# niels747/2D-Weather-Sandbox

Hardware: AMD Instinct MI355X
Metric: Mcell-steps/s (higher is better)
Workload: dtype f32

## Files before the change

2d-weather-sandbox_amd/csrc/wx_ens_score.h:

```cpp
#pragma once
#include <hip/hip_runtime.h>
#include <stdint.h>
#include <string.h>
#include "../../include/wxsim.h"
#include "wx_diag.h"
#include "wx_ens_quant.h"
#include "wx_ens_score_cell.h"

namespace wxs {

typedef unsigned long long u64;
enum { WG = wxq::WG, WAVES = wxq::WAVES, MAX_WGS = 2048, SHARDS = 8, MAP_ROWS = 4 };
enum { NQ = NT * 4, T_LO = 0, T_HI = NQ * wxd::NB, T_CNT = 2 * NQ * wxd::NB, T_SUMN = T_CNT + 16, T_LOW = T_SUMN + 4, T_HIGH = T_LOW + 4 * BINS, T_WORDS = T_HIGH + 4 * BINS };
enum { L_BINS = 0, L_CNT = 2 * NQ * wxd::NB, L_SUMN = L_CNT + 16, L_LOW = L_SUMN + 4, L_HIGH = L_LOW + 4 * BINS, L_WORDS = L_HIGH + 4 * BINS };
static_assert(MAX_MEMBERS == wxq::STAGED_MEMBERS && L_WORDS * 4 == 4720 && T_WORDS == 1180, "the tables");

struct Args {
  int X;
  int x0, y0, w, h;
  int n_sel;
  const wxe::Member *tab;
  u64 *table;
  float4 *error, *variance, *crps;
};
// ... 106 lines not shown
    for (int c = 0; c < 4; c++) {
      for (int k = 0; k < NT; k++)
        for (int b = 0; b < wxd::NB; b++) {
          a.lo[c][k][b] += tab[T_LO + (k * 4 + c) * wxd::NB + b];
          a.hi[c][k][b] += (int64_t)tab[T_HI + (k * 4 + c) * wxd::NB + b];
        }
      for (int q = 0; q < 4; q++) a.cnt[q][c] += (int64_t)tab[T_CNT + q * 4 + c];
      a.sum_count[c] += (int64_t)tab[T_SUMN + c];
      for (int b = 0; b < BINS; b++) a.low[c][b] += (int64_t)tab[T_LOW + c * BINS + b], a.high[c][b] += (int64_t)tab[T_HIGH + c * BINS + b];
    }
}

template <int P>
static hipError_t launch(const Args &a, unsigned wgs, hipStream_t stream)
{
  hipLaunchKernelGGL(k_ens_score<P>, dim3(wgs), dim3(WG), 0, stream, a);
  return hipGetLastError();
}

}

int wx_ens_score_max_members(void) { return wxs::MAX_MEMBERS; }

int wx_ens_score_cells(int n_members, size_t n_cells, const float *const *field, const int8_t *const *wall, const float *truth_field, const int8_t *truth_wall,
                       const uint8_t *member_mask, wx_ens_score *out)
{
  return wxs::score_cells(n_members, n_cells, field, wall, truth_field, truth_wall, member_mask, out);
}

int wx_ensemble_scores(wx_ensemble *e, wx_sim *truth, int field, int x, int y, int w, int h, const uint8_t *member_mask, wx_ens_score *out)
{
  if (!e || !truth || !out) return WX_E_INVALID;
  if (field != WX_FIELD_BASE_CUR && field != WX_FIELD_WATER_CUR)
    return efail(e, WX_E_INVALID, "wx_ensemble_scores: field %d: WX_FIELD_BASE_CUR or WX_FIELD_WATER_CUR (the fields that are stored whole and interleaved)", field);
  const int B = (int)e->member.size();
  const char *why;
  if (int rc = wxs::check_selection(B, member_mask, &why)) return efail(e, rc, "wx_ensemble_scores: %s", why);
  std::vector<int> sel;
  for (int i = 0; i < B; i++)
    if (!member_mask || member_mask[i]) sel.push_back(i);
  for (int i : sel)
    if (e->member[i] == truth) return efail(e, WX_E_INVALID, "wx_ensemble_scores: truth is member %d, which is selected: the truth does not enter (mask it out)", i);
  if (truth->halo != 0 || truth->X != truth->Xg) return efail(e, WX_E_INVALID, "wx_ensemble_scores: truth is a slab handle (whole-domain handles only)");
  if (truth->X != e->X || truth->Y != e->Y) return efail(e, WX_E_INVALID, "wx_ensemble_scores: truth has %d x %d cells, the members %d x %d", truth->X, truth->Y, e->X, e->Y);
  if (truth->device != e->device) return efail(e, WX_E_INVALID, "wx_ensemble_scores: truth lives on device %d, the ensemble on device %d", truth->device, e->device);
  if (w <= 0 || h <= 0 || x < 0 || y < 0 || (long long)x + w > e->X || (long long)y + h > e->Y)
    return efail(e, WX_E_RANGE, "wx_ensemble_scores: rect (%d,%d %dx%d) outside %dx%d (no wrap)", x, y, w, h, e->X, e->Y);
  for (int i : sel)
    if (!e->member[i]->uploaded) return efail(e, WX_E_STATE, "member %d: wx_ensemble_scores before wx_upload", i);
  if (!truth->uploaded) return efail(e, WX_E_STATE, "truth: wx_ensemble_scores before wx_upload");
  if (e->broken) return WX_E_STATE;
  DeviceScope dev_scope(e->member[0]);

  if (truth->ens != e)
    if (int rc = wx_sync(truth)) return efail(e, rc, "truth: %s", truth->err.c_str());

  const size_t cells = (size_t)w * h, table_bytes = (size_t)wxs::SHARDS * wxs::T_WORDS * sizeof(wxs::u64);
  float *const host_ptr[3] = {out->error, out->variance, out->crps};
  size_t at[3], out_bytes = table_bytes;
  for (int p = 0; p < 3; p++) {
    at[p] = out_bytes;
    if (host_ptr[p]) out_bytes += cells * 16;
  }
  const int n_sel = (int)sel.size();
  if (int rc = ens_stat_reserve(e, n_sel + 1, out_bytes)) return rc;
  EnsStatState *st = e->stat;

  auto entry = [&](const wx_sim *m, int i) { return wxe::Member{field == WX_FIELD_BASE_CUR ? m->base[0] : m->water[1], m->wall[0], i, 0}; };
  for (int k = 0; k < n_sel; k++) st->tab_host[k] = entry(e->member[sel[k]], sel[k]);
  st->tab_host[n_sel] = entry(truth, -1);
  wxs::Args a;
  memset(&a, 0, sizeof(a));
  a.X = e->X, a.x0 = x, a.y0 = y, a.w = w, a.h = h, a.n_sel = n_sel;
  a.tab = st->tab_dev;
  a.table = (wxs::u64 *)st->out_dev;
  auto dev_plane = [&](int p) -> float4 * { return host_ptr[p] ? (float4 *)(st->out_dev + at[p]) : nullptr; };
  a.error = dev_plane(0), a.variance = dev_plane(1), a.crps = dev_plane(2);
  int P = 1;
  while (P < n_sel) P <<= 1;

  hipError_t he = hipMemcpyAsync(st->tab_dev, st->tab_host, (size_t)(n_sel + 1) * sizeof(wxe::Member), hipMemcpyHostToDevice, e->stream);
  if (he == hipSuccess) he = hipMemsetAsync(st->out_dev, 0, table_bytes, e->stream);
  if (he == hipSuccess) {
    const unsigned chunks = (unsigned)((w + 63) / 64) * (unsigned)h;
    const unsigned wgs = std::min<unsigned>(chunks, wxs::MAX_WGS);
    ProfScope ps(e->member[0], K_ENS_SCORE);
    switch (P) {
    case 1: he = wxs::launch<1>(a, wgs, e->stream); break;
    case 2: he = wxs::launch<2>(a, wgs, e->stream); break;
    case 4: he = wxs::launch<4>(a, wgs, e->stream); break;
    case 8: he = wxs::launch<8>(a, wgs, e->stream); break;
    case 16: he = wxs::launch<16>(a, wgs, e->stream); break;
    case 32: he = wxs::launch<32>(a, wgs, e->stream); break;
    default: he = wxs::launch<wxs::MAX_MEMBERS>(a, wgs, e->stream); break;
    }
  }
  if (he == hipSuccess) he = hipMemcpyAsync(st->out_host, st->out_dev, out_bytes, hipMemcpyDeviceToHost, e->stream);
  if (he != hipSuccess) {
    (void)hipStreamSynchronize(e->stream);
    return efail(e, WX_E_DEVICE, "wx_ensemble_scores (%s): %s", kKernelNames[K_ENS_SCORE], hipGetErrorString(he));
  }
  if (int rc = wx_ensemble_sync(e)) return rc;
  wxs::Acc *acc = new wxs::Acc();
  wxs::acc_from_table((const wxs::u64 *)st->out_host, *acc);
  wxs::acc_finish(*acc, out);
  delete acc;
// ... 5 lines not shown
```

2d-weather-sandbox_amd/csrc/wx_state_copy.h:

```cpp
#pragma once

namespace {

struct StateCopyPlan {
  FullCtx fc;
};

int state_copy_check(wx_sim *dst, const wx_sim *src, const char *fn)
{
  if (src->halo != 0 || dst->halo != 0 || src->X != src->Xg || dst->X != dst->Xg) return fail(dst, WX_E_INVALID, "%s: whole-domain handles only (a slab's ghost columns and pool bookkeeping belong to its ring)", fn);
  if (src->X != dst->X || src->Y != dst->Y || src->n_drops != dst->n_drops)
    return fail(dst, WX_E_INVALID, "%s: %d x %d cells with %d droplets into %d x %d cells with %d droplets", fn, src->X, src->Y, src->n_drops, dst->X, dst->Y, dst->n_drops);
  if (src->device != dst->device) return fail(dst, WX_E_INVALID, "%s: the handles live on devices %d and %d", fn, src->device, dst->device);
  if (!src->uploaded) return fail(dst, WX_E_STATE, "%s: src was never uploaded", fn);
  if (!src->have_params) return fail(dst, WX_E_STATE, "%s: src has no parameters (wx_set_params)", fn);
  const Storage &a = src->store, &b = dst->store;
  bool same = a.created_blocks == b.created_blocks && a.created_slots == b.created_slots && a.created_small_used == b.created_small_used && a.created_blocks > 0 &&
              (int)a.blocks.size() >= a.created_blocks && (int)b.blocks.size() >= b.created_blocks;
  for (int i = 1; same && i < a.created_blocks; i++) same = a.blocks[i].bytes == b.blocks[i].bytes;
  if (!same) return fail(dst, WX_E_STATE, "%s: the two handles' storage was not laid out alike", fn);
  return WX_OK;
}

int state_copy_enqueue(wx_sim *dst, wx_sim *src, hipStream_t st, StateCopyPlan &plan)
{
  const Storage &a = src->store;
  Storage &b = dst->store;
  if (dst->copy_in_flight) HIPCHK(dst, hipStreamWaitEvent(st, dst->ev_copy_done, 0));
  for (int i = 0; i < a.created_blocks; i++) {
    const size_t bytes = i == 0 ? (a.one_arena ? a.blocks[0].bytes : a.created_small_used) : a.blocks[i].bytes;
    HIPCHK(dst, hipMemcpyAsync(b.blocks[i].p, a.blocks[i].p, bytes, hipMemcpyDeviceToDevice, st));
  }
  for (int k = 0; k < a.created_slots; k++) {
    const int i = block_of(a.blocks, *a.slots[k]);
    if (i < 0 || i >= a.created_blocks) return fail(dst, WX_E_STATE, "wx_copy_state: a registered pointer of src lies outside its blocks");
    *b.slots[k] = b.blocks[i].p + ((const char *)*a.slots[k] - a.blocks[i].p);
  }
  dst->run = src->run;
  dst->run.wet_shape_valid = false;
  dst->run.fix_check = false;
  dst->p = src->p;
  dst->geo = src->geo;
  dst->uni = src->uni;
  dst->have_params = src->have_params;
  dst->uploaded = true;
  dst->w0.even = src->w0.even;
  dst->w0.uni = src->w0.uni;
  dst->w0.initT_saved = src->w0.initT_saved;
  if (src->w0.initT_saved) {
    const size_t nb = ((size_t)src->Y + 1) * 4;
    if (!dst->w0.initT) HIPCHK(dst, hipMalloc((void **)&dst->w0.initT, nb));
    HIPCHK(dst, hipMemcpyAsync(dst->w0.initT, src->w0.initT, nb, hipMemcpyDeviceToDevice, st));
  }
  dst->vx.stale = true;
  dst->vx.untracked = false;
  dst->vx.have[0] = dst->vx.have[1] = false;
  dst->vx.check = false;
  plan.fc = FullCtx{dst->geo, dst->uni, dst->initial_T, dst->snd_T, dst->snd_W, dst->snd_Vel};
  HIPCHK(dst, hipMemcpyAsync(dst->full_ctx, &plan.fc, sizeof(FullCtx), hipMemcpyHostToDevice, st));
  HIPCHK(dst, hipMemsetAsync(&dst->state->ghost_nontrivial, 0, 5 * 4, st));
  HIPCHK(dst, hipMemsetAsync(&dst->state->vx_max_bits, 0, 2 * 4, st));
  if (dst->pair.words) {
    HIPCHK(dst, hipMemsetAsync(dst->pair.words + D2_N_REDO, 0, 4, st));
    HIPCHK(dst, hipMemsetAsync(dst->pair.words + D2_FIXED, 0, 8, st));
  }
  return WX_OK;
}

static_assert(offsetof(DevState, fastest_bits) - offsetof(DevState, ghost_nontrivial) == 16 && offsetof(DevState, cone_violation) - offsetof(DevState, vx_max_bits) == 4,
              "state_copy_enqueue zeroes these words as two runs");

}

int wx_copy_state(wx_sim *dst, wx_sim *src)
{
  if (!dst || !src) return WX_E_INVALID;
  if (dst == src) return WX_OK;
  if (int rc = state_copy_check(dst, src, "wx_copy_state")) return rc;
  DeviceScope dev_scope(src);
  if (int rc = wx_sync(src)) {
    dst->err = "wx_copy_state: src: " + src->err;
    return rc;
  }
  if (dst->comm_stream) HIPCHK(dst, hipStreamSynchronize(dst->comm_stream));
  HIPCHK(dst, hipStreamSynchronize(dst->stream));
  StateCopyPlan plan;
  int rc = state_copy_enqueue(dst, src, dst->stream, plan);
  const hipError_t he = hipStreamSynchronize(dst->stream);
  if (rc == WX_OK && he != hipSuccess) rc = fail(dst, WX_E_DEVICE, "wx_copy_state: %s", hipGetErrorString(he));
  return rc;
}

int wx_ensemble_broadcast(wx_ensemble *e, int src_member, const uint8_t *member_mask)
{
  if (!e) return WX_E_INVALID;
  const int B = (int)e->member.size();
  if (src_member < 0 || src_member >= B) return efail(e, WX_E_INVALID, "wx_ensemble_broadcast: member %d of %d", src_member, B);
  wx_sim *src = e->member[src_member];
  if (!src->uploaded) return efail(e, WX_E_STATE, "member %d: wx_ensemble_broadcast: src was never uploaded", src_member);
  if (!src->have_params) return efail(e, WX_E_STATE, "member %d: wx_ensemble_broadcast: src has no parameters (wx_set_params)", src_member);
  if (e->broken) return WX_E_STATE;
  std::vector<int> sel;
  for (int i = 0; i < B; i++)
    if (i != src_member && (!member_mask || member_mask[i])) sel.push_back(i);
  for (int i : sel)
    if (int rc = epass(e, i, state_copy_check(e->member[i], src, "wx_ensemble_broadcast"))) return rc;
  if (sel.empty()) return WX_OK;
  DeviceScope dev_scope(src);
  if (int rc = epass(e, src_member, validate_ghost_flag(src))) return rc;
  std::vector<StateCopyPlan> plans(sel.size());
  int rc = WX_OK;
  for (size_t k = 0; k < sel.size() && rc == WX_OK; k++) rc = epass(e, sel[k], state_copy_enqueue(e->member[sel[k]], src, e->stream, plans[k]));
  const hipError_t he = hipStreamSynchronize(e->stream);
  if (rc == WX_OK && he != hipSuccess) rc = efail(e, WX_E_DEVICE, "wx_ensemble_broadcast: %s", hipGetErrorString(he));
  return rc;
}
```

2d-weather-sandbox_amd/csrc/wx_tile.h:

```cpp
#pragma once
#include "wx_cells.h"

#include <cstdlib>
#include <algorithm>
#ifdef WX_DEBUG
inline const char *wx_tune_env(const char *name) { return std::getenv(name); }
#else
inline const char *wx_tune_env(const char *) { return nullptr; }
#endif

namespace wx {

constexpr int TX = 64, TY = 16;

template <typename F, typename F2> struct LightPlanesT {
  F *x, *y;
  F2 *zw;
};
using LightPlanes = LightPlanesT<float, float2>;
using LightPlanesC = LightPlanesT<const float, const float2>;

__device__ __forceinline__ size_t fidx(int x, int y, int X) { return (size_t)y * X + x; }
__device__ __forceinline__ int wrapfast(int i, int n) { return i < 0 ? i + n : (i >= n ? i - n : i); }

inline dim3 tile_grid(int X, int Y) { return dim3((X + 63) / 64, (Y + 15) / 16); }

template <int H, int W> struct Planes4 {
  float x[H][W], y[H][W], z[H][W], w[H][W];
  __device__ __forceinline__ void put(int r, int c, float4 v)
  {
    x[r][c] = v.x;
    y[r][c] = v.y;
    z[r][c] = v.z;
    w[r][c] = v.w;
  }
  __device__ __forceinline__ float4 get(int r, int c) const { return make_float4(x[r][c], y[r][c], z[r][c], w[r][c]); }
};

namespace fb_ {
constexpr int REACH = 1;
constexpr int HL = 1 + REACH, HR = REACH, HD = 1 + REACH, HU = REACH;
constexpr int IW = TX + HL + HR, IH = TY + HD + HU;
constexpr int AW = TX + 1, AH = TY + 1;
constexpr float VMAX = 0.9f;
struct SmemOut {
  float vx[AH][AW], vy[AH][AW], T[AH][AW];
  char4 w[AH][AW + 1];
};
}

struct AdvOut {
  float4 b, w;
  char4 wl;
};

__device__ __forceinline__ void edge_wave_prio(int prio)
{
#if defined(__HIP_DEVICE_COMPILE__)
  if (prio == 1) __builtin_amdgcn_s_setprio(1);
  else if (prio == 2) __builtin_amdgcn_s_setprio(2);
  else if (prio >= 3) __builtin_amdgcn_s_setprio(3);
#endif
}
struct VxTrack {
  int *max_bits;
  int *violation;
  float limit;
  int zone_l, zone_r;
  float limit_in;
};
__device__ __forceinline__ float speed8(float q0, float q1, float q2, float q3, float q4, float q5, float q6, float q7)
{
  const float m = fmaxf(fmaxf(fmaxf(fabsf(q0), fabsf(q1)), fmaxf(fabsf(q2), fabsf(q3))), fmaxf(fmaxf(fabsf(q4), fabsf(q5)), fmaxf(fabsf(q6), fabsf(q7))));
// ... 10 lines not shown
#if defined(__HIP_DEVICE_COMPILE__)
  float m = lane_max;
  if (t.zone_l < t.zone_r && strip >= t.zone_l && strip < t.zone_r) {
    if (!(t.limit_in > 0.0f)) return;
    for (int o = 32; o > 0; o >>= 1) m = fmaxf(m, __shfl_xor(m, o));
    if (lane == 0 && t.violation != nullptr && m >= t.limit_in) atomicMax(t.violation, __float_as_int(m));
    return;
  }
  for (int o = 32; o > 0; o >>= 1) m = fmaxf(m, __shfl_xor(m, o));
  if (lane == 0 && t.max_bits != nullptr && m >= 0.5f) {
    atomicMax(t.max_bits, __float_as_int(m));
    if (t.limit > 0.0f && m >= t.limit) atomicMax(t.violation, __float_as_int(m));
  }
#endif
}
__global__ void k_vx_scan(int X, int Y, int col_l, int col_r, const float4 *__restrict__ base, VxTrack t)
{
  float m = 0.0f, m_in = 0.0f;
  const size_t n = (size_t)X * Y;
  for (size_t i = (size_t)blockIdx.x * blockDim.x + threadIdx.x; i < n; i += (size_t)gridDim.x * blockDim.x) {
    const int x = (int)(i % (size_t)X);
    const float v = vx_mag(base[i].x);
    if (col_l >= col_r || x < col_l || x >= col_r)
      m = fmaxf(m, v);
    else
      m_in = fmaxf(m_in, v);
  }
  t.zone_l = t.zone_r = 0;
  vx_track_commit(t, m, threadIdx.x & 63);
  if (t.limit_in > 0.0f) {
    t.zone_l = 0;
    t.zone_r = 1;
    vx_track_commit(t, m_in, threadIdx.x & 63, 0);
  }
}

__global__ void k_light_to_planes(size_t n, const float4 *__restrict__ src, LightPlanes dst)
{
  for (size_t i = (size_t)blockIdx.x * blockDim.x + threadIdx.x; i < n; i += (size_t)gridDim.x * blockDim.x) {
    const float4 l = src[i];
    dst.x[i] = l.x;
    dst.y[i] = l.y;
    dst.zw[i] = make_float2(l.z, l.w);
  }
}
__global__ void k_light_from_planes(size_t n, LightPlanesC src, float4 *__restrict__ dst)
{
  for (size_t i = (size_t)blockIdx.x * blockDim.x + threadIdx.x; i < n; i += (size_t)gridDim.x * blockDim.x) {
    const float2 zw = src.zw[i];
    dst[i] = make_float4(src.x[i], src.y[i], zw.x, zw.y);
  }
}

}
```

2d-weather-sandbox_amd/csrc/wx_wet.h:

```cpp
#pragma once
#include "wx_cells.h"
#include "wx_tile.h"
#include <cstddef>
#include <type_traits>
#include <cstdlib>
#include <algorithm>

namespace wx {

#ifndef WX_WET_MINWAVES
#define WX_WET_MINWAVES 4
#endif
#ifndef WX_WET_WPB
#define WX_WET_WPB 4
#endif
#ifndef WX_ABL_FORCE_AIR
#define WX_ABL_FORCE_AIR 0
#endif

struct FullCtx {
  Geo g;
  Uni u;
  const float *initial_T, *snd_T, *snd_W, *snd_Vel;
};

struct WetIn {
  const float4 *base;
  const char4 *wall;
  const float4 *water;
  LightPlanesC l0;
  LightPlanesC lsrc;
  const float3 *fb;
  const float2 *dep;
  const unsigned char *fb_zero;
  const float4 *zero_row;
  int fb_txn;
};
struct WetOut {
  float4 *base;
  char4 *wall;
  float4 *water;
  LightPlanes light;
  float *p_disp;
  float4 *water0;
  float *curl;
  float *t_disp;
#ifdef WX_WET_TIMING
  unsigned long long *cycles;
#endif
};

struct WetFixList {
  int *count;
  int2 *cells;
  int cap;
  const int *hint_host;
  int *fastest;
  int *hint;
};

struct WetSlowArgs {
  const FullCtx *ctx;
  WetIn in;
  float iterNum;
};
struct GWetRecomputeAcc {
  const Uni &u_;
  const WetIn &in_;
  int X, Y, x, y;
  __device__ __forceinline__ int wx_(int dx) const { return wrapmod(x + dx, X); }
  __device__ __forceinline__ int wy_(int dy) const { return wrapmod(y + dy, Y); }
  __device__ __forceinline__ float4 vel_at(int xx, int yy) const
  {
    const int xr = xx + 1 == X ? 0 : xx + 1, yu = yy + 1 == Y ? 0 : yy + 1;
    return velocity_cell(u_, in_.base[fidx(xx, yy, X)], in_.base[fidx(xr, yy, X)].z, in_.base[fidx(xx, yu, X)].z, in_.wall[fidx(xx, yy, X)].y);
  }
  __device__ __forceinline__ float curl_at(int xx, int yy) const
  {
    const int xr = xx + 1 == X ? 0 : xx + 1, yu = yy + 1 == Y ? 0 : yy + 1;
    const float4 v = vel_at(xx, yy);
    return curl_cell(v.x, v.y, vel_at(xr, yy).y, vel_at(xx, yu).x);
  }
  __device__ __forceinline__ float4 base(int dx, int dy) const { return vel_at(wx_(dx), wy_(dy)); }
  __device__ __forceinline__ char4 wall(int dx, int dy) const { return in_.wall[fidx(wx_(dx), wy_(dy), X)]; }
  __device__ __forceinline__ float4 water(int dx, int dy) const { return in_.water[fidx(wx_(dx), wy_(dy), X)]; }
  __device__ __forceinline__ float2 vort(int dx, int dy) const
  {
    const int xx = wx_(dx), yy = wy_(dy);
    const int xl = xx == 0 ? X - 1 : xx - 1, xr = xx + 1 == X ? 0 : xx + 1, yd = yy == 0 ? Y - 1 : yy - 1, yu = yy + 1 == Y ? 0 : yy + 1;
    return vorticity_cell(curl_at(xx, yy), curl_at(xl, yy), curl_at(xr, yy), curl_at(xx, yd), curl_at(xx, yu));
  }
  __device__ __forceinline__ float light_y0() const { return in_.l0.y[fidx(x, y, X)]; }
  __device__ __forceinline__ float light_x0() const { return in_.l0.x[fidx(x, y, X)]; }
  __device__ __forceinline__ float2 light_xy_up() const
  {
    const size_t i = fidx(x, y + 1 > Y - 1 ? Y - 1 : y + 1, X);
    return make_float2(in_.l0.x[i], in_.l0.y[i]);
  }
  __device__ __forceinline__ bool has_fb() const { return in_.fb != nullptr; }
  __device__ __forceinline__ float4 fb() const
  {
    if (!in_.fb) return make_float4(0.f, 0.f, 0.f, 0.f);
    const float3 v = in_.fb[fidx(x, y, X)];
    return make_float4(v.x, v.y, v.z, 0.f);
  }
  __device__ __forceinline__ float2 dep() const { return in_.dep ? in_.dep[fidx(x, y, X)] : make_float2(0.f, 0.f); }
};
struct BOut {
  float4 b, w;
  char4 wl;
};
__device__ __noinline__ BOut wet_boundary_texel_global(const WetSlowArgs *__restrict__ sa, int x, int y)
{
  const FullCtx *c = sa->ctx;
  GWetRecomputeAcc a{c->u, sa->in, c->g.X, c->g.Y, x, y};
  BOut o;
  boundary_cell(c->u, sa->iterNum, (int)sa->iterNum, c->g, c->initial_T, x, y, a, o.b, o.w, o.wl);
  return o;
}
struct GWetAdvectAcc {
  const WetSlowArgs *sa;
  int X, Y, x, y;
  __device__ __forceinline__ BOut at(int dx, int dy) const { return wet_boundary_texel_global(sa, wrapmod(x + dx, X), wrapmod(y + dy, Y)); }
  __device__ __forceinline__ float4 base(int dx, int dy) const { return at(dx, dy).b; }
  __device__ __forceinline__ char4 wall(int dx, int dy) const { return at(dx, dy).wl; }
  __device__ __forceinline__ float4 base_off(int dx, int dy) const { return at(dx, dy).b; }
  __device__ __forceinline__ float4 water_off(int dx, int dy) const { return at(dx, dy).w; }
  __device__ __forceinline__ char4 wall_off(int dx, int dy) const { return at(dx, dy).wl; }
};
__device__ __noinline__ AdvOut wet_advection_cell_recompute(const WetSlowArgs *__restrict__ sa, int x, int y)
{
  const FullCtx *c = sa->ctx;
  GWetAdvectAcc a{sa, c->g.X, c->g.Y, x, y};
  AdvOut o;
  advection_cell(c->u, c->g, c->initial_T, c->snd_T, c->snd_W, c->snd_Vel, x, y, a, o.b, o.w, o.wl);
  return o;
}
struct GWetLightAcc {
  LightPlanesC l;
  float4 water_;
  char4 wall_;
  float T0, Td;
  int X, x;
  __device__ __forceinline__ float T(int dy) const { return dy == 0 ? T0 : Td; }
  __device__ __forceinline__ float4 water() const { return water_; }
  __device__ __forceinline__ char4 wall() const { return wall_; }
  __device__ __forceinline__ float sun_at(int dx, int j) const { return l.x[fidx(wrapmod(x + dx, X), j, X)]; }
  __device__ __forceinline__ float ir_down_at(int j) const { return l.zw[fidx(x, j, X)].x; }
  __device__ __forceinline__ float ir_up_at(int j) const { return l.zw[fidx(x, j, X)].y; }
};
__device__ __noinline__ void wet_output_cell_exact(const FullCtx *__restrict__ c, const WetIn *__restrict__ in, const WetOut *__restrict__ out, float iterNum,
                                                   int opt_out, int x, int y)
{
  const WetSlowArgs sa{c, *in, iterNum};
  const int X = c->g.X, Y = c->g.Y;
  const AdvOut o0 = wet_advection_cell_recompute(&sa, x, y);
  const AdvOut oL = wet_advection_cell_recompute(&sa, x == 0 ? X - 1 : x - 1, y);
  const AdvOut oD = wet_advection_cell_recompute(&sa, x, y == 0 ? Y - 1 : y - 1);
  const size_t gi = fidx(x, y, X);
  out->base[gi] = pressure_cell(o0.b, oL.b.x, oD.b.y, oD.b.w, oD.wl.x, oD.wl.y);
  out->water[gi] = o0.w;
  out->wall[gi] = o0.wl;
  GWetLightAcc la{in->lsrc, o0.w, o0.wl, o0.b.w, oD.b.w, X, x};
  const float4 l = lighting_cell(c->u, c->g, x, y, la);
  out->light.x[gi] = l.x;
  out->light.y[gi] = l.y;
  out->light.zw[gi] = make_float2(l.z, l.w);
  if (opt_out) out->p_disp[gi] = o0.b.z;
  if (out->t_disp) out->t_disp[gi] = o0.b.w;
}

constexpr int WOUT = 56;
constexpr int WLO = 4;
constexpr int WPAD = 1;
constexpr int WRW = 64 + 2 * WPAD;
constexpr int WQ = 3;
constexpr int WL = 4;
struct WetRing {
  float P[WQ][WRW], T[WQ][WRW], vx[WQ][WRW], vy[WQ][WRW];
  char4 wl[WQ][WRW];
  float qx[WQ][WRW], qy[WQ][WRW], qz[WQ][WRW], qw[WQ][WRW];
  float lx[WL][WRW], lw[WL][WRW];
};
static_assert(sizeof(WetRing) == (5 * WQ + 4 * WQ + 2 * WL) * WRW * 4, "ring layout");

__device__ __forceinline__ float wave_from_left(float v)
{
  const int i = __float_as_int(v);
  return __int_as_float(__builtin_amdgcn_update_dpp(i, i, 0x138 , 0xf, 0xf, false));
}
__device__ __forceinline__ float wave_from_right(float v)
{
  const int i = __float_as_int(v);
  return __int_as_float(__builtin_amdgcn_update_dpp(i, i, 0x130 , 0xf, 0xf, false));
}
__device__ __forceinline__ void wave_fence()
{
  __builtin_amdgcn_fence(__ATOMIC_RELEASE, "wavefront");
  __builtin_amdgcn_wave_barrier();
  __builtin_amdgcn_fence(__ATOMIC_ACQUIRE, "wavefront");
}
__device__ __forceinline__ char4 unpack_wall(int w)
{
  return make_char4((signed char)(w & 0xff), (signed char)((w >> 8) & 0xff), (signed char)((w >> 16) & 0xff), (signed char)(w >> 24));
}

struct MWBoundaryAcc {
  const WetRing &rg;
  int li, o0;
  float vxU, TU;
  char4 wU;
  float4 b00, q00, qU;
  char4 w00, wD;
  float vxD, TD, qzD, qwD;
// ... 94 lines not shown
  __device__ __forceinline__ float ir_up_at(int j) const { return rg.lw[(j + 8) & (WL - 1)][li]; }
};

__device__ __forceinline__ unsigned long long uniform_addr(const void *p)
{
  const unsigned long long v = (unsigned long long)p;
  const unsigned lo = __builtin_amdgcn_readfirstlane((unsigned)v), hi = __builtin_amdgcn_readfirstlane((unsigned)(v >> 32));
  return ((unsigned long long)hi << 32) | lo;
}
#if defined(__HIP_DEVICE_COMPILE__)
template <class T> __device__ __forceinline__ T ld_row(const T *row, unsigned &byte_off)
{
  typedef const __attribute__((address_space(1))) char *GBytes;
  typedef const __attribute__((address_space(1))) T *GPtr;
  asm("" : "+v"(byte_off));
  return *(GPtr)((GBytes)uniform_addr(row) + byte_off);
}
template <class T> __device__ __forceinline__ void st_row(T *row, unsigned &byte_off, T v)
{
  typedef __attribute__((address_space(1))) char *GBytes;
  asm("" : "+v"(byte_off));
  typedef __attribute__((address_space(1))) T *GPtr;
  *(GPtr)((GBytes)uniform_addr(row) + byte_off) = v;
}
#else
template <class T> __device__ __forceinline__ T ld_row(const T *row, unsigned &byte_off) { return *reinterpret_cast<const T *>(reinterpret_cast<const char *>(row) + byte_off); }
template <class T> __device__ __forceinline__ void st_row(T *row, unsigned &byte_off, T v) { *reinterpret_cast<T *>(reinterpret_cast<char *>(row) + byte_off) = v; }
#endif
template <class T> __device__ __forceinline__ T ld_row_v(const T *row, unsigned byte_off) { return ld_row(row, byte_off); }
template <class T> __device__ __forceinline__ void st_row_v(T *row, unsigned byte_off, T v) { st_row(row, byte_off, v); }
__device__ __forceinline__ int ring_back(int s, int k, int n)
{
  const int v = s - k;
  return v < 0 ? v + n : v;
}

constexpr int WMAXSEG = 128;
struct WetSegs {
  int n_seg;
  int bands;
  int start[WMAXSEG + 1];
};
struct WetKArgs {
  const FullCtx *ctx;
  float iterNum;
  WetIn in;
  WetOut out;
  WetFixList fix;
  int n_strips, strip_lo, n_strips_all;
  WetSegs segs;
  int split_at, strip_lo2;
  int edge_prio;
  VxTrack vx;
};
struct WetEnsSlot {
  WetKArgs ka;
  int *overflow;
  int pad_[2 + (16 - (sizeof(WetKArgs) + sizeof(int *) + 8) % 16) % 16 / 4];
};
static_assert(sizeof(WetEnsSlot) % 16 == 0, "table slots keep the 16-byte alignment of the wide scalar loads");
template <bool OPT_OUT, bool HAS_FB, bool QUIET>
__global__ __launch_bounds__(64 * WX_WET_WPB, WX_WET_MINWAVES) void k_march_wet(const FullCtx *__restrict__ ctx, float iterNum, WetIn in_arg, WetOut out_arg,
                                                                    WetFixList fix_arg, int n_strips, int strip_lo,
                                                                    int n_strips_all, WetSegs segs, int split_at, int strip_lo2, int edge_prio_arg, VxTrack vx_arg)
{
  typedef WetKArgs KArgs;
  typedef const __attribute__((address_space(4))) char *KBytes;
#if defined(__HIP_DEVICE_COMPILE__)
  const KBytes ka_c = (KBytes)__builtin_amdgcn_kernarg_segment_ptr();
#else
  const KBytes ka_c = nullptr;
#endif
#include "wx_wet_march_body.h"
}

template <bool OPT_OUT, bool HAS_FB, bool QUIET>
__global__ __launch_bounds__(64 * WX_WET_WPB, WX_WET_MINWAVES) void k_march_wet_ens(const WetEnsSlot *__restrict__ table)
{
  typedef WetKArgs KArgs;
  typedef const __attribute__((address_space(4))) char *KBytes;
  const KBytes ka_c = (KBytes)(const char *)table + (size_t)blockIdx.y * sizeof(WetEnsSlot);
  const __attribute__((address_space(4))) KArgs &ka = *(const __attribute__((address_space(4))) KArgs *)ka_c;
  const FullCtx *__restrict__ ctx = ka.ctx;
  const float iterNum = ka.iterNum;
  const int n_strips = ka.n_strips, strip_lo = ka.strip_lo, n_strips_all = ka.n_strips_all, split_at = ka.split_at, strip_lo2 = ka.strip_lo2;
  const __attribute__((address_space(4))) WetSegs &segs = ka.segs;
#include "wx_wet_march_body.h"
}

#undef WX_WALL_RAW
#undef WX_H_SET
#undef WX_H_ROT

constexpr int WPATCH = 8, WPATCH_C = 4;
struct WetPatch {
  float vx[WPATCH * WPATCH], vy[WPATCH * WPATCH], P[WPATCH * WPATCH], T[WPATCH * WPATCH];
  float qx[WPATCH * WPATCH], qy[WPATCH * WPATCH], qz[WPATCH * WPATCH], qw[WPATCH * WPATCH];
  char4 wl[WPATCH * WPATCH];
};
struct WetPatchAcc {
  const WetPatch &p;
  int cx, cy;
  bool *bad;
  __device__ __forceinline__ int at(int dx, int dy) const
  {
    const int x = cx + dx, y = cy + dy;
    if (x < 0 || x >= WPATCH || y < 0 || y >= WPATCH) {
      *bad = true;
      return 0;
    }
    return y * WPATCH + x;
  }
  __device__ __forceinline__ float4 base(int dx, int dy) const
  {
    const int i = at(dx, dy);
    return make_float4(p.vx[i], p.vy[i], p.P[i], p.T[i]);
  }
  __device__ __forceinline__ char4 wall(int dx, int dy) const { return p.wl[at(dx, dy)]; }
  __device__ __forceinline__ float4 base_off(int dx, int dy) const { return base(dx, dy); }
  __device__ __forceinline__ char4 wall_off(int dx, int dy) const { return wall(dx, dy); }
  __device__ __forceinline__ float4 water_off(int dx, int dy) const
  {
    const int i = at(dx, dy);
    return make_float4(p.qx[i], p.qy[i], p.qz[i], p.qw[i]);
  }
};

constexpr int WSB = 13, WSV = 12, WSC = 11, WSF = 9;
struct WetFixStage {
  float bx[WSB * WSB], by[WSB * WSB], bP[WSB * WSB], bT[WSB * WSB];
  char4 bw[WSB * WSB];
  float vx[WSV * WSV], vy[WSV * WSV];
  float cu[WSC * WSC];
  float fx[WSF * WSF], fy[WSF * WSF];
};
struct WetStageBoundaryAcc {
  const WetFixStage &st;
  const Uni &u_;
  const WetIn &in_;
  int X, Y, x, y;
  int px, py;
  __device__ __forceinline__ float4 base(int dx, int dy) const
  {
    const int iv = (py + 2 + dy) * WSV + (px + 2 + dx), ib = (py + 2 + dy) * WSB + (px + 2 + dx);
    return make_float4(st.vx[iv], st.vy[iv], st.bP[ib], st.bT[ib]);
  }
  __device__ __forceinline__ char4 wall(int dx, int dy) const { return st.bw[(py + 2 + dy) * WSB + (px + 2 + dx)]; }
  __device__ __forceinline__ float4 water(int dx, int dy) const { return in_.water[fidx(wrapmod(x + dx, X), wrapmod(y + dy, Y), X)]; }
  __device__ __forceinline__ float2 vort(int dx, int dy) const
  {
    const int i = (py + 1 + dy) * WSF + (px + 1 + dx);
    return make_float2(st.fx[i], st.fy[i]);
  }
  __device__ __forceinline__ float light_y0() const { return in_.l0.y[fidx(x, y, X)]; }
  __device__ __forceinline__ float light_x0() const { return in_.l0.x[fidx(x, y, X)]; }
  __device__ __forceinline__ float2 light_xy_up() const
  {
    const size_t i = fidx(x, y + 1 > Y - 1 ? Y - 1 : y + 1, X);
    return make_float2(in_.l0.x[i], in_.l0.y[i]);
  }
  __device__ __forceinline__ bool has_fb() const { return in_.fb != nullptr; }
  __device__ __forceinline__ float4 fb() const
  {
    if (!in_.fb) return make_float4(0.f, 0.f, 0.f, 0.f);
    const float3 v = in_.fb[fidx(x, y, X)];
    return make_float4(v.x, v.y, v.z, 0.f);
  }
  __device__ __forceinline__ float2 dep() const { return in_.dep ? in_.dep[fidx(x, y, X)] : make_float2(0.f, 0.f); }
};
__device__ __noinline__ void wet_fix_build_patch(const FullCtx *__restrict__ c, const WetIn *__restrict__ in, float iterNum, WetFixStage *__restrict__ stp,
                                                 WetPatch *__restrict__ ptp, int cx, int cy, int lane)
{
  WetFixStage &st = *stp;
  WetPatch &pt = *ptp;
  const int X = c->g.X, Y = c->g.Y;
  for (int i = lane; i < WSB * WSB; i += 64) {
    const int sy = i / WSB, sx = i - sy * WSB;
    const size_t gi = fidx(wrapmod(cx - 6 + sx, X), wrapmod(cy - 6 + sy, Y), X);
    const float4 b = in->base[gi];
    st.bx[i] = b.x;
    st.by[i] = b.y;
    st.bP[i] = b.z;
    st.bT[i] = b.w;
    st.bw[i] = in->wall[gi];
  }
  wave_fence();
  for (int i = lane; i < WSV * WSV; i += 64) {
    const int sy = i / WSV, sx = i - sy * WSV, ib = sy * WSB + sx;
    const float4 v = velocity_cell(c->u, make_float4(st.bx[ib], st.by[ib], st.bP[ib], st.bT[ib]), st.bP[ib + 1], st.bP[ib + WSB], st.bw[ib].y);
    st.vx[i] = v.x;
    st.vy[i] = v.y;
  }
  wave_fence();
  for (int i = lane; i < WSC * WSC; i += 64) {
    const int sy = i / WSC, sx = i - sy * WSC, iv = sy * WSV + sx;
    st.cu[i] = curl_cell(st.vx[iv], st.vy[iv], st.vy[iv + 1], st.vx[iv + WSV]);
  }
  wave_fence();
  for (int i = lane; i < WSF * WSF; i += 64) {
    const int sy = i / WSF, sx = i - sy * WSF, ic = (sy + 1) * WSC + (sx + 1);
    const float2 f = vorticity_cell(st.cu[ic], st.cu[ic - 1], st.cu[ic + 1], st.cu[ic - WSC], st.cu[ic + WSC]);
    st.fx[i] = f.x;
    st.fy[i] = f.y;
  }
  wave_fence();
  {
    const int px = lane & (WPATCH - 1), py = lane >> 3;
    const int gx = wrapmod(cx - WPATCH_C + px, X), gy = wrapmod(cy - WPATCH_C + py, Y);
    const WetStageBoundaryAcc a{st, c->u, *in, X, Y, gx, gy, px, py};
    float4 bb, bq;
    char4 bwl;
    boundary_cell(c->u, iterNum, (int)iterNum, c->g, c->initial_T, gx, gy, a, bb, bq, bwl);
    pt.vx[lane] = bb.x;
    pt.vy[lane] = bb.y;
    pt.P[lane] = bb.z;
    pt.T[lane] = bb.w;
    pt.qx[lane] = bq.x;
    pt.qy[lane] = bq.y;
    pt.qz[lane] = bq.z;
    pt.qw[lane] = bq.w;
    pt.wl[lane] = bwl;
  }
  wave_fence();
}

template <bool OPT_OUT>
__global__ __launch_bounds__(256) void k_wet_fix(const FullCtx *__restrict__ ctx, float iterNum, WetIn in, WetOut out, int *__restrict__ count,
                                                 const int2 *__restrict__ cells, int cap, int *__restrict__ overflow, int *__restrict__ hint)
{
#include "wx_wet_fix_body.h"
}

template <bool OPT_OUT>
__global__ __launch_bounds__(256) void k_wet_fix_ens(const WetEnsSlot *__restrict__ table)
{
  const WetEnsSlot &sl = table[blockIdx.y];
  const FullCtx *__restrict__ ctx = sl.ka.ctx;
  const float iterNum = sl.ka.iterNum;
  const WetIn in = sl.ka.in;
  const WetOut out = sl.ka.out;
  int *__restrict__ count = sl.ka.fix.count;
  const int2 *__restrict__ cells = sl.ka.fix.cells;
  const int cap = sl.ka.fix.cap;
  int *__restrict__ overflow = sl.overflow;
  int *__restrict__ hint = sl.ka.fix.hint;
#include "wx_wet_fix_body.h"
}

#ifndef WX_WET_ROUNDS
#define WX_WET_ROUNDS 4
#endif
struct WetLaunch {
  int n_strips;
  WetSegs segs;
};
inline int wet_capacity()
{
  static int capacity = 0;
  if (!capacity) {
    int dev = 0, ncu = 0, nb = 0;
    if (hipGetDevice(&dev) != hipSuccess || hipDeviceGetAttribute(&ncu, hipDeviceAttributeMultiprocessorCount, dev) != hipSuccess ||
        hipOccupancyMaxActiveBlocksPerMultiprocessor(&nb, k_march_wet<false, false, true>, 64 * WX_WET_WPB, 0) != hipSuccess || ncu <= 0 || nb <= 0) {
      capacity = 256 * 4 * WX_WET_MINWAVES;
    } else {
      hipFuncAttributes fa;
      int by_regs = nb, by_lds = nb;
      if (hipFuncGetAttributes(&fa, reinterpret_cast<const void *>(k_march_wet<false, false, true>)) == hipSuccess) {
        if (fa.numRegs > 0) by_regs = (512 / (((fa.numRegs + 7) / 8) * 8)) * 4 / WX_WET_WPB;
        if (fa.sharedSizeBytes > 0) by_lds = (int)(163840 / fa.sharedSizeBytes);
        if (wx_tune_env("WX_MARCH_DEBUG")) fprintf(stderr, "[wx_wet] numRegs=%d lds=%zu: blocks/CU by registers %d, by LDS %d, occupancy API %d\n", fa.numRegs, fa.sharedSizeBytes, by_regs, by_lds, nb);
      }
      nb = std::max(1, std::min(nb, std::min(by_regs, by_lds)));
      capacity = ncu * nb * WX_WET_WPB;
    }
    if (wx_tune_env("WX_MARCH_DEBUG")) fprintf(stderr, "[wx_wet] CUs=%d blocks/CU=%d capacity=%d\n", ncu, nb, capacity);
  }
  return capacity;
}
inline double wet_alpha()
{
  double alpha = 1.0;
  if (const char *e = wx_tune_env("WX_WET_ALPHA")) alpha = atof(e) >= 1.0 ? atof(e) : alpha;
  return alpha;
}
inline WetLaunch wet_launch_shape_cap(const Geo &g, int air_from_row, int bands_mode, const int capacity)
{
  WetLaunch w;
  const int strips_all = (g.X + WOUT - 1) / WOUT;
  bool bands = bands_mode >= 2 ? g.Y >= 16 : (bands_mode != 0 && (g.Y >= 8 * 64 || (strips_all < 146 && g.Y >= 128)));
  if (const char *e = wx_tune_env("WX_WET_BANDS")) bands = atoi(e) >= 2 ? g.Y >= 16 : (atoi(e) != 0 && g.Y >= 8 * 64);
  const int Y = bands ? (g.Y + 7) / 8 : g.Y;
  w.segs.bands = bands ? 1 : 0;
  w.n_strips = (g.X + WOUT - 1) / WOUT;
  int rounds = WX_WET_ROUNDS, minrows = 24;
  const double alpha = wet_alpha();
  if (const char *e = wx_tune_env("WX_WET_ROUNDS")) rounds = atoi(e) > 0 ? atoi(e) : rounds;
  {
    const long long cap = capacity, per_row_set = (long long)w.n_strips * (bands ? 8 : 1);
// ... 50 lines not shown
    if (n > 0 && n <= (Y + 7) / 8) n_seg = n;
  }
  w.segs.start[0] = 0;
  double wsum = 0.0, wacc = 0.0;
  for (int sg = 0; sg < n_seg; sg++) wsum += wt[sg];
  for (int sg = 1; sg < n_seg; sg++) {
    wacc += wt[sg - 1];
    const double c = total * wacc / wsum;
    int y = c <= alpha * A ? (int)(c / alpha + 0.5) : A + (int)(c - alpha * A + 0.5);
    if (y <= w.segs.start[sg - 1]) y = w.segs.start[sg - 1] + 1;
    w.segs.start[sg] = y < Y ? y : Y;
  }
  w.segs.start[n_seg] = Y;
  while (n_seg > 1 && w.segs.start[n_seg - 1] >= Y) n_seg--;
  w.segs.start[n_seg] = Y;
  w.segs.n_seg = n_seg;
  return w;
}

inline WetLaunch wet_launch_shape(const Geo &g, int air_from_row, int bands_mode = 1) { return wet_launch_shape_cap(g, air_from_row, bands_mode, wet_capacity()); }

inline int wet_member_share(const Geo &g, int n_members, int capacity)
{
  const int cap = capacity > 0 ? capacity : wet_capacity();
  if (const char *e = wx_tune_env("WX_ENS_SHARE")) n_members = atoi(e) > 0 ? atoi(e) : n_members;
  if (n_members <= 1) return cap;
  const int strips = (g.X + WOUT - 1) / WOUT;
  return std::max(cap / n_members, std::min(cap, strips));
}
inline WetLaunch wet_launch_shape_member(const Geo &g, int air_from_row, int bands_mode, int n_members, int capacity = 0)
{
  return wet_launch_shape_cap(g, air_from_row, bands_mode, wet_member_share(g, n_members, capacity));
}

inline WetLaunch wet_shape_halved(const WetLaunch &w)
{
  WetLaunch h = w;
  int n = 0;
  for (int sg = 0; sg < w.segs.n_seg; sg++) n += w.segs.start[sg + 1] - w.segs.start[sg] >= 12 ? 2 : 1;
  if (n > WMAXSEG) return w;
  n = 0;
  for (int sg = 0; sg < w.segs.n_seg; sg++) {
    const int a = w.segs.start[sg], b = w.segs.start[sg + 1];
    h.segs.start[n++] = a;
    if (b - a >= 12) h.segs.start[n++] = a + (b - a) / 2;
  }
  h.segs.start[n] = w.segs.start[w.segs.n_seg];
  h.segs.n_seg = n;
  return h;
}

inline void launch_march_wet(const WetLaunch &w, float iterNum, const FullCtx *ctx, const WetIn &in, const WetOut &out, const WetFixList &fix,
                             bool opt_out, bool quiet, hipStream_t stream, int strip_lo = 0, int strip_count = -1, int strip_lo2 = 0, int strip_count2 = 0,
                             int edge_prio = 0, const VxTrack *vx = nullptr)
{
  const int ns1 = strip_count < 0 ? w.n_strips : strip_count, ns = ns1 + (strip_count2 > 0 ? strip_count2 : 0);
  if (ns <= 0) return;
  const int groups = ((w.segs.bands ? ns : (ns + 7) / 8) + WX_WET_WPB - 1) / WX_WET_WPB;
  const dim3 grid(8 * groups * w.segs.n_seg);
  static bool dbg = wx_tune_env("WX_MARCH_DEBUG") != nullptr;
  if (dbg) {
    fprintf(stderr, "[wx_wet] strips=%d segs=%d waves=%d first/last segment rows=%d/%d\n", w.n_strips, w.segs.n_seg, w.n_strips * w.segs.n_seg,
            w.segs.start[1] - w.segs.start[0], w.segs.start[w.segs.n_seg] - w.segs.start[w.segs.n_seg - 1]);
    dbg = false;
  }
  const bool has_fb = in.fb != nullptr;
  VxTrack vt = vx ? *vx : VxTrack{nullptr, nullptr, 0.0f, 0, 0};
  if (vx && vx->zone_l < vx->zone_r) {
    vt.zone_l = (vx->zone_l + WOUT - 1) / WOUT;
    vt.zone_r = vx->zone_r / WOUT;
  }
#define WX_LAUNCH_W(O, F, Q) \
  hipLaunchKernelGGL((k_march_wet<O, F, Q>), grid, dim3(64 * WX_WET_WPB), 0, stream, ctx, iterNum, in, out, fix, ns, strip_lo, w.n_strips, w.segs, ns1, strip_lo2, edge_prio, vt)
#define WX_LAUNCH_WQ(O, F) \
  do { if (quiet) WX_LAUNCH_W(O, F, true); else WX_LAUNCH_W(O, F, false); } while (0)
  if (opt_out) {
    if (has_fb) WX_LAUNCH_WQ(true, true); else WX_LAUNCH_WQ(true, false);
  } else {
    if (has_fb) WX_LAUNCH_WQ(false, true); else WX_LAUNCH_WQ(false, false);
  }
#undef WX_LAUNCH_WQ
#undef WX_LAUNCH_W
}

inline void launch_wet_fix(float iterNum, const FullCtx *ctx, const WetIn &in, const WetOut &out, const WetFixList &fix, int *overflow, bool opt_out,
                           hipStream_t stream, int wgs = 0)
{
  const int last = fix.hint ? *(volatile const int *)fix.hint_host : -1;
  const int want = last < 0 ? 512 : (last > 0 ? std::min(512, std::max(32, last)) : 32);
  const dim3 grid(wgs > 0 ? wgs : want), block(256);
  if (opt_out)
    hipLaunchKernelGGL((k_wet_fix<true>), grid, block, 0, stream, ctx, iterNum, in, out, fix.count, fix.cells, fix.cap, overflow, fix.hint);
  else
    hipLaunchKernelGGL((k_wet_fix<false>), grid, block, 0, stream, ctx, iterNum, in, out, fix.count, fix.cells, fix.cap, overflow, fix.hint);
}

inline int ens_member_groups(const WetLaunch &w)
{
  const int groups = ((w.segs.bands ? w.n_strips : (w.n_strips + 7) / 8) + WX_WET_WPB - 1) / WX_WET_WPB;
  return 8 * groups * w.segs.n_seg;
}
inline void launch_march_wet_ens(const WetEnsSlot *table, int n_members, int groups_x, bool opt_out, bool has_fb, bool quiet, hipStream_t stream)
{
  const dim3 grid(groups_x, n_members), block(64 * WX_WET_WPB);
#define WX_LAUNCH_E(O, F, Q) hipLaunchKernelGGL((k_march_wet_ens<O, F, Q>), grid, block, 0, stream, table)
#define WX_LAUNCH_EQ(O, F) \
  do { if (quiet) WX_LAUNCH_E(O, F, true); else WX_LAUNCH_E(O, F, false); } while (0)
  if (opt_out) {
    if (has_fb) WX_LAUNCH_EQ(true, true); else WX_LAUNCH_EQ(true, false);
  } else {
    if (has_fb) WX_LAUNCH_EQ(false, true); else WX_LAUNCH_EQ(false, false);
  }
#undef WX_LAUNCH_EQ
#undef WX_LAUNCH_E
}
inline void launch_wet_fix_ens(const WetEnsSlot *table, int n_members, int wgs_per_member, bool opt_out, hipStream_t stream)
{
  const dim3 grid(wgs_per_member, n_members), block(256);
  if (opt_out) hipLaunchKernelGGL((k_wet_fix_ens<true>), grid, block, 0, stream, table);
  else hipLaunchKernelGGL((k_wet_fix_ens<false>), grid, block, 0, stream, table);
}

__global__ void k_air_from_row(int X, int Y, const char4 *__restrict__ wall, int *__restrict__ out)
{
  int best = 0;
  const size_t n = (size_t)X * Y;
  for (size_t i = (size_t)blockIdx.x * blockDim.x + threadIdx.x; i < n; i += (size_t)gridDim.x * blockDim.x) {
    const char4 w = wall[i];
    if (w.y <= 1 || w.z <= 9) {
      const int row = (int)(i / X) + 1;
      if (row < Y) best = row > best ? row : best;
    }
  }
  for (int o = 32; o > 0; o >>= 1) best = max(best, __shfl_xor(best, o));
  if ((threadIdx.x & 63) == 0 && best > 0) atomicMax(out, best);
}

}
```

2d-weather-sandbox_amd/csrc/wx_wet_fix_body.h:

```cpp
  __shared__ WetPatch patches[4];
  __shared__ WetFixStage stages[4];
  const int wave = threadIdx.x >> 6, lane = threadIdx.x & 63;
  WetPatch &pt = patches[wave];
  const int total = *count, n = total <= cap ? total : 0;
  if (total == 0) {
    if (blockIdx.x == 0 && threadIdx.x == 0 && hint && count[2] != 0) {
      count[2] = 0;
      __hip_atomic_store(hint, 0, __ATOMIC_RELAXED, __HIP_MEMORY_SCOPE_SYSTEM);
    }
    return;
  }
  if (total > cap && blockIdx.x == 0 && threadIdx.x == 0) *overflow = total;
  const int X = ctx->g.X, Y = ctx->g.Y;
  for (int i = blockIdx.x * 4 + wave; i < n; i += gridDim.x * 4) {
    const int2 c = cells[i];
    wet_fix_build_patch(ctx, &in, iterNum, &stages[wave], &pt, c.x, c.y, lane);
    AdvOut o;
    o.b = o.w = make_float4(0.f, 0.f, 0.f, 0.f);
    o.wl = make_char4(0, 0, 0, 0);
    bool bad = false;
    if (lane < 3) {
      const int ox = lane == 1 ? -1 : 0, oy = lane == 2 ? -1 : 0;
      const WetPatchAcc a{pt, WPATCH_C + ox, WPATCH_C + oy, &bad};
      advection_cell(ctx->u, ctx->g, ctx->initial_T, ctx->snd_T, ctx->snd_W, ctx->snd_Vel, wrapmod(c.x + ox, X), wrapmod(c.y + oy, Y), a, o.b, o.w, o.wl);
    }
    const bool any_bad = __any(bad);
    const float vx_l = __shfl(o.b.x, 1), vy_d = __shfl(o.b.y, 2), T_d = __shfl(o.b.w, 2);
    const int wl_d = __shfl(*reinterpret_cast<const int *>(&o.wl), 2);
    if (lane == 0) {
      if (any_bad) {
        wet_output_cell_exact(ctx, &in, &out, iterNum, OPT_OUT, c.x, c.y);
      } else {
        const char4 wD = unpack_wall(wl_d);
        const size_t gi = fidx(c.x, c.y, X);
        out.base[gi] = pressure_cell(o.b, vx_l, vy_d, T_d, wD.x, wD.y);
        out.water[gi] = o.w;
        out.wall[gi] = o.wl;
        GWetLightAcc la{in.lsrc, o.w, o.wl, o.b.w, T_d, X, c.x};
        const float4 l = lighting_cell(ctx->u, ctx->g, c.x, c.y, la);
        out.light.x[gi] = l.x;
        out.light.y[gi] = l.y;
        out.light.zw[gi] = make_float2(l.z, l.w);
        if (OPT_OUT) out.p_disp[gi] = o.b.z;
        if (out.t_disp) out.t_disp[gi] = o.b.w;
      }
    }
    wave_fence();
  }
  __syncthreads();
  if (threadIdx.x == 0 && atomicAdd(count + 1, 1) == (int)gridDim.x - 1) {
    count[1] = 0;
    count[2] = total;
    __hip_atomic_store(count, 0, __ATOMIC_RELAXED, __HIP_MEMORY_SCOPE_AGENT);
    if (hint) __hip_atomic_store(hint, total, __ATOMIC_RELAXED, __HIP_MEMORY_SCOPE_SYSTEM);
  }
```

2d-weather-sandbox_amd/csrc/wx_wet_march_body.h:

```cpp
  const __attribute__((address_space(4))) WetIn &in = *(const __attribute__((address_space(4))) WetIn *)(ka_c + offsetof(KArgs, in));
  const __attribute__((address_space(4))) WetOut &out = *(const __attribute__((address_space(4))) WetOut *)(ka_c + offsetof(KArgs, out));
  const int edge_prio = *(const __attribute__((address_space(4))) int *)(ka_c + offsetof(KArgs, edge_prio));
  __shared__ WetRing rings[WX_WET_WPB];
  const int wave = __builtin_amdgcn_readfirstlane(threadIdx.x >> 6);
  WetRing &rg = rings[wave];
  CUni &u = as_constant(ctx->u);
  const Geo g = ctx->g;
  const CFloatP initial_T = as_constant(ctx->initial_T), snd_T = as_constant(ctx->snd_T), snd_W = as_constant(ctx->snd_W), snd_Vel = as_constant(ctx->snd_Vel);
  const int X = g.X, Y = g.Y;
  const int lane = threadIdx.x & 63, li = lane + WPAD;
  const int iterI = (int)iterNum;
  const bool smooth_iter = iterI % 100 == 0;
  const int n_seg = segs.n_seg, k = blockIdx.x & 7, j = blockIdx.x >> 3;
  const bool bands = segs.bands != 0;
  const int sk0 = bands ? 0 : (k * n_strips) >> 3, nk = bands ? n_strips : (((k + 1) * n_strips) >> 3) - sk0, gk = (nk + WX_WET_WPB - 1) / WX_WET_WPB;
  if (j >= gk * n_seg) return;
  const int seg = j / gk;
  const int sloc = (j - seg * gk) * WX_WET_WPB + wave;
  if (sloc >= nk) return;
  const int sidx = sk0 + sloc;
  const int strip = sidx < split_at ? strip_lo + sidx : strip_lo2 + (sidx - split_at);
  const int item = ((bands ? k * n_seg : 0) + seg) * n_strips_all + strip;
  const int band_lo = bands ? (int)(((long long)k * g.Y) >> 3) : 0, band_hi = bands ? (int)(((long long)(k + 1) * g.Y) >> 3) : g.Y;
  const int c_out = strip * WOUT + lane - WLO;
  const int col = wrapmod(c_out, X);
  const bool lane_out = lane >= WLO && lane < WLO + WOUT && c_out < X;
  unsigned lo4 = (unsigned)col * 4u, lo8 = (unsigned)col * 8u, lo16 = (unsigned)col * 16u;
  unsigned lo12 = (unsigned)col * 12u;
  unsigned so4 = lane_out ? (unsigned)c_out * 4u : 0u, so8 = so4 * 2u, so16 = so4 * 4u;
  const int y_lo = band_lo + segs.start[seg], y_hi = min(band_lo + segs.start[seg + 1], band_hi);
  if (y_lo >= y_hi) return;
  edge_wave_prio(edge_prio);
#define WX_WALL_RAW (reinterpret_cast<const int *>(in.wall))
  (void)item;

  float4 pf_b, pf_q = make_float4(0.f, 0.f, 0.f, 0.f);
  int pf_w;
  float pf_lx = 0.f, pf_l0x = 0.f, pf_l0y = 0.f;
  float2 pf_lzw = make_float2(0.f, 0.f);
  float3 pf_fb = make_float3(0.f, 0.f, 0.f);
  float2 pf_dep = make_float2(0.f, 0.f);
  bool fb_have = false, dep_have = false;
  unsigned short pf_flag = 0x0101;
  float4 b_prev = make_float4(0.f, 0.f, 0.f, 0.f);
  int w_prev = 0;
  float4 q1 = make_float4(0.f, 0.f, 0.f, 0.f);
  float v1x = 0.f, v1y = 0.f;
  float p2 = 0.f, t2 = 0.f;
  int w2 = 0;
  float v3x = 0.f, v3y = 0.f, p3 = 0.f, t3 = 0.f;
  int w3 = 0;
  float c1 = 0.f, c2 = 0.f;
  float vfDx = 0.f;
  float TD = 0.f, vxD = 0.f, qzD = 0.f, qwD = 0.f;
  char4 wD = make_char4(0, 0, 0, 0);
  float l0x1 = 0.f, l0y1 = 0.f, lz1 = 0.f;
  float adv_vy_prev = 0.f, adv_T_prev = 0.f;
  char4 adv_w_prev = make_char4(0, 0, 0, 0);
  unsigned h_big = 0;
  unsigned h_nowall = 0;
  unsigned h_zw0 = 0;
  unsigned h_near = 15;
  float vx_seen = 0.f;
#define WX_H_SET(h, v) h = ((h) & ~1u) | ((v) ? 1u : 0u)
#define WX_H_ROT(h) h = ((h) << 1) | ((h) & 1u)
  float4 st_p = make_float4(0.f, 0.f, 0.f, 0.f), st_q = st_p, st_l = st_p, st_ab = st_p;
  char4 st_w = make_char4(0, 0, 0, 0);
  bool st_valid = false;
  bool st_td = false;

#ifdef WX_WET_TIMING
  const unsigned long long t_begin = __builtin_readcyclecounter();
#endif
  int r = y_lo - 4;
  {
    const size_t e = (size_t)wrapmod(r, Y) * X;
    pf_b = ld_row(in.base + e, lo16);
    pf_w = ld_row(WX_WALL_RAW + e, lo4);
  }
  int sq3 = (r - 3 + 12) % WQ;
  int yw_p1 = wrapmod(r + 1, Y), yw_m1 = wrapmod(r - 1, Y), yw_m2 = wrapmod(r - 2, Y), yw_m3 = wrapmod(r - 3, Y), yw_m4 = wrapmod(r - 4, Y);
  int t = 0;
#define WX_T_GE(n) (!WARM || t >= (n))
  auto step = [&](auto warm_tag) __attribute__((always_inline)) {
    constexpr bool WARM = decltype(warm_tag)::value;
    const float4 b_cur = pf_b, q_up = pf_q;
    int w_raw = pf_w;
    const float lx_cur = pf_lx, l0x_cur = pf_l0x, l0y_cur = pf_l0y;
    const float2 lzw_cur = pf_lzw;
    const float4 fb_cur = make_float4(pf_fb.x, pf_fb.y, pf_fb.z, 0.f);
    const float2 dep_cur = pf_dep;
    const bool fb_cur_have = fb_have || dep_have;
    asm volatile("" : "+v"(w_raw));
    const char4 w_cur = unpack_wall(w_raw);
#ifdef WX_STAGE_MARKS
    asm volatile("; @@ring");
#endif
    auto ring_in = [&]() {
      const int o = sq3 * WRW + li;
      (&rg.T[0][0])[o] = t3;
      (&rg.wl[0][0])[o] = unpack_wall(w3);
      rg.lx[(r - 2 + 8) & (WL - 1)][li] = lx_cur;
      rg.lw[(r - 2 + 8) & (WL - 1)][li] = lzw_cur.y;
    };
    ring_in();
#ifdef WX_STAGE_MARKS
    asm volatile("; @@prefetch");
#endif
    if (r < y_hi + 3) {
      {
        const size_t e = (size_t)yw_p1 * X;
        pf_b = ld_row(in.base + e, lo16);
        pf_w = ld_row(WX_WALL_RAW + e, lo4);
      }
      if (WX_T_GE(2)) {
        const int rl = r - 1;
        const size_t ew = (size_t)yw_m1 * X;
        pf_q = ld_row(in.water + ew, lo16);
        const size_t el = (size_t)(rl < 0 ? 0 : (rl > Y - 1 ? Y - 1 : rl)) * X;
        pf_lx = ld_row(in.lsrc.x + el, lo4);
        pf_lzw = ld_row(in.lsrc.zw + el, lo8);
        pf_l0y = ld_row(in.l0.y + ew, lo4);
        WX_H_SET(h_near, __any(w_cur.y <= 1));
        if (h_near & 15u) pf_l0x = ld_row(in.l0.x + ew, lo4);
      }
      if (HAS_FB) {
        fb_have = __any((pf_flag & 0xffu) == 0);
        dep_have = __any((pf_flag >> 8) == 0);
#if defined(WX_ABL_FB_NOFLAG) || defined(WX_ABL_FB_NOLOAD)
        fb_have = dep_have = false;
#endif
#ifdef WX_ABL_FB_NOLOAD
        pf_fb = make_float3(0.f, 0.f, 0.f);
        pf_dep = make_float2(0.f, 0.f);
#else
        {
          const size_t e = (size_t)yw_m2 * X;
          pf_fb = ld_row(fb_have ? in.fb + e : reinterpret_cast<const float3 *>(in.zero_row), lo12);
          pf_dep = ld_row((dep_have && (h_near & 4u)) ? in.dep + e : reinterpret_cast<const float2 *>(in.zero_row), lo8);
        }
#endif
#if !defined(WX_ABL_FB_NOFLAG) && !defined(WX_ABL_FB_NOLOAD)
        pf_flag = in.fb_zero != nullptr ? reinterpret_cast<const unsigned short *>(in.fb_zero)[(yw_m1 >> 4) * in.fb_txn + (col >> 6)] : (unsigned short)0;
#endif
      }
    }
#ifdef WX_STAGE_MARKS
    asm volatile("; @@stores");
#endif
    if (st_valid && lane_out) {
      const size_t e = (size_t)(r - 5) * X;
      st_row(out.base + e, so16, st_p);
      st_row(out.water + e, so16, st_q);
      st_row(out.wall + e, so4, st_w);
      st_row(out.light.x + e, so4, st_l.x);
      st_row(out.light.y + e, so4, st_l.y);
      st_row(out.light.zw + e, so8, make_float2(st_l.z, st_l.w));
      if (OPT_OUT) st_row(out.p_disp + e, so4, st_ab.z);
#ifndef WX_ABL_NO_TDISP
      if (out.t_disp && st_td) st_row(out.t_disp + e, so4, st_ab.w);
#endif
    }
    st_valid = false;
#ifdef WX_STAGE_MARKS
    asm volatile("; @@velocity");
#endif
    float v0x = 0.f, v0y = 0.f;
    if (WX_T_GE(1)) {
      const float4 v = velocity_cell(u, b_prev, wave_from_right(b_prev.z), b_cur.z, unpack_wall(w_prev).y);
      v0x = v.x;
      v0y = v.y;
    }
#ifdef WX_STAGE_MARKS
    asm volatile("; @@curlvort");
#endif
    float c0 = 0.f;
    if (WX_T_GE(2)) {
      c0 = curl_cell(v1x, v1y, wave_from_right(v1y), v0x);
      if (OPT_OUT) {
        const int yc = r - 2;
        if (lane_out && yc >= y_lo && yc < y_hi) st_row(out.curl + (size_t)yc * X, so4, c0);
      }
    }
    float2 vf = make_float2(0.f, 0.f);
    if (WX_T_GE(4)) vf = vorticity_cell(c1, wave_from_left(c1), wave_from_right(c1), c2, c0);
    const float vfLy = wave_from_left(vf.y);
    float qzL = 0.f, qwL = 0.f, qzR = 0.f, qwR = 0.f;
    if (smooth_iter) {
      qzL = wave_from_left(q1.z);
      qwL = wave_from_left(q1.w);
      qzR = wave_from_right(q1.z);
      qwR = wave_from_right(q1.w);
    }
    wave_fence();

#ifdef WX_STAGE_MARKS
    asm volatile("; @@boundary");
#endif
    if (WX_T_GE(4)) {
      const int ob0 = sq3 * WRW;
      const float4 b00 = make_float4(v3x, v3y, p3, t3);
      const char4 w00 = unpack_wall(w3);
      if (WX_T_GE(5)) {
        const int yb = yw_m3;
        const bool top = yb + 1 > Y - 1;
        MWBoundaryAcc a{rg, li, ob0, v1x, t2, unpack_wall(w2), b00, q1, q_up, w00, wD, vxD, TD, qzD, qwD, qzL, qwL, qzR, qwR, vf, vfLy, vfDx,
                        l0x1, l0y1, top ? l0x1 : l0x_cur, top ? l0y1 : l0y_cur, fb_cur, dep_cur, HAS_FB && fb_cur_have};
        float4 bb, bq;
        char4 bwl;
#ifdef WX_ABL_NOBOUNDARY
        bb = a.base(0, 0);
        bq = a.water(0, 0);
        bwl = a.wall(0, 0);
        bb.x += vf.x + vfLy + vfDx;
#else
        if (WX_ABL_FORCE_AIR || __all(lane < 2 || lane > 60 || air_cell(w00, a.wall(-1, 0), wD, a.wall(1, 0), a.wall(0, 1))))
// ... 113 lines not shown
      adv_vy_prev = ab.y;
      adv_T_prev = ab.w;
      adv_w_prev = awl;
    }
#ifdef WX_STAGE_MARKS
    asm volatile("; @@rotate");
#endif
    v3x = v1x;
    v3y = v1y;
    p3 = p2;
    t3 = t2;
    w3 = w2;
    p2 = b_prev.z;
    t2 = b_prev.w;
    w2 = w_prev;
    b_prev = b_cur;
    w_prev = w_raw;
    q1 = q_up;
    v1x = v0x;
    v1y = v0y;
    c2 = c1;
    c1 = c0;
    vfDx = vf.x;
    l0x1 = l0x_cur;
    l0y1 = l0y_cur;
    lz1 = lzw_cur.x;
    WX_H_ROT(h_big);
    WX_H_ROT(h_nowall);
    WX_H_ROT(h_zw0);
    WX_H_ROT(h_near);
    sq3 = sq3 + 1 == WQ ? 0 : sq3 + 1;
    yw_m4 = yw_m3;
    yw_m3 = yw_m2;
    yw_m2 = yw_m1;
    yw_m1 = yw_m1 + 1 == Y ? 0 : yw_m1 + 1;
    yw_p1 = yw_p1 + 1 == Y ? 0 : yw_p1 + 1;
  };
  for (; t < 8; r++, t++) step(std::true_type{});
  if (!HAS_FB && !OPT_OUT) {
    for (; r <= y_hi + 3;) {
      step(std::false_type{});
      r++;
      if (r > y_hi + 3) break;
      step(std::false_type{});
      r++;
    }
  } else {
    for (; r <= y_hi + 3; r++) step(std::false_type{});
  }
#undef WX_T_GE
  if (st_valid && lane_out) {
    const size_t e = (size_t)(y_hi - 1) * X;
    st_row(out.base + e, so16, st_p);
    st_row(out.water + e, so16, st_q);
    st_row(out.wall + e, so4, st_w);
    st_row(out.light.x + e, so4, st_l.x);
    st_row(out.light.y + e, so4, st_l.y);
    st_row(out.light.zw + e, so8, make_float2(st_l.z, st_l.w));
    if (OPT_OUT) st_row(out.p_disp + e, so4, st_ab.z);
    if (out.t_disp && st_td) st_row(out.t_disp + e, so4, st_ab.w);
  }
  {
    const __attribute__((address_space(4))) VxTrack &vc = *(const __attribute__((address_space(4))) VxTrack *)(ka_c + offsetof(KArgs, vx));
    vx_track_commit(VxTrack{vc.max_bits, vc.violation, vc.limit, vc.zone_l, vc.zone_r, vc.limit_in}, lane >= 2 && lane <= 60 ? vx_seen : 0.0f, lane, strip);
  }
#ifdef WX_WET_TIMING
  if (lane == 0) {
    out.cycles[2 * (size_t)item] = t_begin;
    out.cycles[2 * (size_t)item + 1] = __builtin_readcyclecounter();
  }
#endif
```

2d-weather-sandbox_amd/csrc/wxsim.hip:

```cpp
#include "../../include/wxsim.h"
#include "wx_tile.h"
#include "wx_wet.h"
#include "wx_dry.h"
#include "wx_march.h"
#include "wx_march2.h"
#include "wx_kernels.h"
#include "wx_precip_ens.h"
#include "wx_diag.h"

#include <hip/hip_runtime.h>
#include <hipcub/hipcub.hpp>

#include <algorithm>
#include <cmath>
#include <cstdarg>
#include <cstddef>
#include <cstdio>
#include <cstring>
#include <utility>
#include <string>
#include <vector>

using namespace wx;

// ... 47 lines not shown
  char *p;
  size_t bytes;
};

namespace {

struct FixList {
  int *words = nullptr;
  int2 *cells = nullptr;
  int cap = 0;
  int *hint_host = nullptr, *hint_dev = nullptr;
  bool create(hipStream_t st, size_t capacity, int n_words, int told_index, bool with_hint)
  {
    if (hipMalloc((void **)&words, n_words * sizeof(int)) != hipSuccess || hipMalloc((void **)&cells, std::max<size_t>(capacity, 1) * sizeof(int2)) != hipSuccess ||
        hipMemsetAsync(words, 0, n_words * sizeof(int), st) != hipSuccess) {
      destroy();
      return false;
    }
    cap = (int)capacity;
    if (with_hint && hipHostMalloc((void **)&hint_host, sizeof(int), hipHostMallocMapped) == hipSuccess && hint_host) {
      *hint_host = 1;
      if (hipHostGetDevicePointer((void **)&hint_dev, hint_host, 0) != hipSuccess) hint_dev = nullptr;
      static const int one = 1;
      if (hint_dev) hipMemcpyAsync(words + told_index, &one, 4, hipMemcpyHostToDevice, st);
    } else {
      hint_host = nullptr;
      (void)hipGetLastError();
    }
    return true;
  }
  void destroy()
  {
    hipFree(words);
    hipFree(cells);
    if (hint_host) hipHostFree(hint_host);
    *this = FixList{};
  }
  WetFixList wet(int *fastest_bits) const { return WetFixList{words, cells, cap, hint_host, fastest_bits, hint_dev}; }
  Dry2Fix dry2(int epoch) const { return Dry2Fix{words, cells, cap, epoch, hint_dev, hint_dev ? hint_host : nullptr}; }
};

struct Options {
  int fused = 2;
  int dry_march = 1;
  int dry_pairs = 1;
  int bands_mode = 1;
  int fix_cap_request = 0;
  int place_tries = 6;
  int splat_order = 0;
  int check_launches = 0;
  int pool_exact = 0;
  bool exchange_in_order = false;
  bool lazy_water0 = true;
};

struct RunState {
  int even = 1;
  int drop_cur = 0;
  int splat_par = 0;
  int period_j = 0;
  int air_from_row = -1;
  int64_t iter = 0;
  bool ran_fused = false;
  bool light_planar = false;
  bool fb_dirty = false;
  bool water_trivial = false;
  bool local_water_free = false;
  bool wall_veg_ok = false;
  bool ghost_check = false;
  bool emit_lit = false;
  Uni emit_uni;
  bool fix_check = false;
  bool wet_shape_valid = false;
  bool halo_base_only = false;
  bool water0_pending = false;
  bool disp_lazy = false;
};

struct Water0 {
  bool even = false, initT_saved = false;
  Uni uni;
  float4 *b1 = nullptr, *b2 = nullptr, *light = nullptr;
  char4 *w1 = nullptr, *w2 = nullptr;
  float *initT = nullptr, *curl = nullptr;
};

struct Split {
  hipEvent_t ev_edges = nullptr, ev_unpacked = nullptr;
  bool edges_recorded = false;
  bool unpack_pending = false;
  hipStream_t edge_stream = nullptr;
  hipEvent_t ev_fork = nullptr, ev_join = nullptr;
  FixList edge_fix;
};

struct Pool {
  unsigned char *remote = nullptr, *owned = nullptr;
  unsigned short *flips = nullptr;
  int *best = nullptr;
  int event_cap = 0, edge_cap = 0;
  bool check = false;
  int exact_pending = 0;
  char *ev_mine = nullptr, *ev_all = nullptr;
  int ev_world = 0;
  char *psend[2] = {nullptr, nullptr}, *precv[2] = {nullptr, nullptr};
  hipEvent_t ev_evpacked = nullptr, ev_evcopied = nullptr;
  int stride_events = 1 << 30;
  int *ev_seen_host = nullptr;
  hipEvent_t ev_counted = nullptr;
  bool count_pending = false;
};

struct VxWatch {
  int cone = WX_SLAB_CONE;
  float bound = 0.f;
  bool stale = true;
  bool untracked = false;
// ... 29 lines not shown
  size_t small_used = 0;
  bool one_arena = false;
  size_t arena_skew = 0;
  int arena_count = 0;
  std::vector<void **> slots;
  int created_blocks = 0, created_slots = 0;
  size_t created_small_used = 0;
  std::vector<void *> alloc_pads;
};

struct Profile {
  bool on = false;
  hipEvent_t tail = nullptr;
  bool chain = false;
  std::vector<ProfRec> recs;
  std::vector<hipEvent_t> ev_pool;
  double ms[K_COUNT] = {0};
  int n[K_COUNT] = {0};
};

}

struct wx_sim {
  int X = 0, Y = 0;
  int Xg = 0, x0 = 0;
  int halo = 0, n_drops = 0;
  int device = 0;
  int rank = 0;
  int seam = 0;
  bool uploaded = false, have_params = false;
  wx_params p{};
  Geo geo{};
  Uni uni{};
  Options opt;
  RunState run;
  hipStream_t stream = nullptr;
  hipStream_t comm_stream = nullptr;
  hipStream_t copy_stream = nullptr;
  hipEvent_t ev_fields_ready = nullptr, ev_copy_done = nullptr;
  bool copy_in_flight = false;
  float4 *base[3] = {nullptr, nullptr, nullptr};
  float4 *water[3] = {nullptr, nullptr, nullptr}, *light[2] = {nullptr, nullptr};
  char4 *wall[2] = {nullptr, nullptr};
  float *curl = nullptr;
  float2 *vort = nullptr, *dep = nullptr;
  float3 *fb = nullptr;
  float4 *fb_rgba = nullptr;
  half4 *emitted = nullptr;
  unsigned long long *diag_table = nullptr, *diag_host = nullptr;
  float *drops[2] = {nullptr, nullptr};
  float *initial_T = nullptr, *snd_T = nullptr, *snd_W = nullptr, *snd_Vel = nullptr;
  DevState *state = nullptr;
  LightPlanes lp[3] = {{nullptr, nullptr, nullptr}, {nullptr, nullptr, nullptr}, {nullptr, nullptr, nullptr}};
  float *tdisp = nullptr;
  float *pdisp = nullptr;
  FullCtx *full_ctx = nullptr;
  float4 *zero_row = nullptr;
  SplatGrid sg{};
  int *det_key[2] = {nullptr, nullptr}, *det_idx[2] = {nullptr, nullptr};
  float *det_val = nullptr;
  void *det_tmp = nullptr;
  size_t det_tmp_bytes = 0;
  WetLaunch wet_shape{};
  int wet_shape_members = 1;
  wx_ensemble *ens = nullptr;
  FixList fix;
  FixList pair;
  int pair_epoch = 0;
  Water0 w0;
  Split split;
  Pool pool;
  VxWatch vx;
  Transport tx;
  Placement place;
  Storage store;
  Profile prof;
  std::string err;
};

struct DeviceScope {
  int prev = -1;
  explicit DeviceScope(const wx_sim *s)
  {
    int cur = -1;
    if (s && hipGetDevice(&cur) == hipSuccess && cur != s->device) {
      prev = cur;
      (void)hipSetDevice(s->device);
    }
  }
  ~DeviceScope()
  {
    if (prev >= 0) (void)hipSetDevice(prev);
  }
};

extern "C" void transport_release(wx_sim *s);

namespace {

int fail(wx_sim *s, int code, const char *fmt, ...)
{
  char buf[512];
  va_list ap;
  va_start(ap, fmt);
  vsnprintf(buf, sizeof(buf), fmt, ap);
  va_end(ap);
// ... 282 lines not shown
                s->run.fb_dirty ? s->dep : nullptr};
    ProfScope ps(s, K_BOUNDARY);
    hipLaunchKernelGGL(k_boundary, grid, block, 0, s->stream, g, u, s->initial_T, in, s->base[0], s->water[0], s->wall[0]);
    LAUNCH_CHECK(s, "boundary");
  } else {
    if (int rc_ = copy_field(s, s->base[1], s->base[0])) return rc_;
    if (int rc_ = copy_field(s, s->water[1], s->water[0])) return rc_;
    if (int rc_ = copy_wall(s, s->wall[1], s->wall[0])) return rc_;
  }
  if (mask & WX_PASS_ADVECTION) {
    GridPtrs in{s->base[0], s->water[0], s->wall[0], nullptr, nullptr, nullptr, nullptr};
    ProfScope ps(s, K_ADVECTION);
    hipLaunchKernelGGL(k_advection, grid, block, 0, s->stream, g, u, s->initial_T, s->snd_T, s->snd_W, s->snd_Vel, in, s->base[1],
                       s->water[1], s->wall[1]);
    LAUNCH_CHECK(s, "advection");
  } else {
    if (int rc_ = copy_field(s, s->base[0], s->base[1])) return rc_;
    if (int rc_ = copy_field(s, s->water[0], s->water[1])) return rc_;
    if (int rc_ = copy_wall(s, s->wall[0], s->wall[1])) return rc_;
  }
  if (mask & WX_PASS_PRESSURE) {
    ProfScope ps(s, K_PRESSURE);
    hipLaunchKernelGGL(k_pressure, grid, block, 0, s->stream, g, s->base[1], s->wall[1], s->base[0], s->wall[0]);
    LAUNCH_CHECK(s, "pressure");
  } else {
    if (int rc_ = copy_field(s, s->base[1], s->base[0])) return rc_;
    if (int rc_ = copy_wall(s, s->wall[1], s->wall[0])) return rc_;
  }
  const int src = s->run.even ? 0 : 1, dst = s->run.even ? 1 : 0;
  if (mask & WX_PASS_LIGHTING) {
    ProfScope ps(s, K_LIGHTING);
    hipLaunchKernelGGL(k_lighting, grid, block, 0, s->stream, g, u, s->base[1], s->water[1], s->wall[1], s->light[src], s->light[dst]);
    LAUNCH_CHECK(s, "lighting");
  }
  return WX_OK;
}

static void light_to_planes(wx_sim *s)
{
  if (s->run.light_planar) return;
  for (int i = 0; i < 2; i++) hipLaunchKernelGGL(k_light_to_planes, dim3(2048), dim3(256), 0, s->stream, ncell(s), s->light[i], s->lp[i]);
  s->run.light_planar = true;
}
static void light_to_rgba(wx_sim *s)
{
  if (!s->run.light_planar) return;
  for (int i = 0; i < 2; i++) {
    LightPlanesC src{s->lp[i].x, s->lp[i].y, s->lp[i].zw};
    hipLaunchKernelGGL(k_light_from_planes, dim3(2048), dim3(256), 0, s->stream, ncell(s), src, s->light[i]);
  }
  s->run.light_planar = false;
}

static hipStream_t exchange_stream(const wx_sim *s)
{
  const bool in_order = (s->pool.remote && s->opt.pool_exact) || s->opt.exchange_in_order || s->tx.xchg_inline;
  return (s->comm_stream && !in_order) ? s->comm_stream : s->stream;
}

static void wait_unpacked(wx_sim *s)
{
  if (!s->split.unpack_pending) return;
  hipStreamWaitEvent(s->stream, s->split.ev_unpacked, 0);
  s->split.unpack_pending = false;
}

static int mark_unpacked(wx_sim *s, hipStream_t st)
{
  HIPCHK(s, hipEventRecord(s->split.ev_unpacked, st));
  s->split.unpack_pending = true;
  return WX_OK;
}

static VxTrack vx_track(wx_sim *s)
{
  if (s->halo > 0) s->vx.check = true;
  const int zl = s->halo > 0 ? 3 * s->halo : 0, zr = s->halo > 0 ? s->X - 3 * s->halo : 0;
  return VxTrack{&s->state->vx_max_bits, &s->state->cone_violation, s->halo > 0 ? (float)(s->vx.cone - 5) : 0.0f, zl, zr, s->halo > 0 ? (float)std::max(1, 2 * s->halo - 8) : 0.0f};
}

static int edge_stream_ready(wx_sim *s, bool need_fix_list)
{
  if (!s->split.edge_stream) {
    int prio_lo = 0, prio_hi = 0;
    if (hipDeviceGetStreamPriorityRange(&prio_lo, &prio_hi) != hipSuccess) prio_lo = prio_hi = 0;
    HIPCHK(s, hipStreamCreateWithPriority(&s->split.edge_stream, hipStreamNonBlocking, prio_hi));
    HIPCHK(s, hipEventCreateWithFlags(&s->split.ev_fork, hipEventDisableTiming));
    HIPCHK(s, hipEventCreateWithFlags(&s->split.ev_join, hipEventDisableTiming));
  }
  if (need_fix_list && !s->split.edge_fix.cells) {
    const size_t cap = std::min<size_t>(std::max<size_t>((size_t)s->Y * 8 * 64, 1u << 14), 1u << 20);
    if (!s->split.edge_fix.create(s->stream, cap, 4, 0, false)) return fail(s, WX_E_NOMEM, "wx_step: the edge group's exact-path cell list");
  }
  return WX_OK;
}

template <class Launch> int split_iteration(wx_sim *s, int edge_mode, int nl, int nr0, int n_strips, bool need_fix_list, Launch &&launch)
{
  Split &sp = s->split;
  if (edge_mode == 0 || s->halo == 0 || nl >= nr0) {
    if (edge_mode & 2) wait_unpacked(s);
    launch(s->stream, 0, -1, 0, 0, false);
  } else {
    if (int rc = edge_stream_ready(s, need_fix_list)) return rc;
    hipEventRecord(sp.ev_fork, s->stream);
    hipStreamWaitEvent(sp.edge_stream, sp.ev_fork, 0);
    if ((edge_mode & 2) && sp.unpack_pending) {
      hipStreamWaitEvent(sp.edge_stream, sp.ev_unpacked, 0);
      sp.unpack_pending = false;
    }
    launch(sp.edge_stream, 0, nl, nr0, n_strips - nr0, true);
    if (edge_mode & 1) {
      hipEventRecord(sp.ev_edges, sp.edge_stream);
      sp.edges_recorded = true;
    }
    hipEventRecord(sp.ev_join, sp.edge_stream);
    launch(s->stream, nl, nr0 - nl, 0, 0, false);
    hipStreamWaitEvent(s->stream, sp.ev_join, 0);
  }
  return WX_OK;
}

static bool march_wet_quiet(const wx_sim *s) { return !(s->uni.userInputType >= 1) && !(s->uni.airplaneValues[3] < 0.0f || s->uni.airplaneValues[3] > 0.9f); }

#ifdef WX_WET_TIMING
static unsigned long long *dbg_cycles = nullptr;
#endif
struct WetIter {
  WetIn in;
  WetOut out;
  bool opt_out, quiet;
  float iter;
};
int march_wet_prepare(wx_sim *s, bool opt_out, bool precip, WetIter &wi, int share_members = 1)
{
  const int src = s->run.even ? 0 : 1;
  light_to_planes(s);
  const LightPlanes light_dst = s->run.even ? s->lp[1] : s->lp[2];
  const bool fb = s->run.fb_dirty;
  WetIn in{s->base[0], s->wall[0], s->water[1], LightPlanesC{s->lp[0].x, s->lp[0].y, s->lp[0].zw},
           LightPlanesC{s->lp[src].x, s->lp[src].y, s->lp[src].zw}, fb ? s->fb : nullptr, fb ? s->dep : nullptr, fb ? s->sg.fb_zero : nullptr,
           s->zero_row, s->sg.TXn};
  const bool lazy_w0 = opt_out && !precip && !fb && s->opt.lazy_water0;
  WetOut out{s->base[1], s->wall[1], s->water[2], light_dst, s->pdisp, lazy_w0 ? nullptr : s->water[0], s->curl, (precip || opt_out) ? s->tdisp : nullptr};
  if (opt_out) s->run.disp_lazy = true;
  if (opt_out) {
    s->run.water0_pending = lazy_w0;
    s->w0.even = s->run.even;
    s->w0.initT_saved = false;
    s->w0.uni = s->uni;
    s->w0.uni.iterNum = (float)s->run.iter;
    s->w0.uni.iterI = (int)s->w0.uni.iterNum;
  }
#ifdef WX_WET_TIMING
  if (!dbg_cycles && hipMalloc((void **)&dbg_cycles, 16 * 8192 * WMAXSEG) != hipSuccess) return fail(s, WX_E_NOMEM, "wx_step: timing buffer");
  out.cycles = dbg_cycles;
#endif
  if (s->run.air_from_row < 0 && wet_alpha() == 1.0) {
    s->run.air_from_row = 0;
    s->run.wet_shape_valid = false;
  }
  if (s->run.air_from_row < 0) {
    int *d = &s->state->scratch_int, v = 0;
    hipMemsetAsync(d, 0, 4, s->stream);
    hipLaunchKernelGGL(k_air_from_row, dim3(1024), dim3(256), 0, s->stream, s->X, s->Y, s->wall[0], d);
    hipMemcpyAsync(&v, d, 4, hipMemcpyDeviceToHost, s->stream);
    if (hipStreamSynchronize(s->stream) != hipSuccess) return fail(s, WX_E_DEVICE, "wx_step: terrain scan failed");
    s->run.air_from_row = v < s->Y ? v : s->Y;
    s->run.wet_shape_valid = false;
  }
  if (!s->run.wet_shape_valid || s->wet_shape_members != share_members) {
    s->wet_shape = share_members > 1 ? wet_launch_shape_member(s->geo, s->run.air_from_row, s->opt.bands_mode, share_members)
                                     : wet_launch_shape(s->geo, s->run.air_from_row, s->opt.bands_mode);
    s->wet_shape_members = share_members;
    s->run.wet_shape_valid = true;
    if (wx_tune_env("WX_MARCH_DEBUG")) fprintf(stderr, "[wx_wet] air_from_row=%d of %d\n", s->run.air_from_row, s->Y);
  }
  if (!s->fix.cells) {
    size_t cap = std::min<size_t>(std::max<size_t>(ncell(s) / 4, 1u << 16), 1u << 23);
    if (s->opt.fix_cap_request > 0) cap = (size_t)s->opt.fix_cap_request;
    if (!s->fix.create(s->stream, cap, 4, 2, true)) return fail(s, WX_E_NOMEM, "wx_step: %zu bytes for the exact-path cell list", cap * sizeof(int2));
  }
  wi.in = in;
  wi.out = out;
  wi.opt_out = opt_out;
  wi.quiet = march_wet_quiet(s);
  wi.iter = (float)s->run.iter;
  return WX_OK;
}

int march_wet_launch(wx_sim *s, const WetIter &wi, int edge_mode)
{
  const WetIn &in = wi.in;
  const WetOut &out = wi.out;
  const bool opt_out = wi.opt_out, quiet = wi.quiet;
  const WetLaunch &shape = s->wet_shape;
  {
    ProfScope ps(s, K_MARCH_WET);
    const WetFixList fix = s->fix.wet(&s->state->fastest_bits);
    const VxTrack vt = vx_track(s);
    const float iter = wi.iter;
    auto launch = [&](hipStream_t st, int lo0, int cnt0, int lo1, int cnt1, bool edge_group) {
      bool halved = edge_group;
      int edge_prio = 0;
      if (edge_group) {
        edge_prio = WX_SPLIT_PRIO;
        if (const char *e = wx_tune_env("WX_SPLIT_PRIO")) edge_prio = atoi(e);
        if (const char *e = wx_tune_env("WX_SPLIT_HALVE")) halved = atoi(e) != 0;
      }
      const WetFixList fl = edge_group ? s->split.edge_fix.wet(&s->state->fastest_bits) : fix;
      launch_march_wet(halved ? wet_shape_halved(shape) : shape, iter, s->full_ctx, in, out, fl, opt_out, quiet, st, lo0, cnt0, lo1, cnt1, edge_prio, &vt);
      launch_wet_fix(iter, s->full_ctx, in, out, fl, &s->state->fix_overflow, opt_out, st, halved ? 64 : 0);
    };
    const int nl = s->halo > 0 ? (2 * s->halo - 1) / WOUT + 1 : 0, nr0 = s->halo > 0 ? (s->X - 2 * s->halo) / WOUT : shape.n_strips;
    if (int rc = split_iteration(s, edge_mode, nl, nr0, shape.n_strips, true, launch)) return rc;
    s->run.fix_check = true;
    LAUNCH_CHECK(s, "march_wet");
  }
#ifdef WX_WET_TIMING
  if (s->run.iter == 40) {
    hipStreamSynchronize(s->stream);
    const int ns = shape.n_strips, nseg = shape.segs.n_seg * (shape.segs.bands ? 8 : 1), per_band = shape.segs.n_seg;
    std::vector<unsigned long long> c(2 * (size_t)ns * nseg);
    hipMemcpy(c.data(), dbg_cycles, c.size() * 8, hipMemcpyDeviceToHost);
    unsigned long long t0 = ~0ull, t1 = 0;
    for (size_t i = 0; i < c.size(); i += 2) { t0 = c[i] < t0 ? c[i] : t0; t1 = c[i + 1] > t1 ? c[i + 1] : t1; }
    fprintf(stderr, "[wx_wet timing] kernel span %llu ticks, %d strips x %d segments\n", t1 - t0, ns, nseg);
    for (int sg = 0; sg < nseg; sg++) {
      double st = 0, du = 0, dmin = 1e30, dmax = 0, en = 0;
      for (int k = 0; k < ns; k++) {
        const size_t i = 2 * ((size_t)sg * ns + k);
        const double d = (double)(c[i + 1] - c[i]);
        st += (double)(c[i] - t0); du += d; en += (double)(c[i + 1] - t0);
        dmin = d < dmin ? d : dmin; dmax = d > dmax ? d : dmax;
      }
      const int sl = sg % per_band;
      fprintf(stderr, "  seg %3d rows %4d..%4d (%3d): start %7.0f end %7.0f  dur avg %6.0f min %6.0f max %6.0f  per row %5.1f\n", sg, shape.segs.start[sl], shape.segs.start[sl + 1],
              shape.segs.start[sl + 1] - shape.segs.start[sl], st / ns, en / ns, du / ns, dmin, dmax, du / ns / (shape.segs.start[sl + 1] - shape.segs.start[sl] + 8));
    }
  }
#endif
  return WX_OK;
}

void march_wet_commit(wx_sim *s)
{
  std::swap(s->base[0], s->base[1]);
  std::swap(s->wall[0], s->wall[1]);
  std::swap(s->water[1], s->water[2]);
  if (!s->run.even) std::swap(s->lp[0], s->lp[2]);
}

int iterate_march_wet(wx_sim *s, bool opt_out, bool precip, int edge_mode = 0)
{
  WetIter wi;
  if (int rc = march_wet_prepare(s, opt_out, precip, wi)) return rc;
  if (int rc = march_wet_launch(s, wi, edge_mode)) return rc;
  march_wet_commit(s);
  return WX_OK;
}

static bool dry_has_water(const wx_sim *s)
{
  return !(s->run.water_trivial && s->p.userInputType < 0 && s->p.airplaneValues[3] == 0.0f && s->p.soundingForcing == 0.0f);
}
static bool dry_marches(const wx_sim *s) { return !dry_has_water(s) && s->opt.dry_march && s->X >= 64; }

static bool dry_runs_in_order(const wx_sim *s)
{
  const bool dry = s->opt.fused && (s->p.pass_mask & 0x3Fu) == WX_PASS_DRY;
  const bool precip = (s->p.pass_mask & WX_PASS_PRECIPITATION) && s->p.enablePrecipitation && s->n_drops > 0;
  return dry && s->run.halo_base_only && s->opt.dry_pairs && !precip && dry_marches(s) && s->run.wall_veg_ok && s->p.userInputType < 0 && !(s->p.airplaneValues[3] > 0.9f) &&
         s->Y >= 16;
}

int iterate_dry(wx_sim *s, bool write_disp, int edge_mode = 0)
{
  if (write_disp) s->run.disp_lazy = false;
  const bool water = dry_has_water(s);
  DryIn in{s->base[0], s->wall[0], s->water[1]};
  DryOut out{s->base[1], s->wall[1], s->water[2], s->base[2]};
  const bool wall_const = s->run.wall_veg_ok && s->p.userInputType < 0 && !(s->p.airplaneValues[3] > 0.9f);
  bool wall_written = true;
  if (dry_marches(s)) {
    ProfScope ps(s, K_MARCH_DRY);
    const int n_strips = march_dry_strips(s->geo);
    const int nl = s->halo > 0 ? (2 * s->halo - 1) / MOUT + 1 : 0, nr0 = s->halo > 0 ? (s->X - 2 * s->halo) / MOUT : n_strips;
    const VxTrack vt = vx_track(s);
    auto launch = [&](hipStream_t st, int lo0, int cnt0, int lo1, int cnt1, bool) {
      launch_march_dry(s->geo, s->uni, s->full_ctx, in, out, write_disp, !wall_const, st, lo0, cnt0, lo1, cnt1, &vt);
    };
    if (int rc = split_iteration(s, edge_mode, nl, nr0, n_strips, false, launch)) return rc;
    LAUNCH_CHECK(s, "march_dry");
    wall_written = !wall_const;
  } else {
    ProfScope ps(s, K_FUSED_DRY);
    s->vx.untracked = true;
    launch_fused_dry(s->geo, s->uni, s->full_ctx, in, out, water, write_disp, s->stream);
    LAUNCH_CHECK(s, "fused_dry");
  }
  std::swap(s->base[0], s->base[1]);
  if (wall_written) std::swap(s->wall[0], s->wall[1]);
// ... 267 lines not shown
  HIPCHK(s, hipMemsetAsync(s->pool.remote, 0, (size_t)s->n_drops, s->stream));
  HIPCHK(s, hipMemsetAsync(s->pool.owned, 0, (size_t)s->n_drops, s->stream));
  HIPCHK(s, hipMemsetAsync(s->pool.flips, 0, (size_t)s->n_drops * 2, s->stream));
  hipLaunchKernelGGL(k_pool_edges_pack, dim3((s->n_drops + 255) / 256), dim3(256), 0, s->stream, s->geo, s->n_drops, 0, s->X, 0, 0, s->drops[0], s->pool.remote,
                     nullptr, nullptr, nullptr, nullptr, s->state, 0);
  HIPCHK(s, hipGetLastError());
  return WX_OK;
}

int wx_init_droplets(wx_sim *s, uint32_t seed)
{
  if (!s) return WX_E_INVALID;
  DeviceScope dev_scope(s);
  if (s->n_drops <= 0) return fail(s, WX_E_STATE, "wx_init_droplets: the handle has no droplets");
  if (int rc = drain_comm(s)) return rc;
  hipLaunchKernelGGL(k_init_droplets, dim3((s->n_drops + 255) / 256), dim3(256), 0, s->stream, s->n_drops, seed, s->drops[0], s->drops[1]);
  HIPCHK(s, hipGetLastError());
  if (int rc = pool_reset(s)) return rc;
  HIPCHK(s, hipStreamSynchronize(s->stream));
  s->run.period_j = 0;
  s->pool.exact_pending = 0;
  return WX_OK;
}

static int reset_after_upload(wx_sim *s, const float *drops)
{
  const size_t n = ncell(s);
  s->run.water0_pending = false;
  for (int i = 0; i < 2; i++) {
    HIPCHK(s, hipMemsetAsync(s->light[i], 0, n * 16, s->stream));
    if (drops && s->n_drops > 0)
      HIPCHK(s, hipMemcpyAsync(s->drops[i], drops, (size_t)s->n_drops * 20, hipMemcpyHostToDevice, s->stream));
  }
  HIPCHK(s, hipMemsetAsync(s->curl, 0, n * 4, s->stream));
  HIPCHK(s, hipMemsetAsync(s->vort, 0, n * 8, s->stream));
  HIPCHK(s, hipMemsetAsync(s->fb, 0, n * 12, s->stream));
  HIPCHK(s, hipMemsetAsync(s->dep, 0, n * 8, s->stream));
  HIPCHK(s, hipMemsetAsync(s->state->lightning, 0, 16, s->stream));
  HIPCHK(s, hipMemsetAsync(&s->state->px_count, 0, 60, s->stream));
  if (int rc = pool_reset(s)) return rc;
  if (s->sg.acc3) {
    HIPCHK(s, hipMemsetAsync(s->sg.acc3, 0, (size_t)s->sg.AP * s->sg.AH * 12, s->stream));
    HIPCHK(s, hipMemsetAsync(s->sg.acc2, 0, (size_t)s->sg.AP * s->sg.AH * 8, s->stream));
    HIPCHK(s, hipMemsetAsync(s->sg.dirty, 0, 2 * (size_t)s->sg.TXn * s->sg.TYn, s->stream));
    HIPCHK(s, hipMemsetAsync(s->sg.fb_zero, 1, 2 * (size_t)s->sg.TXn * s->sg.TYn, s->stream));
    HIPCHK(s, hipMemsetAsync(s->sg.work, 0, 64, s->stream));
    s->run.splat_par = 0;
  }
  HIPCHK(s, hipStreamSynchronize(s->stream));
  s->run.fb_dirty = false;
  s->run.air_from_row = -1;
  s->run.ghost_check = false;
  s->run.light_planar = false;
  s->run.period_j = 0;
  s->pool.exact_pending = 0;
  s->tx.since_exchange = 0;
  s->tx.exchanged = false;
  s->vx.stale = true;
  s->vx.untracked = false;
  s->vx.have[0] = s->vx.have[1] = false;
  s->run.ran_fused = false;
  s->run.even = 1;
  s->run.emit_lit = false;
  s->run.drop_cur = 0;
  s->uploaded = true;
  return WX_OK;
}

struct SetupScratch {
  char *mem = nullptr;
  double *veg;
  int32_t *rows;
  float *snow, *T, *tot, *cloud;
  unsigned int *sea;
};
static int setup_scratch(wx_sim *s, SetupScratch &q, const char *who)
{
  const int X = s->X, Y = s->Y;
  const size_t bytes = (size_t)X * (4 + 8 + 4 + 4) + (size_t)Y * 12;
  if (hipMalloc(&q.mem, bytes) != hipSuccess) return fail(s, WX_E_NOMEM, "%s: %zu bytes of device scratch", who, bytes);
  q.veg = (double *)q.mem;
  q.rows = (int32_t *)(q.veg + X);
  q.snow = (float *)(q.rows + X);
  q.T = q.snow + X;
  q.tot = q.T + Y;
  q.cloud = q.tot + Y;
  q.sea = (unsigned int *)(q.cloud + Y);
  return WX_OK;
}
static int setup_fill(wx_sim *s, SetupScratch &q, const float *T_air, const float *total_water, const float *cloud_water, const float *drops, const char *who)
{
  const int X = s->X, Y = s->Y;
  hipMemcpyAsync(q.T, T_air, (size_t)Y * 4, hipMemcpyHostToDevice, s->stream);
  hipMemcpyAsync(q.tot, total_water, (size_t)Y * 4, hipMemcpyHostToDevice, s->stream);
  hipMemcpyAsync(q.cloud, cloud_water, (size_t)Y * 4, hipMemcpyHostToDevice, s->stream);
  hipLaunchKernelGGL(k_setup_columns, grid2d(s), dim3(BX, BY), 0, s->stream, X, Y, q.rows, q.sea, q.veg, q.snow, q.T, q.tot, q.cloud, s->base[0], s->water[0],
                     s->wall[0]);
  const size_t n = ncell(s);
  hipMemcpyAsync(s->base[1], s->base[0], n * 16, hipMemcpyDeviceToDevice, s->stream);
  hipMemcpyAsync(s->water[1], s->water[0], n * 16, hipMemcpyDeviceToDevice, s->stream);
  hipMemcpyAsync(s->wall[1], s->wall[0], n * 4, hipMemcpyDeviceToDevice, s->stream);
  hipError_t e = hipStreamSynchronize(s->stream);
  hipFree(q.mem);
  q.mem = nullptr;
  if (e != hipSuccess) return fail(s, WX_E_DEVICE, "%s: %s", who, hipGetErrorString(e));
  s->run.water_trivial = s->run.local_water_free = false;
// ... 65 lines not shown
    HIPCHK(s, hipMemcpyAsync(s->full_ctx, &fc, sizeof(fc), hipMemcpyHostToDevice, s->stream));
  }
  if (p->inactiveDroplets >= 0.0f)
    HIPCHK(s, hipMemcpyAsync(&s->state->inactiveDroplets, &p->inactiveDroplets, 4, hipMemcpyHostToDevice, s->stream));
  HIPCHK(s, hipStreamSynchronize(s->stream));
  s->have_params = true;
  return WX_OK;
}

static bool step_runs_march_wet(const wx_sim *s) { return s->opt.fused && (s->p.pass_mask & 0x3Fu) == 0x3Fu; }

static int step_begin(wx_sim *s, bool dry)
{
  if (s->copy_in_flight) {
    HIPCHK(s, hipStreamWaitEvent(s->stream, s->ev_copy_done, 0));
    s->copy_in_flight = false;
  }
  if (!dry || s->p.userInputType >= 0 || s->p.airplaneValues[3] > 0.9f) s->run.wall_veg_ok = false;
  if (!dry || s->p.userInputType >= 0 || s->p.airplaneValues[3] != 0.0f || s->p.soundingForcing != 0.0f) s->run.water_trivial = s->run.local_water_free = s->run.halo_base_only = false;
  if (s->p.userInputType >= 10) s->run.air_from_row = -1;
  return WX_OK;
}
static void step_begin_iterations(wx_sim *s, int n_iter)
{
  s->split.edges_recorded = false;
  if (n_iter > 0) s->run.water0_pending = false;
}
static void step_end(wx_sim *s, int n_iter, bool dry)
{
  if (n_iter > 0) {
    s->run.emit_lit = !dry && (s->p.pass_mask & WX_PASS_LIGHTING) != 0;
    s->run.emit_uni = s->uni;
  }
}

int wx_step(wx_sim *s, int n_iter) { return wx_step_overlap(s, n_iter, 0u); }

int wx_step_overlap(wx_sim *s, int n_iter, unsigned flags)
{
  if (!s) return WX_E_INVALID;
  DeviceScope dev_scope(s);
  if (n_iter < 0) return fail(s, WX_E_INVALID, "wx_step: n_iter < 0");
  if (!s->uploaded || !s->have_params) return fail(s, WX_E_STATE, "wx_step before wx_upload / wx_set_params");
  struct TailReset {
    wx_sim *s;
    ~TailReset()
    {
      s->prof.tail = nullptr;
      s->prof.chain = false;
    }
  } tail_reset{s};
  s->prof.tail = nullptr;
  s->prof.chain = true;
  if (!s->place.done && !s->place.busy && n_iter > 0) {
    s->place.done = true;
    if (s->opt.place_tries > 0 && s->halo == 0 && ncell(s) >= WX_PLACEMENT_AUTO_CELLS && !s->store.blocks.empty()) {
      const std::string err_keep = s->err;
      if (wx_tune_placement(s, s->opt.place_tries, 20, nullptr, nullptr) != WX_OK) {
        s->err = err_keep;
        (void)hipGetLastError();
      }
    }
  }
  const unsigned mask = s->p.pass_mask;
  const bool precip = (mask & WX_PASS_PRECIPITATION) && s->p.enablePrecipitation && s->n_drops > 0;
  const bool fused = step_runs_march_wet(s);
  const bool dry = s->opt.fused && (mask & 0x3Fu) == WX_PASS_DRY;
  if (int rc = step_begin(s, dry)) return rc;
  if (precip && s->pool.remote && s->opt.pool_exact && n_iter > 0 && (n_iter > 1 || s->pool.exact_pending > 0))
    return fail(s, WX_E_STATE, "wx_step: WX_OPT_POOL_EXACT takes one iteration per call, each followed by wx_pool_events_pack / all-gather / wx_pool_events_apply");
  if (precip && s->pool.remote && n_iter > 0) {
    const int allowed = wx_slab_period(s) - s->run.period_j;
    if (n_iter > allowed)
      return fail(s, WX_E_STATE, "wx_step: %d iterations asked, %d done since the last halo exchange; %d ghost columns allow %d per period with particles",
                  n_iter, s->run.period_j, s->halo, wx_slab_period(s));
  }
  const bool dry_in_order = dry_runs_in_order(s);
  const bool can_split = (fused || (dry && dry_marches(s))) && s->comm_stream != nullptr && s->halo > 0 && !(precip && s->opt.pool_exact) && !dry_in_order;
  if (!can_split) wait_unpacked(s);
  if (!fused && s->run.light_planar) {
    wait_unpacked(s);
    light_to_rgba(s);
  }
  step_begin_iterations(s, n_iter);
  const int show_at = (flags & WX_OVERLAP_MORE_TO_COME) ? -1 : n_iter - 1;
  for (int it = 0; it < n_iter; it++) {
    int edge_mode = 0;
    if (can_split) edge_mode = ((flags & WX_OVERLAP_EDGES_LAST) && it == 0 ? 2 : 0) | ((flags & WX_OVERLAP_EDGES_FIRST) && it == n_iter - 1 && !precip ? 1 : 0);
    if (can_split && it == 0 && !(edge_mode & 2)) wait_unpacked(s);
    int rc;
    const bool pair = dry && s->opt.dry_pairs && !precip && edge_mode == 0 && it + 1 < n_iter && dry_marches(s) && s->run.wall_veg_ok && s->p.userInputType < 0 &&
                      !(s->p.airplaneValues[3] > 0.9f) && s->Y >= 16 &&
                      !(can_split && (flags & WX_OVERLAP_EDGES_FIRST) && it + 1 == n_iter - 1);
    if (pair) {
      rc = iterate_dry_pair(s, it + 1 == show_at);
      if (rc != WX_OK) return rc;
      s->run.ran_fused = true;
      s->run.iter += 2;
      it += 1;
      clear_particle_textures(s);
      continue;
    }
    if (dry)
      rc = iterate_dry(s, precip || it == show_at, edge_mode);
    else if (fused)
      rc = iterate_march_wet(s, it == show_at, precip, edge_mode);
// ... 87 lines not shown
  case WX_OPT_ROW_BANDS:
    if (value < 0 || value > 2) return fail(s, WX_E_INVALID, "wx_set_option: WX_OPT_ROW_BANDS takes 0, 1 or 2");
    s->opt.bands_mode = value;
    s->run.wet_shape_valid = false;
    return WX_OK;
  case WX_OPT_POOL_EXACT:
    if (!s->pool.remote) return fail(s, WX_E_STATE, "wx_set_option: WX_OPT_POOL_EXACT is for slab handles with particles");
    if (int rc = wx_sync(s)) return rc;
    s->opt.pool_exact = value != 0;
    s->pool.exact_pending = 0;
    return WX_OK;
  case WX_OPT_DRY_PAIRS:
    if (int rc = wx_sync(s)) return rc;
    s->opt.dry_pairs = value != 0;
    return WX_OK;
  case WX_OPT_PLACEMENT_SEARCH:
    if (value < 0 || value > 64) return fail(s, WX_E_INVALID, "wx_set_option: WX_OPT_PLACEMENT_SEARCH takes 0 (never) .. 64 tries");
    s->opt.place_tries = value;
    return WX_OK;
  case WX_OPT_WATER0_ON_DEMAND:
    if (int rc = materialize_water0(s)) return rc;
    s->opt.lazy_water0 = value != 0;
    return WX_OK;
  case WX_OPT_EXCHANGE_OVERLAP:
    s->opt.exchange_in_order = value == 0;
    return WX_OK;
  case WX_OPT_FIX_CAP:
    if (value < 0) return fail(s, WX_E_INVALID, "wx_set_option: WX_OPT_FIX_CAP >= 0");
    if (s->fix.cells) return fail(s, WX_E_STATE, "wx_set_option: WX_OPT_FIX_CAP before the first step");
    s->opt.fix_cap_request = value;
    return WX_OK;
  case WX_OPT_SPLAT_ORDER: {
    if (value != 0 && value != 1) return fail(s, WX_E_INVALID, "wx_set_option: WX_OPT_SPLAT_ORDER takes 0 (atomics) or 1 (deterministic)");
    if (value && s->n_drops > 0 && !s->det_val) {
      const size_t n = (size_t)s->n_drops;
      for (int i = 0; i < 2; i++) {
        if (int rc = dalloc(s, &s->det_key[i], n)) return rc;
        if (int rc = dalloc(s, &s->det_idx[i], n)) return rc;
      }
      if (int rc = dalloc(s, &s->det_val, 5 * n)) return rc;
      std::vector<int> iota(n);
      for (size_t i = 0; i < n; i++) iota[i] = (int)i;
      HIPCHK(s, hipMemcpy(s->det_idx[0], iota.data(), n * 4, hipMemcpyHostToDevice));
      HIPCHK(s, hipcub::DeviceRadixSort::SortPairs(nullptr, s->det_tmp_bytes, s->det_key[0], s->det_key[1], s->det_idx[0], s->det_idx[1], s->n_drops, 0, 31,
                                                   s->stream));
      HIPCHK(s, hipMalloc(&s->det_tmp, s->det_tmp_bytes ? s->det_tmp_bytes : 16));
    }
    s->opt.splat_order = value;
    return WX_OK;
  }
  case WX_OPT_CHECK_LAUNCHES:
    s->opt.check_launches = value != 0;
    return WX_OK;
  default:
    return fail(s, WX_E_INVALID, "wx_set_option: unknown option %d", option);
  }
}

static int validate_ghost_flag(wx_sim *s)
{
  if (s->vx.check) {
    int bits = 0;
    HIPCHK(s, hipMemcpyAsync(&bits, &s->state->cone_violation, 4, hipMemcpyDeviceToHost, s->stream));
    HIPCHK(s, hipStreamSynchronize(s->stream));
    s->vx.check = false;
    if (bits) {
      float v;
      memcpy(&v, &bits, 4);
      HIPCHK(s, hipMemsetAsync(&s->state->cone_violation, 0, 4, s->stream));
      return fail(s, WX_E_STATE, "|vx| reached %.3f cells / iteration in an exchange period sized for |vx| < %d (%d ghost columns per iteration): the flow accelerated "
                                 "faster than the margin of wx_slab_set_vx_bound allows, ghost columns were consumed faster than assumed and the slab may differ "
                                 "from the undecomposed run since (a velocity of 2 * halo - 8 = %d cells / iteration and more is reported wherever it occurs: from three halo widths "
                                 "inside the slab it reaches the ghost columns)", v, s->vx.cone - 5, s->vx.cone, std::max(1, 2 * s->halo - 8));
    }
  }
  if (s->run.fix_check) {
    int over = 0;
    HIPCHK(s, hipMemcpyAsync(&over, &s->state->fix_overflow, 4, hipMemcpyDeviceToHost, s->stream));
    HIPCHK(s, hipStreamSynchronize(s->stream));
    s->run.fix_check = false;
    if (over) {
      HIPCHK(s, hipMemsetAsync(&s->state->fix_overflow, 0, 4, s->stream));
      return fail(s, WX_E_STATE, "%d output cells of one iteration were fed by velocities >= 0.9 cells/iteration; the exact path holds %d: the state has "
                                 "left the simulation's range (velocities are documented as -1 .. 1) and the results since are invalid", over, s->fix.cap);
    }
  }
  if (s->pool.check) {
    int over = 0;
    HIPCHK(s, hipMemcpyAsync(&over, &s->state->pool_overflow, 4, hipMemcpyDeviceToHost, s->stream));
    HIPCHK(s, hipStreamSynchronize(s->stream));
    s->pool.check = false;
    if (over) {
      HIPCHK(s, hipMemsetAsync(&s->state->pool_overflow, 0, 4, s->stream));
      return fail(s, WX_E_STATE, "a droplet-pool exchange buffer received %d entries (event capacity %d, edge capacity %d): droplets were lost", over,
                  s->pool.event_cap, s->pool.edge_cap);
    }
  }
  if (!s->run.ghost_check) return WX_OK;
  int flag = 0;
  wait_unpacked(s);
  HIPCHK(s, hipMemcpyAsync(&flag, &s->state->ghost_nontrivial, 4, hipMemcpyDeviceToHost, s->stream));
  HIPCHK(s, hipStreamSynchronize(s->stream));
  s->run.ghost_check = false;
  if (flag) {
    s->run.water_trivial = s->run.local_water_free = s->run.wall_veg_ok = false;
    return fail(s, WX_E_STATE, "a neighbour's ghost columns carry water (or a negative vegetation byte) although wx_slab_assert_water_free(1) was "
// ... 35 lines not shown
  }
  s->store.blocks = to;
  FullCtx fc{s->geo, s->uni, s->initial_T, s->snd_T, s->snd_W, s->snd_Vel};
  HIPCHK(s, hipMemcpyAsync(s->full_ctx, &fc, sizeof(fc), hipMemcpyHostToDevice, s->stream));
  HIPCHK(s, hipStreamSynchronize(s->stream));
  return WX_OK;
}
void free_set(std::vector<Block> &B)
{
  for (Block &b : B) hipFree(b.p);
  B.clear();
}
size_t set_bytes(const std::vector<Block> &B)
{
  size_t n = 0;
  for (const Block &b : B) n += b.bytes;
  return n;
}
bool alloc_set(const std::vector<Block> &like, std::vector<Block> &out, int variant, std::vector<char *> &pads)
{
  const size_t n = like.size();
  out.assign(n, Block{nullptr, 0});
  for (size_t k = 0; k < n; k++) {
    const size_t i = (variant & 1) ? n - 1 - (k + (size_t)variant * 5) % n : (k + (size_t)variant * 5) % n;
    if (k % 3 == 0) {
      char *pad = nullptr;
      if (hipMalloc((void **)&pad, (size_t)(3 + 14 * ((variant + (int)k) % 7)) << 20) == hipSuccess) pads.push_back(pad);
      else (void)hipGetLastError();
    }
    if (block_alloc(like[i].bytes, &out[i]) != hipSuccess) {
      (void)hipGetLastError();
      free_set(out);
      return false;
    }
  }
  return true;
}
int copy_set(wx_sim *s, const std::vector<Block> &dst, const std::vector<Block> &src)
{
  for (size_t i = 0; i < src.size(); i++) HIPCHK(s, hipMemcpyAsync(dst[i].p, src[i].p, src[i].bytes, hipMemcpyDeviceToDevice, s->stream));
  return WX_OK;
}
}

int wx_tune_placement(wx_sim *s, int tries, int iters_per_try, float *ms_before, float *ms_after)
{
  if (!s) return WX_E_INVALID;
  DeviceScope dev_scope(s);
  if (tries < 1 || iters_per_try < 1) return fail(s, WX_E_INVALID, "wx_tune_placement: tries >= 1, iters_per_try >= 1");
  if (s->ens) return fail(s, WX_E_STATE, "wx_tune_placement: the handle is a member of an ensemble (its iterations share their launches with the other members)");
  if (!s->uploaded || !s->have_params) return fail(s, WX_E_STATE, "wx_tune_placement before wx_upload / wx_set_params");
  if (s->pool.remote) return fail(s, WX_E_STATE, "wx_tune_placement: not on slab handles with particles (the exchange period would advance)");
  if (int rc = materialize_water0(s)) return rc;
  if (int rc = wx_sync(s)) return rc;
  struct Busy {
    wx_sim *s;
    explicit Busy(wx_sim *s_) : s(s_) { s->place.busy = true; s->place.done = true; }
    ~Busy() { s->place.busy = false; }
  } busy(s);
  TuneSnap snap;
  if (s->store.blocks.empty() || !snap_take(s, snap)) return fail(s, WX_E_STATE, "wx_tune_placement: the handle's planes are not in registered blocks");
  int pair_ctl[D2_WORDS] = {0};
  if (s->pair.words) HIPCHK(s, hipMemcpy(pair_ctl, s->pair.words, sizeof(pair_ctl), hipMemcpyDeviceToHost));
  hipEvent_t e0, e1;
  HIPCHK(s, hipEventCreate(&e0));
  HIPCHK(s, hipEventCreate(&e1));
  const bool was_profiling = s->prof.on;
  s->prof.on = false;
  const bool dbg = wx_tune_env("WX_TUNE_DEBUG") != nullptr;
  auto probe = [&](float *ms) -> int {
    int rc = wx_step(s, 4);
    if (rc == WX_OK && hipEventRecord(e0, s->stream) != hipSuccess) rc = WX_E_DEVICE;
    if (rc == WX_OK) rc = wx_step(s, iters_per_try);
    if (rc == WX_OK && (hipEventRecord(e1, s->stream) != hipSuccess || hipEventSynchronize(e1) != hipSuccess || hipEventElapsedTime(ms, e0, e1) != hipSuccess)) rc = WX_E_DEVICE;
    *ms /= (float)iters_per_try;
    return rc;
  };
  const std::vector<Block> original = s->store.blocks;
  const size_t total = set_bytes(original);
  std::vector<char *> pads;
  auto room_for = [&](size_t bytes) {
    size_t free_b = 0, total_b = 0;
    return hipMemGetInfo(&free_b, &total_b) == hipSuccess && free_b > bytes + (size_t(2) << 30);
  };
  std::vector<Block> backup;
  if (!room_for(total) || !alloc_set(original, backup, 0, pads) || copy_set(s, backup, original) != WX_OK) {
    free_set(backup);
    for (char *p : pads) hipFree(p);
    hipEventDestroy(e0);
    hipEventDestroy(e1);
    s->prof.on = was_profiling;
    return fail(s, WX_E_NOMEM, "wx_tune_placement: no room for a copy of the state (%zu bytes)", total);
  }
  int rc = WX_OK;
  float first_ms = 0.f, best_ms = 0.f;
  rc = wx_step(s, 6 * iters_per_try);
  snap_put(s, snap);
  if (rc == WX_OK) rc = probe(&first_ms);
  snap_put(s, snap);
  if (rc == WX_OK) rc = probe(&first_ms);
  snap_put(s, snap);
  std::vector<Block> best = original;
  best_ms = first_ms;
  if (dbg) fprintf(stderr, "[wx_tune_placement] current allocations (%zu blocks, %zu MB): %.4f ms / iteration\n", original.size(), total >> 20, first_ms);
  if (dbg && wx_tune_env("WX_TUNE_DEBUG")[0] == '2') {
    fprintf(stderr, "[wx_tune_blocks] 0 %.4f", first_ms);
// ... 192 lines not shown
  if (!s || iter < 0) return WX_E_INVALID;
  s->run.iter = iter;
  return WX_OK;
}

__global__ void k_fb_to_rgba(size_t first, size_t n, const float3 *__restrict__ fb, float4 *__restrict__ out, const DevState *__restrict__ st, int mailbox)
{
  for (size_t i = first + (size_t)blockIdx.x * blockDim.x + threadIdx.x; i < first + n; i += (size_t)gridDim.x * blockDim.x) {
    const float3 v = fb[i];
    out[i] = make_float4(v.x, v.y, v.z, (mailbox && i == 1) ? st->mailbox_w : 0.0f);
  }
}
static int fb_to_rgba(wx_sim *s, int y0, int h)
{
  const size_t n = ncell(s);
  if (h <= 0 || y0 < 0 || y0 + h > s->Y) {
    y0 = 0;
    h = s->Y;
  }
  if (!s->fb_rgba && hipMalloc((void **)&s->fb_rgba, n * sizeof(float4)) != hipSuccess) {
    (void)hipGetLastError();
    s->fb_rgba = nullptr;
    s->err = "WX_FIELD_PRECIP_FB: no device memory for the RGBA copy of the feedback texture";
    return WX_E_NOMEM;
  }
  const size_t cells = (size_t)h * s->X;
  hipLaunchKernelGGL(k_fb_to_rgba, dim3((unsigned)std::min<size_t>(2048, (cells + 255) / 256)), dim3(256), 0, s->stream, (size_t)y0 * s->X, cells, s->fb, s->fb_rgba, s->state,
                     s->pool.remote ? 0 : 1);
  return hipGetLastError() == hipSuccess ? WX_OK : WX_E_DEVICE;
}

static void water0_scratch_free(wx_sim *s)
{
  for (void *q : {(void *)s->w0.b1, (void *)s->w0.b2, (void *)s->w0.light, (void *)s->w0.w1, (void *)s->w0.w2, (void *)s->w0.curl}) hipFree(q);
  s->w0.b1 = s->w0.b2 = s->w0.light = nullptr;
  s->w0.w1 = s->w0.w2 = nullptr;
  s->w0.curl = nullptr;
}
static int materialize_water0(wx_sim *s)
{
  if (!s->run.water0_pending) return WX_OK;
  DeviceScope dev_scope(s);
  const size_t n = ncell(s);
  if (!s->w0.b1) {
    bool ok = hipMalloc((void **)&s->w0.b1, n * 16) == hipSuccess && hipMalloc((void **)&s->w0.b2, n * 16) == hipSuccess && hipMalloc((void **)&s->w0.light, n * 16) == hipSuccess &&
              hipMalloc((void **)&s->w0.w1, n * 4) == hipSuccess && hipMalloc((void **)&s->w0.w2, n * 4) == hipSuccess && hipMalloc((void **)&s->w0.curl, n * 4) == hipSuccess;
    if (!ok) {
      water0_scratch_free(s);
      (void)hipGetLastError();
      return fail(s, WX_E_NOMEM, "waterTexture_0 on demand: %zu bytes of scratch", n * 60);
    }
  }
  const dim3 grid = grid2d(s), block(BX, BY);
  const float4 *base_in = s->base[1], *water_in = s->water[2];
  const char4 *wall_in = s->wall[1];
  const LightPlanes &l0 = s->w0.even ? s->lp[0] : s->lp[2];
  const float4 *light0 = s->w0.light;
  if (s->w0.even && !s->run.light_planar)
    light0 = s->light[0];
  else
    hipLaunchKernelGGL(k_light_from_planes, dim3(2048), dim3(256), 0, s->stream, n, LightPlanesC{l0.x, l0.y, l0.zw}, s->w0.light);
  ProfScope ps(s, K_BOUNDARY);
  hipLaunchKernelGGL(k_velocity, grid, block, 0, s->stream, s->geo, s->w0.uni, base_in, wall_in, s->w0.b1, s->w0.w1);
  hipLaunchKernelGGL(k_curl, grid, block, 0, s->stream, s->geo, s->w0.b1, s->w0.curl);
  hipLaunchKernelGGL(k_vorticity, grid, block, 0, s->stream, s->geo, s->w0.curl, s->vort);
  GridPtrs in{s->w0.b1, water_in, s->w0.w1, s->vort, light0, nullptr, nullptr};
  hipLaunchKernelGGL(k_boundary, grid, block, 0, s->stream, s->geo, s->w0.uni, s->w0.initT_saved ? s->w0.initT : s->initial_T, in, s->w0.b2, s->water[0], s->w0.w2);
  LAUNCH_CHECK(s, "waterTexture_0 on demand");
  s->run.water0_pending = false;
  return WX_OK;
}

static int field_info(wx_sim *s, int field, const void **ptr, int *channels, int *elem, int y0 = 0, int h = 0)
{
  switch (field) {
  case WX_FIELD_BASE_CUR: *ptr = s->base[0]; *channels = 4; *elem = 4; return 0;
  case WX_FIELD_BASE_DISP:
    if (s->run.ran_fused && s->run.disp_lazy) {
      const int r0 = h > 0 ? y0 : 0, rows = h > 0 ? h : s->Y;
      const size_t cnt = (size_t)rows * s->X;
      hipLaunchKernelGGL(k_base_disp_assemble, dim3((unsigned)std::min<size_t>(4096, (cnt + 255) / 256)), dim3(256), 0, s->stream, s->X, s->Y, r0, rows, s->base[0], s->pdisp, s->tdisp,
                         s->wall[0], s->base[2]);
    }
    *ptr = s->run.ran_fused ? s->base[2] : s->base[1]; *channels = 4; *elem = 4; return 0;
  case WX_FIELD_WATER_0:
    if (int rc = materialize_water0(s)) return rc < -1 ? rc : WX_E_DEVICE;
    *ptr = s->water[0]; *channels = 4; *elem = 4; return 0;
  case WX_FIELD_WATER_CUR: *ptr = s->water[1]; *channels = 4; *elem = 4; return 0;
  case WX_FIELD_WALL_CUR: *ptr = s->wall[0]; *channels = 4; *elem = 1; return 0;
  case WX_FIELD_WALL_DISP: *ptr = s->run.ran_fused ? s->wall[0] : s->wall[1]; *channels = 4; *elem = 1; return 0;
  case WX_FIELD_LIGHT_0:
  case WX_FIELD_LIGHT_1: {
    const int i = field == WX_FIELD_LIGHT_1 ? 1 : 0;
    if (s->run.light_planar) {
      const int r0 = h > 0 ? y0 : 0, rows = h > 0 ? h : s->Y;
      const size_t off = (size_t)r0 * s->X, cnt = (size_t)rows * s->X;
      const int wgs = (int)std::min<size_t>(2048, (cnt + 255) / 256);
      hipLaunchKernelGGL(k_light_from_planes, dim3(wgs), dim3(256), 0, s->stream, cnt, LightPlanesC{s->lp[i].x + off, s->lp[i].y + off, s->lp[i].zw + off}, s->light[i] + off);
    }
    *ptr = s->light[i]; *channels = 4; *elem = 4; return 0;
  }
  case WX_FIELD_CURL: *ptr = s->curl; *channels = 1; *elem = 4; return 0;
  case WX_FIELD_VORT: *ptr = s->vort; *channels = 2; *elem = 4; return 0;
  case WX_FIELD_PRECIP_FB:
    if (int rc = fb_to_rgba(s, y0, h)) return rc < -1 ? rc : WX_E_DEVICE;
    *ptr = s->fb_rgba; *channels = 4; *elem = 4; return 0;
  case WX_FIELD_PRECIP_DEP: *ptr = s->dep; *channels = 2; *elem = 4; return 0;
  default: return -1;
  }
}

static int emitted_rect(wx_sim *s, int x, int y, int w, int h)
{
  if (!s->emitted) {
    HIPCHK(s, hipMalloc((void **)&s->emitted, ncell(s) * sizeof(half4)));
    HIPCHK(s, hipMemsetAsync(s->emitted, 0, ncell(s) * sizeof(half4), s->stream));
  }
  if (s->copy_in_flight) {
    HIPCHK(s, hipStreamWaitEvent(s->stream, s->ev_copy_done, 0));
    s->copy_in_flight = false;
  }
  const dim3 grid((w + BX - 1) / BX, (h + BY - 1) / BY), block(BX, BY);
  if (!s->run.emit_lit) {
    HIPCHK(s, hipMemset2DAsync(s->emitted + ((size_t)y * s->X + x), (size_t)s->X * sizeof(half4), 0, (size_t)w * sizeof(half4), h, s->stream));
    return WX_OK;
  }
  const int src = s->run.even ? 1 : 0;
  if (s->run.light_planar)
    hipLaunchKernelGGL(k_emitted<true>, grid, block, 0, s->stream, s->geo, s->run.emit_uni, x, y, w, h, s->water[1], s->wall[0], nullptr, s->lp[src].x, s->emitted);
  else
    hipLaunchKernelGGL(k_emitted<false>, grid, block, 0, s->stream, s->geo, s->run.emit_uni, x, y, w, h, s->water[1], s->wall[0], s->light[src], nullptr, s->emitted);
  HIPCHK(s, hipGetLastError());
  return WX_OK;
}

int wx_read_rect(wx_sim *s, int field, int x, int y, int w, int h, void *dst, int dtype)
{
  if (!s || !dst) return WX_E_INVALID;
  DeviceScope dev_scope(s);
  if (field == WX_FIELD_LIGHTNING) {
    if (dtype != WX_DTYPE_F32 || x != 0 || y != 0 || w != 1 || h != 1) return fail(s, WX_E_RANGE, "lightning data is a 1x1 f32 texture");
    wait_unpacked(s);
    HIPCHK(s, hipMemcpyAsync(dst, s->state->lightning, 16, hipMemcpyDeviceToHost, s->stream));
    HIPCHK(s, hipStreamSynchronize(s->stream));
    return WX_OK;
  }
  wait_unpacked(s);
  if (int rc = validate_ghost_flag(s)) return rc;
  if (field == WX_FIELD_EMITTED) {
    if (w <= 0 || h <= 0 || x < 0 || y < 0 || (long long)x + w > s->X || (long long)y + h > s->Y)
      return fail(s, WX_E_RANGE, "wx_read_rect: rect (%d,%d %dx%d) outside %dx%d (no wrap)", x, y, w, h, s->X, s->Y);
    if (dtype != WX_DTYPE_F16 && dtype != WX_DTYPE_F32) return fail(s, WX_E_INVALID, "wx_read_rect: emittedLight is RGBA16F: WX_DTYPE_F16 or WX_DTYPE_F32");
    const int rc = emitted_rect(s, x, y, w, h);
    if (rc != WX_OK) return rc;
    const half4 *src = s->emitted + ((size_t)y * s->X + x);
    if (dtype == WX_DTYPE_F16) {
      HIPCHK(s, hipMemcpy2DAsync(dst, (size_t)w * 8, src, (size_t)s->X * 8, (size_t)w * 8, h, hipMemcpyDeviceToHost, s->stream));
      HIPCHK(s, hipStreamSynchronize(s->stream));
      return WX_OK;
    }
    std::vector<__half> tmp((size_t)w * h * 4);
    HIPCHK(s, hipMemcpy2DAsync(tmp.data(), (size_t)w * 8, src, (size_t)s->X * 8, (size_t)w * 8, h, hipMemcpyDeviceToHost, s->stream));
    HIPCHK(s, hipStreamSynchronize(s->stream));
    float *d = (float *)dst;
    for (size_t i = 0; i < tmp.size(); i++) d[i] = __half2float(tmp[i]);
    return WX_OK;
  }
  if (w <= 0 || h <= 0 || x < 0 || y < 0 || (long long)x + w > s->X || (long long)y + h > s->Y)
    return fail(s, WX_E_RANGE, "wx_read_rect: rect (%d,%d %dx%d) outside %dx%d (no wrap)", x, y, w, h, s->X, s->Y);
  const void *ptr;
  int ch, el;
  if (int rc = field_info(s, field, &ptr, &ch, &el, y, h)) {
    if (rc != -1) return rc;
    return fail(s, WX_E_INVALID, "wx_read_rect: unknown field %d", field);
  }
  const bool is_wall = (el == 1);
  if (is_wall ? (dtype != WX_DTYPE_I8 && dtype != WX_DTYPE_I32) : (dtype != WX_DTYPE_F32))
    return fail(s, WX_E_INVALID, "wx_read_rect: dtype %d does not fit field %d", dtype, field);
  const size_t texel = (size_t)ch * el;
  const char *src = (const char *)ptr + ((size_t)y * s->X + x) * texel;
  if (is_wall && dtype == WX_DTYPE_I32) {
    std::vector<int8_t> tmp((size_t)w * h * 4);
    HIPCHK(s, hipMemcpy2DAsync(tmp.data(), (size_t)w * texel, src, (size_t)s->X * texel, (size_t)w * texel, h, hipMemcpyDeviceToHost, s->stream));
    HIPCHK(s, hipStreamSynchronize(s->stream));
    int32_t *d = (int32_t *)dst;
    for (size_t i = 0; i < tmp.size(); i++) d[i] = tmp[i];
    return WX_OK;
  }
  HIPCHK(s, hipMemcpy2DAsync(dst, (size_t)w * texel, src, (size_t)s->X * texel, (size_t)w * texel, h, hipMemcpyDeviceToHost, s->stream));
  HIPCHK(s, hipStreamSynchronize(s->stream));
  return WX_OK;
}

int wx_read_particles(wx_sim *s, int first, int count, float *dst)
{
  if (!s || !dst) return WX_E_INVALID;
  DeviceScope dev_scope(s);
  if (first < 0 || count < 0 || (long long)first + count > s->n_drops) return fail(s, WX_E_RANGE, "wx_read_particles: [%d, %d) outside 0..%d", first, first + count, s->n_drops);
  if (count == 0) return WX_OK;
  wait_unpacked(s);
  if (int rc = validate_ghost_flag(s)) return rc;
  HIPCHK(s, hipMemcpyAsync(dst, s->drops[s->run.drop_cur] + 5 * (size_t)first, (size_t)count * 20, hipMemcpyDeviceToHost, s->stream));
  HIPCHK(s, hipStreamSynchronize(s->stream));
  return WX_OK;
}

static int diag_enqueue(wx_sim *s)
{
  if (!s->uploaded) return fail(s, WX_E_STATE, "wx_diag_collect before wx_upload");
  if ((unsigned long long)s->Xg * (unsigned long long)s->Y >= 0xFFFFFFFFull)
    return fail(s, WX_E_INVALID, "wx_diag_collect: %d x %d cells: global cell indices are 32 bits wide", s->Xg, s->Y);
  wait_unpacked(s);
  if (int rc = validate_ghost_flag(s)) return rc;
  const size_t bytes = (size_t)wxd::SHARDS * wxd::T_WORDS * sizeof(unsigned long long);
  if (!s->diag_table) {
    if (hipMalloc((void **)&s->diag_table, bytes) != hipSuccess) {
      s->diag_table = nullptr;
      return fail(s, WX_E_NOMEM, "wx_diag_collect: the device table");
    }
    if (hipHostMalloc((void **)&s->diag_host, bytes) != hipSuccess) {
      s->diag_host = nullptr;
      hipFree(s->diag_table);
      s->diag_table = nullptr;
      return fail(s, WX_E_NOMEM, "wx_diag_collect: the pinned copy of the table");
    }
  }
  HIPCHK(s, hipMemsetAsync(s->diag_table, 0, bytes, s->stream));
  const int Xo = s->X - 2 * s->halo;
  const unsigned chunks = (unsigned)((Xo + wxd::WG - 1) / wxd::WG) * (unsigned)s->Y;
  hipLaunchKernelGGL(wxd::k_diag_cells, dim3(std::min<unsigned>(chunks, wxd::MAX_WGS)), dim3(wxd::WG), 0, s->stream, s->X, s->Y, s->halo, Xo, s->Xg, s->x0, s->base[0], s->water[1],
                     s->wall[0], s->diag_table);
  if (s->n_drops > 0) {
    const unsigned wgs = std::min<unsigned>((unsigned)((s->n_drops + wxd::WG - 1) / wxd::WG), wxd::MAX_WGS);
    hipLaunchKernelGGL(wxd::k_diag_drops, dim3(wgs), dim3(wxd::WG), 0, s->stream, s->geo, s->n_drops, s->halo, s->X - s->halo, s->drops[s->run.drop_cur], s->pool.remote,
                       s->diag_table);
  }
  HIPCHK(s, hipGetLastError());
  HIPCHK(s, hipMemcpyAsync(s->diag_host, s->diag_table, bytes, hipMemcpyDeviceToHost, s->stream));
  return WX_OK;
}
static int diag_complete(wx_sim *s, wx_diag_raw *out)
{
  HIPCHK(s, hipStreamSynchronize(s->stream));
  wxd::raw_from_table(s->diag_host, out);
  out->x_global = s->Xg;
  out->y_rows = s->Y;
  out->iter = s->run.iter;
  out->count[wxd::C_CELLS] = (int64_t)(s->X - 2 * s->halo) * s->Y;
  return WX_OK;
}

int wx_diag_collect(wx_sim *s, wx_diag_raw *out)
{
  if (!s || !out) return WX_E_INVALID;
  DeviceScope dev_scope(s);
  if (int rc = diag_enqueue(s)) return rc;
  return diag_complete(s, out);
}
int wx_diag_merge(wx_diag_raw *into, const wx_diag_raw *other) { return wxd::diag_merge(into, other); }
int wx_diag_finish(const wx_diag_raw *raw, wx_diag *out) { return wxd::diag_finish(raw, out); }
int wx_diag_accumulate(wx_diag_raw *into, int quantity, const float *values, size_t n) { return wxd::diag_accumulate(into, quantity, values, n); }
int wx_diag_accumulate_cells(wx_diag_raw *into, int x_global, int y_rows, int x, int y, int n, const float *base, const float *water, const int8_t *wall)
{
  return wxd::diag_accumulate_cells(into, x_global, y_rows, x, y, n, base, water, wall);
}
int wx_diagnostics(wx_sim *s, wx_diag *out)
{
  if (!s || !out) return WX_E_INVALID;
  wx_diag_raw raw;
  if (int rc = wx_diag_collect(s, &raw)) return rc;
  return wxd::diag_finish(&raw, out);
}

namespace {
const int kStreamFields[6] = {WX_FIELD_BASE_DISP, WX_FIELD_WATER_CUR, WX_FIELD_WALL_DISP, WX_FIELD_LIGHT_0, WX_FIELD_CURL, WX_FIELD_PRECIP_FB};
}

size_t wx_stream_bytes(int w, int h) { return (w > 0 && h > 0) ? (size_t)w * h * (16 + 16 + 4 + 16 + 4 + 16 + 8) : 0; }

void *wx_host_alloc(size_t bytes)
{
  void *p = nullptr;
  return hipHostMalloc(&p, bytes, hipHostMallocDefault) == hipSuccess ? p : nullptr;
// ... 38 lines not shown
                               (size_t)w * texel[f], h, hipMemcpyDeviceToHost, s->copy_stream));
    dst += (size_t)w * h * texel[f];
  }
  HIPCHK(s, hipMemcpy2DAsync(dst, (size_t)w * 8, s->emitted + ((size_t)y * s->X + x), (size_t)s->X * 8, (size_t)w * 8, h, hipMemcpyDeviceToHost, s->copy_stream));
  HIPCHK(s, hipEventRecord(s->ev_copy_done, s->copy_stream));
  s->copy_in_flight = true;
  return WX_OK;
}

int wx_stream_wait(wx_sim *s)
{
  if (!s) return WX_E_INVALID;
  if (s->copy_stream) HIPCHK(s, hipStreamSynchronize(s->copy_stream));
  return WX_OK;
}

int wx_set_stream(wx_sim *s, void *hip_stream)
{
  if (!s) return WX_E_INVALID;
  if (s->ens) return fail(s, WX_E_STATE, "wx_set_stream: the handle is a member of an ensemble and runs on the ensemble's stream");
  HIPCHK(s, hipStreamSynchronize(s->stream));
  s->stream = (hipStream_t)hip_stream;
  return WX_OK;
}

int wx_set_comm_stream(wx_sim *s, void *hip_stream)
{
  if (!s) return WX_E_INVALID;
  if (s->ens) return fail(s, WX_E_STATE, "wx_set_comm_stream: the handle is a member of an ensemble (whole-domain members have no halo exchange)");
  DeviceScope dev_scope(s);
  HIPCHK(s, hipStreamSynchronize(s->stream));
  if (s->comm_stream) HIPCHK(s, hipStreamSynchronize(s->comm_stream));
  s->comm_stream = (hipStream_t)hip_stream;
  s->split.edges_recorded = s->split.unpack_pending = false;
  if (hip_stream && !s->split.ev_edges) {
    HIPCHK(s, hipEventCreateWithFlags(&s->split.ev_edges, hipEventDisableTiming));
    HIPCHK(s, hipEventCreateWithFlags(&s->split.ev_unpacked, hipEventDisableTiming));
  }
  return WX_OK;
}

void *wx_device_ptr(wx_sim *s, int field)
{
  if (!s) return nullptr;
  wait_unpacked(s);
  if (field == WX_FIELD_LIGHTNING) return s->state->lightning;
  if (field == WX_FIELD_EMITTED) return emitted_rect(s, 0, 0, s->X, s->Y) == WX_OK ? s->emitted : nullptr;
  const void *ptr;
  int ch, el;
  if ((field == WX_FIELD_BASE_CUR || field == WX_FIELD_WALL_CUR) && s->run.ran_fused && s->run.disp_lazy) {
    if (field_info(s, WX_FIELD_BASE_DISP, &ptr, &ch, &el) || hipStreamSynchronize(s->stream) != hipSuccess) return nullptr;
    s->run.disp_lazy = false;
  }
  if (field_info(s, field, &ptr, &ch, &el)) return nullptr;
  if (field == WX_FIELD_BASE_CUR) s->vx.untracked = true;
  return const_cast<void *>(ptr);
}

int wx_local_width(const wx_sim *s) { return s ? s->X : 0; }

size_t wx_halo_bytes(const wx_sim *s) { return s ? (size_t)s->halo * s->Y * (4 * 16 + 4 + (s->pool.remote ? 16 + 8 : 0)) : 0; }
size_t wx_halo_message_bytes(const wx_sim *s) { return s ? (s->run.halo_base_only ? (size_t)s->halo * s->Y * 16 : wx_halo_bytes(s)) : 0; }

static int halo_xstart(const wx_sim *s, int side, bool pack)
{
  if (pack) return side == 0 ? s->halo : s->X - 2 * s->halo;
  return side == 0 ? 0 : s->X - s->halo;
}

static HaloBufs halo_bufs(const wx_sim *s, void *const dev_buf[2], bool pack, int *n_slots)
{
  const int n = s->halo * s->Y;
  const size_t o8 = (size_t)n * (s->pool.remote ? 80 : 64), o4 = o8 + (s->pool.remote ? (size_t)n * 8 : 0);
  HaloBufs hb{};
  int k = 0;
  for (int side = 0; side < 2; side++) {
    if (!dev_buf[side]) continue;
    hb.x_start[k] = halo_xstart(s, side, pack);
    hb.buf16[k] = (float4 *)dev_buf[side];
    hb.buf8[k] = (float2 *)((char *)dev_buf[side] + o8);
    hb.buf4[k] = (char4 *)((char *)dev_buf[side] + o4);
    k++;
  }
  *n_slots = k;
  return hb;
}
static int halo_pack_impl(wx_sim *s, void *const dev_buf[2])
{
  DeviceScope dev_scope(s);
  if (s->halo == 0) return fail(s, WX_E_STATE, "handle has no halo");
  if (s->run.halo_base_only && !(s->run.water_trivial && s->run.wall_veg_ok))
    return fail(s, WX_E_STATE, "the slabs agreed on the water-free dry stencil (wx_slab_assert_water_free(s, 1)) but THIS slab is not water-free -- its upload "
                               "carried water, or it was given new contents since: its neighbours expect base-only halo messages. Combine wx_water_free "
                               "of every slab and call wx_slab_assert_water_free on all of them again");
  const int n = s->halo * s->Y;
  const LightPlanes none{nullptr, nullptr, nullptr};
  HaloPtrs f{s->base[0], s->water[1], s->light[0], s->light[1], s->run.light_planar ? s->lp[0] : none, s->run.light_planar ? s->lp[1] : none, s->wall[0],
             s->pool.remote ? s->fb : nullptr, s->pool.remote ? s->dep : nullptr};
  hipStream_t st = exchange_stream(s);
  if (st != s->stream) {
    if (!s->split.edges_recorded) {
      HIPCHK(s, hipEventRecord(s->split.ev_edges, s->stream));
      s->split.edges_recorded = true;
    }
    HIPCHK(s, hipStreamWaitEvent(st, s->split.ev_edges, 0));
  }
  ProfScope ps(s, K_HALO);
  int slots = 0;
  const HaloBufs hb = halo_bufs(s, dev_buf, true, &slots);
// ... 260 lines not shown
```

2d-weather-sandbox_amd/engine.py:

```python
from __future__ import annotations

import ctypes as C
import os
import subprocess
from typing import Optional

import numpy as np

from .params import WxParams

_HERE = os.path.dirname(os.path.abspath(__file__))
CSRC = os.path.join(_HERE, "csrc")
FAST_LIB_PATH = os.path.join(CSRC, "libwxsim_fast.so")
LIB_PATH = os.environ.get("WXSIM_LIB") or os.path.join(CSRC, "libwxsim.so")

FIELD_IDS = {
    "BASE_CUR": 0, "BASE_DISP": 1, "WATER_0": 2, "WATER_CUR": 3, "WALL_CUR": 4, "WALL_DISP": 5,
    "LIGHT_0": 6, "LIGHT_1": 7, "CURL": 8, "VORT": 9, "PRECIP_FB": 10, "PRECIP_DEP": 11, "LIGHTNING": 12, "EMITTED": 13,
}
FIELD_CHANNELS = {"CURL": 1, "VORT": 2, "PRECIP_DEP": 2}
DTYPE_F32, DTYPE_I8, DTYPE_I32, DTYPE_F16 = 0, 1, 2, 3

EXPORTS = [
    "wx_create", "wx_create_slab", "wx_destroy", "wx_last_error", "wx_abi_version", "wx_upload", "wx_set_params",
    "wx_step", "wx_sync", "wx_get_iter", "wx_set_iter", "wx_read_rect", "wx_read_particles", "wx_set_stream",
    "wx_device_ptr", "wx_local_width", "wx_halo_bytes", "wx_halo_message_bytes", "wx_halo_pack", "wx_halo_unpack", "wx_halo_pack_both", "wx_halo_unpack_both", "wx_profile",
    "wx_profile_read", "wx_kernel_count", "wx_kernel_name", "wx_slab_set_rank", "wx_slab_period_begin", "wx_pool_event_bytes",
    "wx_pool_edge_bytes", "wx_pool_events_pack", "wx_pool_events_apply", "wx_pool_edges_pack", "wx_pool_edges_apply", "wx_pool_flags", "wx_lightning_get", "wx_lightning_set", "wx_setup_columns", "wx_setup_terrain", "wx_init_droplets", "wx_fastest_velocity",
    "wx_stream_bytes", "wx_host_alloc", "wx_host_free", "wx_stream_frame", "wx_stream_wait", "wx_set_comm_stream", "wx_step_overlap",
    "wx_set_option", "wx_water_free", "wx_slab_assert_water_free", "wx_tune_placement",
    "wx_comm_unique_id", "wx_comm_init", "wx_exchange", "wx_slab_step", "wx_group_create", "wx_group_destroy", "wx_group_last_error",
    "wx_group_count", "wx_group_transport", "wx_group_slab", "wx_group_agree", "wx_group_step", "wx_group_sync", "wx_group_set_option",
    "wx_group_exchange", "wx_slab_vx_take", "wx_slab_set_vx_bound", "wx_slab_cone", "wx_slab_period", "wx_pair_stats", "wx_placement_info", "wx_arith",
    "wx_diag_collect", "wx_diag_merge", "wx_diag_finish", "wx_diag_accumulate", "wx_diag_accumulate_cells", "wx_diagnostics", "wx_group_diagnostics",
    "wx_ensemble_create", "wx_ensemble_destroy", "wx_ensemble_last_error", "wx_ensemble_count", "wx_ensemble_member", "wx_ensemble_step",
    "wx_ensemble_sync", "wx_ensemble_diagnostics", "wx_ensemble_stats", "wx_ensemble_create_droplets", "wx_ensemble_particle_stats",
    "wx_ensemble_statistics", "wx_ens_stat_cells",
    "wx_copy_state", "wx_ensemble_broadcast", "wx_ensemble_perturb", "wx_ens_perturb_cells",
    "wx_ensemble_quantiles", "wx_ens_quant_cells", "wx_ens_quant_staged_members",
    "wx_ensemble_scores", "wx_ens_score_cells", "wx_ens_score_max_members",
    "wx_ensemble_assimilate", "wx_ens_assim_cells",
]


class WxDiag(C.Structure):
    _fields_ = [
        ("iter", C.c_int64), ("n_air", C.c_int64), ("n_wall", C.c_int64), ("n_marker_mismatch", C.c_int64), ("n_negative_water", C.c_int64),
        ("n_nonfinite_base", C.c_int64), ("n_nonfinite_water", C.c_int64),
        ("first_nonfinite_base_x", C.c_int64), ("first_nonfinite_base_y", C.c_int64),
        ("first_nonfinite_water_x", C.c_int64), ("first_nonfinite_water_y", C.c_int64),
        ("sum_base", C.c_double * 4), ("sum_water", C.c_double * 4), ("sum_soil_moisture", C.c_double), ("sum_snow", C.c_double),
        ("sum_vegetation", C.c_int64),
        ("min_base", C.c_double * 4), ("max_base", C.c_double * 4), ("min_water", C.c_double * 4), ("max_water", C.c_double * 4),
        ("min_base_x", C.c_int64 * 4), ("min_base_y", C.c_int64 * 4), ("max_base_x", C.c_int64 * 4), ("max_base_y", C.c_int64 * 4),
        ("min_water_x", C.c_int64 * 4), ("min_water_y", C.c_int64 * 4), ("max_water_x", C.c_int64 * 4), ("max_water_y", C.c_int64 * 4),
        ("n_droplets_active", C.c_int64), ("n_droplets_nonfinite", C.c_int64),
        ("sum_droplet_mass_x", C.c_double), ("sum_droplet_mass_y", C.c_double),
    ]


DIAG_QUANTITIES, DIAG_BINS = 12, 16
DIAG_Q = {"vx": 0, "vy": 1, "pressure": 2, "temperature": 3, "water": 4, "cloud": 5, "precipitation": 6, "smoke": 7,
          "soil_moisture": 8, "snow": 9, "droplet_mass_x": 10, "droplet_mass_y": 11}


class WxDiagRaw(C.Structure):
    _fields_ = [
        ("x_global", C.c_int64), ("y_rows", C.c_int64), ("iter", C.c_int64), ("count", C.c_int64 * 10),
        ("first_nonfinite", C.c_uint64 * 2), ("key_max", C.c_uint64 * 8), ("key_min", C.c_uint64 * 8),
        ("bin_hi", (C.c_int64 * DIAG_BINS) * DIAG_QUANTITIES), ("bin_lo", (C.c_uint64 * DIAG_BINS) * DIAG_QUANTITIES),
    ]


DIAG_RAW_BYTES = C.sizeof(WxDiagRaw)


def _diag_dict(d: WxDiag) -> dict:
    def at(x, y):
        return (int(x), int(y)) if x >= 0 else None
    out = {}
    for name, _ in WxDiag._fields_:
        if name.endswith(("_x", "_y")) and not name.startswith("sum_"):
            continue
        v = getattr(d, name)
        out[name] = list(v) if hasattr(v, "__len__") else v
    out["first_nonfinite_base"] = at(d.first_nonfinite_base_x, d.first_nonfinite_base_y)
    out["first_nonfinite_water"] = at(d.first_nonfinite_water_x, d.first_nonfinite_water_y)
    for k in ("min_base", "max_base", "min_water", "max_water"):
        xs, ys = getattr(d, k + "_x"), getattr(d, k + "_y")
        out[k + "_at"] = [at(xs[c], ys[c]) for c in range(4)]
        out[k] = [out[k][c] if xs[c] >= 0 or out[k][c] == out[k][c] else None for c in range(4)]
    return out


# ... 370 lines not shown
    L.wx_last_error.argtypes = [vp]
    L.wx_last_error.restype = C.c_char_p
    L.wx_abi_version.restype = i32
    L.wx_arith.restype = i32
    L.wx_upload.argtypes = [vp, vp, vp, vp, vp]
    L.wx_set_params.argtypes = [vp, C.POINTER(WxParams), vp, vp, vp, vp]
    L.wx_step.argtypes = [vp, i32]
    L.wx_step_overlap.argtypes = [vp, i32, C.c_uint]
    L.wx_set_comm_stream.argtypes = [vp, vp]
    L.wx_sync.argtypes = [vp]
    L.wx_set_option.argtypes = [vp, i32, i32]
    L.wx_water_free.argtypes = [vp]
    L.wx_tune_placement.argtypes = [vp, i32, i32, vp, vp]
    L.wx_slab_assert_water_free.argtypes = [vp, i32]
    L.wx_get_iter.argtypes = [vp]
    L.wx_get_iter.restype = i64
    L.wx_set_iter.argtypes = [vp, i64]
    L.wx_read_rect.argtypes = [vp, i32, i32, i32, i32, i32, vp, i32]
    L.wx_read_particles.argtypes = [vp, i32, i32, vp]
    L.wx_set_stream.argtypes = [vp, vp]
    L.wx_device_ptr.argtypes = [vp, i32]
    L.wx_device_ptr.restype = vp
    L.wx_local_width.argtypes = [vp]
    L.wx_halo_bytes.argtypes = [vp]
    L.wx_halo_bytes.restype = C.c_size_t
    L.wx_halo_message_bytes.argtypes = [vp]
    L.wx_halo_message_bytes.restype = C.c_size_t
    L.wx_halo_pack.argtypes = [vp, i32, vp]
    L.wx_halo_unpack.argtypes = [vp, i32, vp]
    L.wx_halo_pack_both.argtypes = [vp, vp, vp]
    L.wx_halo_unpack_both.argtypes = [vp, vp, vp]
    L.wx_profile.argtypes = [vp, i32]
    L.wx_profile_read.argtypes = [vp, i32, vp, vp]
    L.wx_kernel_count.restype = i32
    L.wx_kernel_name.argtypes = [i32]
    L.wx_kernel_name.restype = C.c_char_p
    L.wx_slab_set_rank.argtypes = [vp, i32]
    L.wx_slab_period_begin.argtypes = [vp]
    L.wx_pool_event_bytes.argtypes = [vp]
    L.wx_pool_event_bytes.restype = C.c_size_t
    L.wx_pool_edge_bytes.argtypes = [vp]
    L.wx_pool_edge_bytes.restype = C.c_size_t
    L.wx_pool_events_pack.argtypes = [vp, vp]
    L.wx_pool_events_apply.argtypes = [vp, vp, i32, C.c_size_t]
    L.wx_pool_edges_pack.argtypes = [vp, vp, vp, i32]
    L.wx_pool_edges_apply.argtypes = [vp, vp]
    L.wx_pool_flags.argtypes = [vp, vp]
    L.wx_lightning_get.argtypes = [vp, vp]
    L.wx_lightning_set.argtypes = [vp, vp]
    L.wx_setup_columns.argtypes = [vp] + [vp] * 8
    L.wx_init_droplets.argtypes = [vp, C.c_uint32]
    L.wx_fastest_velocity.argtypes = [vp, C.POINTER(C.c_float)]
    L.wx_placement_info.argtypes = [vp, C.POINTER(C.c_float), C.POINTER(C.c_float)]
    L.wx_pair_stats.argtypes = [vp, C.POINTER(C.c_int64), C.POINTER(C.c_int64)]
    L.wx_slab_vx_take.argtypes = [vp, C.POINTER(C.c_float)]
    L.wx_slab_set_vx_bound.argtypes = [vp, C.c_float]
    L.wx_slab_cone.argtypes = [vp]
    L.wx_slab_period.argtypes = [vp]
    L.wx_setup_terrain.argtypes = [vp, C.c_double, C.c_double, C.c_int, C.c_double] + [vp] * 4
    L.wx_stream_bytes.argtypes = [i32, i32]
    L.wx_stream_bytes.restype = C.c_size_t
    L.wx_host_alloc.argtypes = [C.c_size_t]
    L.wx_host_alloc.restype = vp
    L.wx_host_free.argtypes = [vp]
    L.wx_host_free.restype = None
    L.wx_stream_frame.argtypes = [vp, i32, i32, i32, i32, vp]
    L.wx_stream_wait.argtypes = [vp]
    L.wx_comm_unique_id.argtypes = [vp]
    L.wx_comm_init.argtypes = [vp, vp, i32, i32]
    L.wx_exchange.argtypes = [vp]
    L.wx_slab_step.argtypes = [vp, i32]
    L.wx_group_create.argtypes = [i32, vp, i32, i32, i32, i32, i32, C.POINTER(vp)]
    L.wx_group_destroy.argtypes = [vp]
    L.wx_group_destroy.restype = None
    L.wx_group_last_error.argtypes = [vp]
    L.wx_group_last_error.restype = C.c_char_p
    L.wx_group_count.argtypes = [vp]
    L.wx_group_transport.argtypes = [vp]
    L.wx_group_slab.argtypes = [vp, i32]
    L.wx_group_slab.restype = vp
    L.wx_group_agree.argtypes = [vp]
    L.wx_group_step.argtypes = [vp, i32]
    L.wx_group_sync.argtypes = [vp]
    L.wx_group_set_option.argtypes = [vp, i32, i32]
    L.wx_group_exchange.argtypes = [vp]
    L.wx_diag_collect.argtypes = [vp, vp]
    L.wx_diag_merge.argtypes = [vp, vp]
    L.wx_diag_finish.argtypes = [vp, vp]
    L.wx_diag_accumulate.argtypes = [vp, i32, vp, C.c_size_t]
    L.wx_diag_accumulate_cells.argtypes = [vp, i32, i32, i32, i32, i32, vp, vp, vp]
    L.wx_diagnostics.argtypes = [vp, vp]
    L.wx_group_diagnostics.argtypes = [vp, vp]
    L.wx_ensemble_create.argtypes = [i32, i32, i32, C.POINTER(vp)]
    L.wx_ensemble_create_droplets.argtypes = [i32, i32, i32, i32, C.POINTER(vp)]
    L.wx_ensemble_particle_stats.argtypes = [vp, C.POINTER(C.c_int64), C.POINTER(C.c_int64)]
    L.wx_ensemble_destroy.argtypes = [vp]
    L.wx_ensemble_destroy.restype = None
    L.wx_ensemble_last_error.argtypes = [vp]
    L.wx_ensemble_last_error.restype = C.c_char_p
    L.wx_ensemble_count.argtypes = [vp]
    L.wx_ensemble_member.argtypes = [vp, i32]
    L.wx_ensemble_member.restype = vp
    L.wx_ensemble_step.argtypes = [vp, i32]
    L.wx_ensemble_sync.argtypes = [vp]
    L.wx_ensemble_diagnostics.argtypes = [vp, vp]
    L.wx_ensemble_stats.argtypes = [vp, C.POINTER(C.c_int64), C.POINTER(C.c_int64), C.POINTER(C.c_int64)]
# ... 99 lines not shown
        if drops is not None and self.n_droplets > 0:
            drops = np.ascontiguousarray(drops, np.float32).reshape(-1)
            if drops.size != self.n_droplets * 5:
                raise ValueError("drops must hold n_droplets x 5 values")
            d = drops.ctypes.data
        self._chk(lib().wx_upload(self._h, base.ctypes.data, water.ctypes.data, wall.ctypes.data, d))

    def set_params(self, p: WxParams, initial_T=None, snd_T=None, snd_W=None, snd_Vel=None):
        arrs = []
        for a in (initial_T, snd_T, snd_W, snd_Vel):
            if a is None:
                arrs.append(None)
            else:
                a = np.ascontiguousarray(a, np.float32)
                if a.size < self.Y + 1:
                    raise ValueError("profile arrays need Y+1 entries")
                arrs.append(a)
        ptr = [None if a is None else a.ctypes.data for a in arrs]
        self._chk(lib().wx_set_params(self._h, C.byref(p), *ptr))

    OVERLAP_EDGES_FIRST, OVERLAP_EDGES_LAST = 1, 2

    def step(self, n: int = 1, overlap: int = 0):
        if not self._stepped and n > 0:
            self._stepped = True
            self.generation += 1
        if overlap:
            self._chk(lib().wx_step_overlap(self._h, int(n), int(overlap)))
        else:
            self._chk(lib().wx_step(self._h, int(n)))

    def sync(self):
        self._chk(lib().wx_sync(self._h))

    def copy_from(self, src: "Handle"):
        self.generation += 1
        self._chk(lib().wx_copy_state(self._h, src._h))
        self._stepped = self._stepped or src._stepped

    def tune_placement(self, tries: int = 6, iters_per_try: int = 30):
        a, b = C.c_float(0), C.c_float(0)
        self.generation += 1
        self._chk(lib().wx_tune_placement(self._h, int(tries), int(iters_per_try), C.byref(a), C.byref(b)))
        return float(a.value), float(b.value)

    def water_free(self) -> bool:
        return bool(lib().wx_water_free(self._h))

    def slab_assert_water_free(self, agreed: bool):
        self._chk(lib().wx_slab_assert_water_free(self._h, 1 if agreed else 0))

    OPT_SPLAT_ORDER, OPT_CHECK_LAUNCHES, OPT_KERNEL_SET, OPT_DRY_KERNEL, OPT_ROW_BANDS, OPT_FIX_CAP, OPT_POOL_EXACT, OPT_EXCHANGE_OVERLAP, OPT_DRY_PAIRS = 1, 2, 3, 4, 5, 6, 7, 8, 10
    OPT_PLACEMENT_SEARCH = 12
    OPT_WATER0_ON_DEMAND = 11

    def set_option(self, option: int, value: int):
        self._chk(lib().wx_set_option(self._h, int(option), int(value)))

    @property
    def iter(self) -> int:
        return lib().wx_get_iter(self._h)

    @iter.setter
    def iter(self, v: int):
        self._chk(lib().wx_set_iter(self._h, int(v)))

    def read_rect(self, field: str, x: int = 0, y: int = 0, w: Optional[int] = None, h: Optional[int] = None, *, int32: bool = False):
        w = self.X - x if w is None else w
        h = self.Y - y if h is None else h
        if field == "LIGHTNING":
            out = np.zeros(4, np.float32)
            self._chk(lib().wx_read_rect(self._h, 12, 0, 0, 1, 1, out.ctypes.data, DTYPE_F32))
            return out
        ch = FIELD_CHANNELS.get(field, 4)
        if field.startswith("WALL"):
            out = np.zeros((max(h, 0), max(w, 0), ch), np.int32 if int32 else np.int8)
            dt = DTYPE_I32 if int32 else DTYPE_I8
        elif field == "EMITTED":
            out = np.zeros((max(h, 0), max(w, 0), 4), np.float16)
            dt = DTYPE_F16
        else:
            out = np.zeros((max(h, 0), max(w, 0), ch), np.float32)
            dt = DTYPE_F32
        self._chk(lib().wx_read_rect(self._h, FIELD_IDS[field], x, y, w, h, out.ctypes.data, dt))
        return out

    def read_particles(self, first: int = 0, count: Optional[int] = None):
        count = self.n_droplets - first if count is None else count
        out = np.zeros((max(count, 0), 5), np.float32)
        self._chk(lib().wx_read_particles(self._h, first, count, out.ctypes.data))
        return out

    def diagnostics(self) -> dict:
        d = WxDiag()
        self._chk(lib().wx_diagnostics(self._h, C.byref(d)))
        return _diag_dict(d)

    def diagnostics_raw(self) -> bytes:
        r = WxDiagRaw()
        self._chk(lib().wx_diag_collect(self._h, C.byref(r)))
        return bytes(r)

    def set_stream(self, stream_ptr: int):
        self._chk(lib().wx_set_stream(self._h, C.c_void_p(stream_ptr)))

    def set_comm_stream(self, stream_ptr: int):
# ... 36 lines not shown
                raise MemoryError(f"wx_host_alloc({nbytes})")
            self._pin = (p, nbytes)
        self._chk(L.wx_stream_frame(self._h, x, y, w, h, C.c_void_p(self._pin[0])))
        self._frame = (w, h)

    def stream_wait(self):
        self._chk(lib().wx_stream_wait(self._h))
        w, h = self._frame
        raw = (C.c_char * self._pin[1]).from_address(self._pin[0])
        out, off = {}, 0
        for name, dt, ch in self.STREAM_FIELDS:
            n = w * h * ch
            out[name] = np.frombuffer(raw, dtype=dt, count=n, offset=off).reshape(h, w, ch)
            off += n * np.dtype(dt).itemsize
        return out

    def setup_columns(self, desc, drops=None):
        want = {"wall_rows": (np.int32, self.X), "sea": (np.uint8, self.X), "veg_noise": (np.float64, self.X), "snow": (np.float32, self.X),
                "T_air": (np.float32, self.Y), "total_water": (np.float32, self.Y), "cloud_water": (np.float32, self.Y)}
        arrs = []
        for k, (dt, n) in want.items():
            a = np.ascontiguousarray(desc[k], dt)
            if a.shape != (n,):
                raise ValueError(f"setup_columns: {k} has shape {a.shape}, expected ({n},)")
            arrs.append(a)
        dp = None
        if drops is not None:
            drops = np.ascontiguousarray(drops, np.float32)
            if drops.shape != (self.n_droplets, 5):
                raise ValueError("setup_columns: drops must be (n_droplets, 5) float32")
            dp = drops.ctypes.data_as(C.c_void_p)
        self._chk(lib().wx_setup_columns(self._h, *[a.ctypes.data_as(C.c_void_p) for a in arrs], dp))

    def setup_terrain(self, sounding, seed: float = 0.5, height_mult: float = 0.3, snap: int = 2, sim_height: float = 12000.0, drops=None):
        arrs = []
        for k in ("T_air", "total_water", "cloud_water"):
            a = np.ascontiguousarray(sounding[k], np.float32)
            if a.shape != (self.Y,):
                raise ValueError(f"setup_terrain: {k} has shape {a.shape}, expected ({self.Y},)")
            arrs.append(a)
        dp = None
        if drops is not None:
            drops = np.ascontiguousarray(drops, np.float32)
            if drops.shape != (self.n_droplets, 5):
                raise ValueError("setup_terrain: drops must be (n_droplets, 5) float32")
            dp = drops.ctypes.data_as(C.c_void_p)
        self._chk(lib().wx_setup_terrain(self._h, float(seed), float(height_mult), int(snap), float(sim_height), *[a.ctypes.data_as(C.c_void_p) for a in arrs], dp))

    def fastest_velocity(self) -> float:
        v = C.c_float(0)
        self._chk(lib().wx_fastest_velocity(self._h, C.byref(v)))
        return float(v.value)

    def placement_info(self):
        a, b = C.c_float(0), C.c_float(0)
        return (float(a.value), float(b.value)) if lib().wx_placement_info(self._h, C.byref(a), C.byref(b)) == 1 else None

    def pair_stats(self):
        a, b = C.c_int64(0), C.c_int64(0)
        self._chk(lib().wx_pair_stats(self._h, C.byref(a), C.byref(b)))
        return int(a.value), int(b.value)

    def slab_vx_take(self) -> float:
        v = C.c_float(0)
        self._chk(lib().wx_slab_vx_take(self._h, C.byref(v)))
        return float(v.value)

    def slab_set_vx_bound(self, v_measured: float):
        self._chk(lib().wx_slab_set_vx_bound(self._h, C.c_float(float(v_measured))))

    @property
    def slab_cone(self) -> int:
        return int(lib().wx_slab_cone(self._h))

    @property
    def slab_period(self) -> int:
        return int(lib().wx_slab_period(self._h))

    def init_droplets(self, seed: int = 1):
        self._chk(lib().wx_init_droplets(self._h, C.c_uint32(int(seed) & 0xFFFFFFFF)))

    def slab_set_rank(self, rank: int):
        self._chk(lib().wx_slab_set_rank(self._h, rank))

    def slab_period_begin(self):
        self._chk(lib().wx_slab_period_begin(self._h))

    def pool_event_bytes(self) -> int:
        return lib().wx_pool_event_bytes(self._h)

    def pool_edge_bytes(self) -> int:
        return lib().wx_pool_edge_bytes(self._h)

    def pool_events_pack(self, dev_buf: int):
        self._chk(lib().wx_pool_events_pack(self._h, C.c_void_p(dev_buf)))

    def pool_events_apply(self, dev_bufs: int, n_ranks: int, stride_bytes: int = 0):
        self._chk(lib().wx_pool_events_apply(self._h, C.c_void_p(dev_bufs), int(n_ranks), int(stride_bytes)))

    def pool_edges_pack(self, dev_left: int, dev_right: int, refresh_inactive: bool = False):
        self._chk(lib().wx_pool_edges_pack(self._h, C.c_void_p(dev_left), C.c_void_p(dev_right), 1 if refresh_inactive else 0))

    def pool_edges_apply(self, dev_buf: int):
        self._chk(lib().wx_pool_edges_apply(self._h, C.c_void_p(dev_buf)))

    def pool_flags(self) -> np.ndarray:
# ... 251 lines not shown
```

include/wxsim.h:

```cpp
#ifndef WXSIM_H
#define WXSIM_H

#include <stddef.h>
#include <stdint.h>

#ifdef __cplusplus
extern "C" {
#endif

#define WX_ABI_VERSION 11

#define WX_OK 0
#define WX_E_INVALID (-1)
#define WX_E_DEVICE (-2)
#define WX_E_NOMEM (-3)
#define WX_E_RANGE (-4)
#define WX_E_STATE (-5)

typedef struct wx_params {
  float dragMultiplier, wind;
  float vorticity, landEvaporation, waterEvaporation, dynamicWaterTemperature;
  float evapHeat, waterWeight;
  float sunAngle;
  float dryLapse;
// ... 43 lines not shown
  WX_FIELD_COUNT = 14
};

enum { WX_DTYPE_F32 = 0, WX_DTYPE_I8 = 1, WX_DTYPE_I32 = 2, WX_DTYPE_F16 = 3 };

typedef struct wx_sim wx_sim;

int wx_create(int X, int Y, int n_droplets, wx_sim **out);

int wx_create_slab(int X_global, int Y, int x0, int X_owned, int halo, int n_droplets, wx_sim **out);
#define WX_SLAB_CONE 6
#define WX_SLAB_CONE_PARTICLES 9
#define WX_SLAB_PERIOD_PARTICLES(halo) ((halo) < 12 ? 0 : ((1 + ((halo) - 12) / WX_SLAB_CONE_PARTICLES) < 15 ? (1 + ((halo) - 12) / WX_SLAB_CONE_PARTICLES) : 15))
int wx_slab_vx_take(wx_sim *s, float *vmax);
int wx_slab_set_vx_bound(wx_sim *s, float v_measured);
int wx_slab_cone(const wx_sim *s);
int wx_slab_period(const wx_sim *s);

void wx_destroy(wx_sim *s);
const char *wx_last_error(const wx_sim *s);
int wx_abi_version(void);
#define WX_ARITH_EXACT 0
#define WX_ARITH_FAST 1
int wx_arith(void);

int wx_upload(wx_sim *s, const float *base, const float *water, const int8_t *wall, const float *drops);

int wx_setup_columns(wx_sim *s, const int32_t *wall_rows, const uint8_t *sea_column, const double *veg_noise, const float *snow,
                     const float *T_air, const float *total_water, const float *cloud_water, const float *drops);

int wx_setup_terrain(wx_sim *s, double seed, double height_mult, int snap, double sim_height, const float *T_air, const float *total_water,
                     const float *cloud_water, const float *drops);

int wx_init_droplets(wx_sim *s, uint32_t seed);

int wx_set_params(wx_sim *s, const wx_params *p, const float *initial_T, const float *sounding_T,
                  const float *sounding_W, const float *sounding_Vel);

int wx_step(wx_sim *s, int n_iter);
int wx_sync(wx_sim *s);

#define WX_OPT_SPLAT_ORDER 1
#define WX_OPT_CHECK_LAUNCHES 2
#define WX_OPT_KERNEL_SET 3
#define WX_OPT_DRY_KERNEL 4
#define WX_OPT_ROW_BANDS 5
#define WX_OPT_FIX_CAP 6
#define WX_OPT_POOL_EXACT 7
#define WX_OPT_EXCHANGE_OVERLAP 8
#define WX_OPT_DRY_PAIRS 10
#define WX_OPT_WATER0_ON_DEMAND 11
#define WX_OPT_PLACEMENT_SEARCH 12
#define WX_PLACEMENT_AUTO_CELLS (8u << 20)
int wx_set_option(wx_sim *s, int option, int value);

int64_t wx_get_iter(const wx_sim *s);
int wx_set_iter(wx_sim *s, int64_t iter);

int wx_read_rect(wx_sim *s, int field, int x, int y, int w, int h, void *dst, int dtype);

int wx_read_particles(wx_sim *s, int first, int count, float *dst);

size_t wx_stream_bytes(int w, int h);
void *wx_host_alloc(size_t bytes);
void wx_host_free(void *p);
int wx_stream_frame(wx_sim *s, int x, int y, int w, int h, void *host_dst);
int wx_stream_wait(wx_sim *s);

int wx_tune_placement(wx_sim *s, int tries, int iters_per_try, float *ms_before, float *ms_after);
int wx_placement_info(const wx_sim *s, float *ms_first, float *ms_kept);

int wx_set_stream(wx_sim *s, void *hip_stream);
void *wx_device_ptr(wx_sim *s, int field);
int wx_local_width(const wx_sim *s);
size_t wx_halo_bytes(const wx_sim *s);
size_t wx_halo_message_bytes(const wx_sim *s);
int wx_halo_pack(wx_sim *s, int side, void *dev_buf);
int wx_halo_unpack(wx_sim *s, int side, const void *dev_buf);
int wx_halo_pack_both(wx_sim *s, void *dev_left, void *dev_right);
int wx_halo_unpack_both(wx_sim *s, const void *dev_left, const void *dev_right);
int wx_water_free(const wx_sim *s);
int wx_slab_assert_water_free(wx_sim *s, int agreed);

#define WX_OVERLAP_EDGES_FIRST 1u
#define WX_OVERLAP_EDGES_LAST 2u
#define WX_OVERLAP_MORE_TO_COME 4u
int wx_set_comm_stream(wx_sim *s, void *hip_stream);
int wx_step_overlap(wx_sim *s, int n_iter, unsigned flags);

int wx_slab_set_rank(wx_sim *s, int rank);
int wx_slab_period_begin(wx_sim *s);
size_t wx_pool_event_bytes(const wx_sim *s);
size_t wx_pool_edge_bytes(const wx_sim *s);
int wx_pool_events_pack(wx_sim *s, void *dev_buf);
int wx_pool_events_apply(wx_sim *s, const void *dev_bufs, int n_ranks, size_t stride_bytes);
int wx_pool_edges_pack(wx_sim *s, void *dev_left, void *dev_right, int refresh_inactive);
int wx_pool_edges_apply(wx_sim *s, const void *dev_buf);
int wx_pool_flags(wx_sim *s, uint8_t *host_dst);
int wx_lightning_get(wx_sim *s, float out[4]);
int wx_lightning_set(wx_sim *s, const float in[4]);

#define WX_UNIQUE_ID_BYTES 128
int wx_comm_unique_id(void *id128);
int wx_comm_init(wx_sim *s, const void *id128, int rank, int world);
int wx_exchange(wx_sim *s);
int wx_slab_step(wx_sim *s, int n_iter);

// ... 181 lines not shown
```

Measured before the change: 49300.

## Add planar split storage for water field with per-strip zero flags

Adds an optional planar layout for the water field: the float4 is split into two float2 planes (xy, zw), plus a per-56-column strip flag that marks strips whose z/w channels are all zero. Conversion kernels move data between RGBA and planar forms, and the wet march and fix kernels gain a PLANAR_Q template path. Consumers that expect RGBA get a view that converts back lazily. The aim is to cut memory traffic for water and to let later code skip zero strips. In exchange it adds conversion passes and bookkeeping, and it is gated behind a new option.

```diff
diff --git a/2d-weather-sandbox_amd/csrc/wx_ens_score.h b/2d-weather-sandbox_amd/csrc/wx_ens_score.h
--- a/2d-weather-sandbox_amd/csrc/wx_ens_score.h
+++ b/2d-weather-sandbox_amd/csrc/wx_ens_score.h
@@ -182,6 +182,7 @@
   if (e->broken) return WX_E_STATE;
   DeviceScope dev_scope(e->member[0]);
 
+  if (field != WX_FIELD_BASE_CUR) water_rgba_view(truth, 1);
   if (truth->ens != e)
     if (int rc = wx_sync(truth)) return efail(e, rc, "truth: %s", truth->err.c_str());
 
diff --git a/2d-weather-sandbox_amd/csrc/wx_state_copy.h b/2d-weather-sandbox_amd/csrc/wx_state_copy.h
--- a/2d-weather-sandbox_amd/csrc/wx_state_copy.h
+++ b/2d-weather-sandbox_amd/csrc/wx_state_copy.h
@@ -37,6 +37,8 @@
     *b.slots[k] = b.blocks[i].p + ((const char *)*a.slots[k] - a.blocks[i].p);
   }
   dst->run = src->run;
+  dst->run.water_planar = false;
+  dst->run.water_view_fresh[1] = dst->run.water_view_fresh[2] = false;
   dst->run.wet_shape_valid = false;
   dst->run.fix_check = false;
   dst->p = src->p;
@@ -78,6 +80,8 @@
   if (dst == src) return WX_OK;
   if (int rc = state_copy_check(dst, src, "wx_copy_state")) return rc;
   DeviceScope dev_scope(src);
+  water_rgba_view(src, 1);
+  water_rgba_view(src, 2);
   if (int rc = wx_sync(src)) {
     dst->err = "wx_copy_state: src: " + src->err;
     return rc;
diff --git a/2d-weather-sandbox_amd/csrc/wx_tile.h b/2d-weather-sandbox_amd/csrc/wx_tile.h
--- a/2d-weather-sandbox_amd/csrc/wx_tile.h
+++ b/2d-weather-sandbox_amd/csrc/wx_tile.h
@@ -19,6 +19,15 @@
 };
 using LightPlanes = LightPlanesT<float, float2>;
 using LightPlanesC = LightPlanesT<const float, const float2>;
+
+constexpr int WQ_STRIP = 56;
+template <typename F2, typename B> struct WaterPlanesT {
+  F2 *xy, *zw;
+  B *zero;
+};
+using WaterPlanes = WaterPlanesT<float2, unsigned char>;
+using WaterPlanesC = WaterPlanesT<const float2, const unsigned char>;
+__device__ __forceinline__ bool zw_bits_zero(float z, float w) { return (__float_as_uint(z) | __float_as_uint(w)) == 0u; }
 
 __device__ __forceinline__ size_t fidx(int x, int y, int X) { return (size_t)y * X + x; }
 __device__ __forceinline__ int wrapfast(int i, int n) { return i < 0 ? i + n : (i >= n ? i - n : i); }
@@ -135,4 +144,34 @@
   }
 }
 
+__global__ __launch_bounds__(256) void k_water_to_planes(int X, int Y, const float4 *__restrict__ src, WaterPlanes dst, unsigned char *__restrict__ spare_zero)
+{
+  const int n_strips = (X + WQ_STRIP - 1) / WQ_STRIP, lane = threadIdx.x & 63;
+  const size_t total = (size_t)Y * n_strips;
+  for (size_t sr = (size_t)blockIdx.x * 4 + (threadIdx.x >> 6); sr < total; sr += (size_t)gridDim.x * 4) {
+    const int row = (int)(sr / n_strips), x = (int)(sr - (size_t)row * n_strips) * WQ_STRIP + lane;
+    const bool in = lane < WQ_STRIP && x < X;
+    bool z0 = true;
+    if (in) {
+      const size_t i = fidx(x, row, X);
+      const float4 q = src[i];
+      dst.xy[i] = make_float2(q.x, q.y);
+      dst.zw[i] = make_float2(q.z, q.w);
+      z0 = zw_bits_zero(q.z, q.w);
+    }
+    const bool all0 = __all(z0);
+    if (lane == 0) {
+      dst.zero[sr] = all0 ? 1 : 0;
+      spare_zero[sr] = 0;
+    }
+  }
 }
+__global__ void k_water_from_planes(size_t n, WaterPlanesC src, float4 *__restrict__ dst)
+{
+  for (size_t i = (size_t)blockIdx.x * blockDim.x + threadIdx.x; i < n; i += (size_t)gridDim.x * blockDim.x) {
+    const float2 xy = src.xy[i], zw = src.zw[i];
+    dst[i] = make_float4(xy.x, xy.y, zw.x, zw.y);
+  }
+}
+
+}
diff --git a/2d-weather-sandbox_amd/csrc/wx_wet.h b/2d-weather-sandbox_amd/csrc/wx_wet.h
--- a/2d-weather-sandbox_amd/csrc/wx_wet.h
+++ b/2d-weather-sandbox_amd/csrc/wx_wet.h
@@ -59,14 +59,47 @@
   int *hint;
 };
 
-struct WetSlowArgs {
+struct WetInQ : WetIn {
+  WaterPlanesC q;
+};
+struct WetOutQ : WetOut {
+  WaterPlanes q;
+};
+template <class T> struct wet_is_planar : std::false_type {};
+template <> struct wet_is_planar<WetInQ> : std::true_type {};
+template <> struct wet_is_planar<WetOutQ> : std::true_type {};
+__device__ __forceinline__ const WetIn &wet_in_sel(std::false_type, const WetIn &in, const WaterPlanesC &) { return in; }
+__device__ __forceinline__ WetInQ wet_in_sel(std::true_type, const WetIn &in, const WaterPlanesC &q) { return WetInQ{in, q}; }
+__device__ __forceinline__ const WetOut &wet_out_sel(std::false_type, const WetOut &out, const WaterPlanes &) { return out; }
+__device__ __forceinline__ WetOutQ wet_out_sel(std::true_type, const WetOut &out, const WaterPlanes &q) { return WetOutQ{out, q}; }
+template <class In> __device__ __forceinline__ float4 wet_water_ld(const In &in, size_t gi)
+{
+  if constexpr (wet_is_planar<In>::value) {
+    const float2 a = in.q.xy[gi], b = in.q.zw[gi];
+    return make_float4(a.x, a.y, b.x, b.y);
+  } else {
+    return in.water[gi];
+  }
+}
+template <class Out> __device__ __forceinline__ void wet_water_st(const Out &out, size_t gi, int x, int y, int X, float4 v)
+{
+  if constexpr (wet_is_planar<Out>::value) {
+    out.q.xy[gi] = make_float2(v.x, v.y);
+    out.q.zw[gi] = make_float2(v.z, v.w);
+    if (!zw_bits_zero(v.z, v.w)) out.q.zero[(size_t)y * ((X + WQ_STRIP - 1) / WQ_STRIP) + x / WQ_STRIP] = 0;
+  } else {
+    out.water[gi] = v;
+  }
+}
+
+template <class In> struct WetSlowArgsT {
   const FullCtx *ctx;
-  WetIn in;
+  In in;
   float iterNum;
 };
-struct GWetRecomputeAcc {
+template <class In> struct GWetRecomputeAcc {
   const Uni &u_;
-  const WetIn &in_;
+  const In &in_;
   int X, Y, x, y;
   __device__ __forceinline__ int wx_(int dx) const { return wrapmod(x + dx, X); }
   __device__ __forceinline__ int wy_(int dy) const { return wrapmod(y + dy, Y); }
@@ -83,7 +116,7 @@
   }
   __device__ __forceinline__ float4 base(int dx, int dy) const { return vel_at(wx_(dx), wy_(dy)); }
   __device__ __forceinline__ char4 wall(int dx, int dy) const { return in_.wall[fidx(wx_(dx), wy_(dy), X)]; }
-  __device__ __forceinline__ float4 water(int dx, int dy) const { return in_.water[fidx(wx_(dx), wy_(dy), X)]; }
+  __device__ __forceinline__ float4 water(int dx, int dy) const { return wet_water_ld(in_, fidx(wx_(dx), wy_(dy), X)); }
   __device__ __forceinline__ float2 vort(int dx, int dy) const
   {
     const int xx = wx_(dx), yy = wy_(dy);
@@ -110,28 +143,28 @@
   float4 b, w;
   char4 wl;
 };
-__device__ __noinline__ BOut wet_boundary_texel_global(const WetSlowArgs *__restrict__ sa, int x, int y)
+template <class In> __device__ __noinline__ BOut wet_boundary_texel_global(const WetSlowArgsT<In> *__restrict__ sa, int x, int y)
 {
   const FullCtx *c = sa->ctx;
-  GWetRecomputeAcc a{c->u, sa->in, c->g.X, c->g.Y, x, y};
+  GWetRecomputeAcc<In> a{c->u, sa->in, c->g.X, c->g.Y, x, y};
   BOut o;
   boundary_cell(c->u, sa->iterNum, (int)sa->iterNum, c->g, c->initial_T, x, y, a, o.b, o.w, o.wl);
   return o;
 }
-struct GWetAdvectAcc {
-  const WetSlowArgs *sa;
+template <class In> struct GWetAdvectAcc {
+  const WetSlowArgsT<In> *sa;
   int X, Y, x, y;
-  __device__ __forceinline__ BOut at(int dx, int dy) const { return wet_boundary_texel_global(sa, wrapmod(x + dx, X), wrapmod(y + dy, Y)); }
+  __device__ __forceinline__ BOut at(int dx, int dy) const { return wet_boundary_texel_global<In>(sa, wrapmod(x + dx, X), wrapmod(y + dy, Y)); }
   __device__ __forceinline__ float4 base(int dx, int dy) const { return at(dx, dy).b; }
   __device__ __forceinline__ char4 wall(int dx, int dy) const { return at(dx, dy).wl; }
   __device__ __forceinline__ float4 base_off(int dx, int dy) const { return at(dx, dy).b; }
   __device__ __forceinline__ float4 water_off(int dx, int dy) const { return at(dx, dy).w; }
   __device__ __forceinline__ char4 wall_off(int dx, int dy) const { return at(dx, dy).wl; }
 };
-__device__ __noinline__ AdvOut wet_advection_cell_recompute(const WetSlowArgs *__restrict__ sa, int x, int y)
+template <class In> __device__ __noinline__ AdvOut wet_advection_cell_recompute(const WetSlowArgsT<In> *__restrict__ sa, int x, int y)
 {
   const FullCtx *c = sa->ctx;
-  GWetAdvectAcc a{sa, c->g.X, c->g.Y, x, y};
+  GWetAdvectAcc<In> a{sa, c->g.X, c->g.Y, x, y};
   AdvOut o;
   advection_cell(c->u, c->g, c->initial_T, c->snd_T, c->snd_W, c->snd_Vel, x, y, a, o.b, o.w, o.wl);
   return o;
@@ -149,17 +182,17 @@
   __device__ __forceinline__ float ir_down_at(int j) const { return l.zw[fidx(x, j, X)].x; }
   __device__ __forceinline__ float ir_up_at(int j) const { return l.zw[fidx(x, j, X)].y; }
 };
-__device__ __noinline__ void wet_output_cell_exact(const FullCtx *__restrict__ c, const WetIn *__restrict__ in, const WetOut *__restrict__ out, float iterNum,
+template <class In, class Out> __device__ __noinline__ void wet_output_cell_exact(const FullCtx *__restrict__ c, const In *__restrict__ in, const Out *__restrict__ out, float iterNum,
                                                    int opt_out, int x, int y)
 {
-  const WetSlowArgs sa{c, *in, iterNum};
+  const WetSlowArgsT<In> sa{c, *in, iterNum};
   const int X = c->g.X, Y = c->g.Y;
-  const AdvOut o0 = wet_advection_cell_recompute(&sa, x, y);
-  const AdvOut oL = wet_advection_cell_recompute(&sa, x == 0 ? X - 1 : x - 1, y);
-  const AdvOut oD = wet_advection_cell_recompute(&sa, x, y == 0 ? Y - 1 : y - 1);
+  const AdvOut o0 = wet_advection_cell_recompute<In>(&sa, x, y);
+  const AdvOut oL = wet_advection_cell_recompute<In>(&sa, x == 0 ? X - 1 : x - 1, y);
+  const AdvOut oD = wet_advection_cell_recompute<In>(&sa, x, y == 0 ? Y - 1 : y - 1);
   const size_t gi = fidx(x, y, X);
   out->base[gi] = pressure_cell(o0.b, oL.b.x, oD.b.y, oD.b.w, oD.wl.x, oD.wl.y);
-  out->water[gi] = o0.w;
+  wet_water_st(*out, gi, x, y, X, o0.w);
   out->wall[gi] = o0.wl;
   GWetLightAcc la{in->lsrc, o0.w, o0.wl, o0.b.w, oD.b.w, X, x};
   const float4 l = lighting_cell(c->u, c->g, x, y, la);
@@ -360,6 +393,8 @@
   int split_at, strip_lo2;
   int edge_prio;
   VxTrack vx;
+  WaterPlanesC qin;
+  WaterPlanes qout;
 };
 struct WetEnsSlot {
   WetKArgs ka;
@@ -367,10 +402,10 @@
   int pad_[2 + (16 - (sizeof(WetKArgs) + sizeof(int *) + 8) % 16) % 16 / 4];
 };
 static_assert(sizeof(WetEnsSlot) % 16 == 0, "table slots keep the 16-byte alignment of the wide scalar loads");
-template <bool OPT_OUT, bool HAS_FB, bool QUIET>
+template <bool OPT_OUT, bool HAS_FB, bool QUIET, bool PLANAR_Q = false>
 __global__ __launch_bounds__(64 * WX_WET_WPB, WX_WET_MINWAVES) void k_march_wet(const FullCtx *__restrict__ ctx, float iterNum, WetIn in_arg, WetOut out_arg,
                                                                     WetFixList fix_arg, int n_strips, int strip_lo,
-                                                                    int n_strips_all, WetSegs segs, int split_at, int strip_lo2, int edge_prio_arg, VxTrack vx_arg)
+                                                                    int n_strips_all, WetSegs segs, int split_at, int strip_lo2, int edge_prio_arg, VxTrack vx_arg, WaterPlanesC qin_arg, WaterPlanes qout_arg)
 {
   typedef WetKArgs KArgs;
   typedef const __attribute__((address_space(4))) char *KBytes;
@@ -393,6 +428,7 @@
   const float iterNum = ka.iterNum;
   const int n_strips = ka.n_strips, strip_lo = ka.strip_lo, n_strips_all = ka.n_strips_all, split_at = ka.split_at, strip_lo2 = ka.strip_lo2;
   const __attribute__((address_space(4))) WetSegs &segs = ka.segs;
+  constexpr bool PLANAR_Q = false;
 #include "wx_wet_march_body.h"
 }
 
@@ -442,10 +478,10 @@
   float cu[WSC * WSC];
   float fx[WSF * WSF], fy[WSF * WSF];
 };
-struct WetStageBoundaryAcc {
+template <class In> struct WetStageBoundaryAcc {
   const WetFixStage &st;
   const Uni &u_;
-  const WetIn &in_;
+  const In &in_;
   int X, Y, x, y;
   int px, py;
   __device__ __forceinline__ float4 base(int dx, int dy) const
@@ -454,7 +490,7 @@
     return make_float4(st.vx[iv], st.vy[iv], st.bP[ib], st.bT[ib]);
   }
   __device__ __forceinline__ char4 wall(int dx, int dy) const { return st.bw[(py + 2 + dy) * WSB + (px + 2 + dx)]; }
-  __device__ __forceinline__ float4 water(int dx, int dy) const { return in_.water[fidx(wrapmod(x + dx, X), wrapmod(y + dy, Y), X)]; }
+  __device__ __forceinline__ float4 water(int dx, int dy) const { return wet_water_ld(in_, fidx(wrapmod(x + dx, X), wrapmod(y + dy, Y), X)); }
   __device__ __forceinline__ float2 vort(int dx, int dy) const
   {
     const int i = (py + 1 + dy) * WSF + (px + 1 + dx);
@@ -476,7 +512,7 @@
   }
   __device__ __forceinline__ float2 dep() const { return in_.dep ? in_.dep[fidx(x, y, X)] : make_float2(0.f, 0.f); }
 };
-__device__ __noinline__ void wet_fix_build_patch(const FullCtx *__restrict__ c, const WetIn *__restrict__ in, float iterNum, WetFixStage *__restrict__ stp,
+template <class In> __device__ __noinline__ void wet_fix_build_patch(const FullCtx *__restrict__ c, const In *__restrict__ in, float iterNum, WetFixStage *__restrict__ stp,
                                                  WetPatch *__restrict__ ptp, int cx, int cy, int lane)
 {
   WetFixStage &st = *stp;
@@ -515,7 +551,7 @@
   {
     const int px = lane & (WPATCH - 1), py = lane >> 3;
     const int gx = wrapmod(cx - WPATCH_C + px, X), gy = wrapmod(cy - WPATCH_C + py, Y);
-    const WetStageBoundaryAcc a{st, c->u, *in, X, Y, gx, gy, px, py};
+    const WetStageBoundaryAcc<In> a{st, c->u, *in, X, Y, gx, gy, px, py};
     float4 bb, bq;
     char4 bwl;
     boundary_cell(c->u, iterNum, (int)iterNum, c->g, c->initial_T, gx, gy, a, bb, bq, bwl);
@@ -532,9 +568,10 @@
   wave_fence();
 }
 
-template <bool OPT_OUT>
+template <bool OPT_OUT, bool PLANAR_Q = false>
 __global__ __launch_bounds__(256) void k_wet_fix(const FullCtx *__restrict__ ctx, float iterNum, WetIn in, WetOut out, int *__restrict__ count,
-                                                 const int2 *__restrict__ cells, int cap, int *__restrict__ overflow, int *__restrict__ hint)
+                                                 const int2 *__restrict__ cells, int cap, int *__restrict__ overflow, int *__restrict__ hint, WaterPlanesC qin,
+                                                 WaterPlanes qout)
 {
 #include "wx_wet_fix_body.h"
 }
@@ -552,6 +589,9 @@
   const int cap = sl.ka.fix.cap;
   int *__restrict__ overflow = sl.overflow;
   int *__restrict__ hint = sl.ka.fix.hint;
+  constexpr bool PLANAR_Q = false;
+  const WaterPlanesC qin{nullptr, nullptr, nullptr};
+  const WaterPlanes qout{nullptr, nullptr, nullptr};
 #include "wx_wet_fix_body.h"
 }
 
@@ -708,8 +748,11 @@
 
 inline void launch_march_wet(const WetLaunch &w, float iterNum, const FullCtx *ctx, const WetIn &in, const WetOut &out, const WetFixList &fix,
                              bool opt_out, bool quiet, hipStream_t stream, int strip_lo = 0, int strip_count = -1, int strip_lo2 = 0, int strip_count2 = 0,
-                             int edge_prio = 0, const VxTrack *vx = nullptr)
-{
+                             int edge_prio = 0, const VxTrack *vx = nullptr, const WaterPlanesC *qin = nullptr, const WaterPlanes *qout = nullptr)
+{
+  const bool planar_q = qin && qout && qin->xy && qout->xy;
+  const WaterPlanesC qi = planar_q ? *qin : WaterPlanesC{nullptr, nullptr, nullptr};
+  const WaterPlanes qo = planar_q ? *qout : WaterPlanes{nullptr, nullptr, nullptr};
   const int ns1 = strip_count < 0 ? w.n_strips : strip_count, ns = ns1 + (strip_count2 > 0 ? strip_count2 : 0);
   if (ns <= 0) return;
   const int groups = ((w.segs.bands ? ns : (ns + 7) / 8) + WX_WET_WPB - 1) / WX_WET_WPB;
@@ -727,28 +770,41 @@
     vt.zone_r = vx->zone_r / WOUT;
   }
 #define WX_LAUNCH_W(O, F, Q) \
-  hipLaunchKernelGGL((k_march_wet<O, F, Q>), grid, dim3(64 * WX_WET_WPB), 0, stream, ctx, iterNum, in, out, fix, ns, strip_lo, w.n_strips, w.segs, ns1, strip_lo2, edge_prio, vt)
+  hipLaunchKernelGGL((k_march_wet<O, F, Q>), grid, dim3(64 * WX_WET_WPB), 0, stream, ctx, iterNum, in, out, fix, ns, strip_lo, w.n_strips, w.segs, ns1, strip_lo2, edge_prio, vt, qi, qo)
 #define WX_LAUNCH_WQ(O, F) \
   do { if (quiet) WX_LAUNCH_W(O, F, true); else WX_LAUNCH_W(O, F, false); } while (0)
-  if (opt_out) {
+#define WX_LAUNCH_WP(O, Q) \
+  hipLaunchKernelGGL((k_march_wet<O, false, Q, true>), grid, dim3(64 * WX_WET_WPB), 0, stream, ctx, iterNum, in, out, fix, ns, strip_lo, w.n_strips, w.segs, ns1, strip_lo2, edge_prio, vt, qi, qo)
+  if (planar_q && has_fb) {
+    fprintf(stderr, "[wx_wet] launch_march_wet: planar water together with feedback textures\n");
+    std::abort();
+  }
+  if (planar_q) {
+    if (opt_out) { if (quiet) WX_LAUNCH_WP(true, true); else WX_LAUNCH_WP(true, false); }
+    else { if (quiet) WX_LAUNCH_WP(false, true); else WX_LAUNCH_WP(false, false); }
+  } else if (opt_out) {
     if (has_fb) WX_LAUNCH_WQ(true, true); else WX_LAUNCH_WQ(true, false);
   } else {
     if (has_fb) WX_LAUNCH_WQ(false, true); else WX_LAUNCH_WQ(false, false);
   }
+#undef WX_LAUNCH_WP
 #undef WX_LAUNCH_WQ
 #undef WX_LAUNCH_W
 }
 
 inline void launch_wet_fix(float iterNum, const FullCtx *ctx, const WetIn &in, const WetOut &out, const WetFixList &fix, int *overflow, bool opt_out,
-                           hipStream_t stream, int wgs = 0)
-{
+                           hipStream_t stream, int wgs = 0, const WaterPlanesC *qin = nullptr, const WaterPlanes *qout = nullptr)
+{
+  const bool planar_q = qin && qout && qin->xy && qout->xy;
+  const WaterPlanesC qi = planar_q ? *qin : WaterPlanesC{nullptr, nullptr, nullptr};
+  const WaterPlanes qo = planar_q ? *qout : WaterPlanes{nullptr, nullptr, nullptr};
   const int last = fix.hint ? *(volatile const int *)fix.hint_host : -1;
   const int want = last < 0 ? 512 : (last > 0 ? std::min(512, std::max(32, last)) : 32);
   const dim3 grid(wgs > 0 ? wgs : want), block(256);
-  if (opt_out)
-    hipLaunchKernelGGL((k_wet_fix<true>), grid, block, 0, stream, ctx, iterNum, in, out, fix.count, fix.cells, fix.cap, overflow, fix.hint);
-  else
-    hipLaunchKernelGGL((k_wet_fix<false>), grid, block, 0, stream, ctx, iterNum, in, out, fix.count, fix.cells, fix.cap, overflow, fix.hint);
+#define WX_LAUNCH_F(O, P) hipLaunchKernelGGL((k_wet_fix<O, P>), grid, block, 0, stream, ctx, iterNum, in, out, fix.count, fix.cells, fix.cap, overflow, fix.hint, qi, qo)
+  if (planar_q) { if (opt_out) WX_LAUNCH_F(true, true); else WX_LAUNCH_F(false, true); }
+  else { if (opt_out) WX_LAUNCH_F(true, false); else WX_LAUNCH_F(false, false); }
+#undef WX_LAUNCH_F
 }
 
 inline int ens_member_groups(const WetLaunch &w)
diff --git a/2d-weather-sandbox_amd/csrc/wx_wet_fix_body.h b/2d-weather-sandbox_amd/csrc/wx_wet_fix_body.h
--- a/2d-weather-sandbox_amd/csrc/wx_wet_fix_body.h
+++ b/2d-weather-sandbox_amd/csrc/wx_wet_fix_body.h
@@ -12,9 +12,11 @@
   }
   if (total > cap && blockIdx.x == 0 && threadIdx.x == 0) *overflow = total;
   const int X = ctx->g.X, Y = ctx->g.Y;
+  const auto &fin = wet_in_sel(std::integral_constant<bool, PLANAR_Q>{}, in, qin);
+  const auto &fout = wet_out_sel(std::integral_constant<bool, PLANAR_Q>{}, out, qout);
   for (int i = blockIdx.x * 4 + wave; i < n; i += gridDim.x * 4) {
     const int2 c = cells[i];
-    wet_fix_build_patch(ctx, &in, iterNum, &stages[wave], &pt, c.x, c.y, lane);
+    wet_fix_build_patch(ctx, &fin, iterNum, &stages[wave], &pt, c.x, c.y, lane);
     AdvOut o;
     o.b = o.w = make_float4(0.f, 0.f, 0.f, 0.f);
     o.wl = make_char4(0, 0, 0, 0);
@@ -29,12 +31,12 @@
     const int wl_d = __shfl(*reinterpret_cast<const int *>(&o.wl), 2);
     if (lane == 0) {
       if (any_bad) {
-        wet_output_cell_exact(ctx, &in, &out, iterNum, OPT_OUT, c.x, c.y);
+        wet_output_cell_exact(ctx, &fin, &fout, iterNum, OPT_OUT, c.x, c.y);
       } else {
         const char4 wD = unpack_wall(wl_d);
         const size_t gi = fidx(c.x, c.y, X);
         out.base[gi] = pressure_cell(o.b, vx_l, vy_d, T_d, wD.x, wD.y);
-        out.water[gi] = o.w;
+        wet_water_st(fout, gi, c.x, c.y, X, o.w);
         out.wall[gi] = o.wl;
         GWetLightAcc la{in.lsrc, o.w, o.wl, o.b.w, T_d, X, c.x};
         const float4 l = lighting_cell(ctx->u, ctx->g, c.x, c.y, la);
diff --git a/2d-weather-sandbox_amd/csrc/wx_wet_march_body.h b/2d-weather-sandbox_amd/csrc/wx_wet_march_body.h
--- a/2d-weather-sandbox_amd/csrc/wx_wet_march_body.h
+++ b/2d-weather-sandbox_amd/csrc/wx_wet_march_body.h
@@ -1,5 +1,7 @@
   const __attribute__((address_space(4))) WetIn &in = *(const __attribute__((address_space(4))) WetIn *)(ka_c + offsetof(KArgs, in));
   const __attribute__((address_space(4))) WetOut &out = *(const __attribute__((address_space(4))) WetOut *)(ka_c + offsetof(KArgs, out));
+  const __attribute__((address_space(4))) WaterPlanesC &qin = *(const __attribute__((address_space(4))) WaterPlanesC *)(ka_c + offsetof(KArgs, qin));
+  const __attribute__((address_space(4))) WaterPlanes &qout = *(const __attribute__((address_space(4))) WaterPlanes *)(ka_c + offsetof(KArgs, qout));
   const int edge_prio = *(const __attribute__((address_space(4))) int *)(ka_c + offsetof(KArgs, edge_prio));
   __shared__ WetRing rings[WX_WET_WPB];
   const int wave = __builtin_amdgcn_readfirstlane(threadIdx.x >> 6);
@@ -27,6 +29,11 @@
   const bool lane_out = lane >= WLO && lane < WLO + WOUT && c_out < X;
   unsigned lo4 = (unsigned)col * 4u, lo8 = (unsigned)col * 8u, lo16 = (unsigned)col * 16u;
   unsigned lo12 = (unsigned)col * 12u;
+  [[maybe_unused]] unsigned zf_in = 0u, zf_out = 0u;
+  if constexpr (PLANAR_Q) {
+    zf_in = (unsigned)(col / WOUT);
+    zf_out = (unsigned)strip;
+  }
   unsigned so4 = lane_out ? (unsigned)c_out * 4u : 0u, so8 = so4 * 2u, so16 = so4 * 4u;
   const int y_lo = band_lo + segs.start[seg], y_hi = min(band_lo + segs.start[seg + 1], band_hi);
   if (y_lo >= y_hi) return;
@@ -41,6 +48,7 @@
   float3 pf_fb = make_float3(0.f, 0.f, 0.f);
   float2 pf_dep = make_float2(0.f, 0.f);
   bool fb_have = false, dep_have = false;
+  [[maybe_unused]] unsigned char pf_zf = 0, pf_df = 0;
   unsigned short pf_flag = 0x0101;
   float4 b_prev = make_float4(0.f, 0.f, 0.f, 0.f);
   int w_prev = 0;
@@ -116,7 +124,13 @@
       if (WX_T_GE(2)) {
         const int rl = r - 1;
         const size_t ew = (size_t)yw_m1 * X;
-        pf_q = ld_row(in.water + ew, lo16);
+        if constexpr (PLANAR_Q) {
+          const float2 qxy = ld_row(qin.xy + ew, lo8);
+          const float2 qzw = ld_row(__all(pf_zf == 1) ? reinterpret_cast<const float2 *>(in.zero_row) : qin.zw + ew, lo8);
+          pf_q = make_float4(qxy.x, qxy.y, qzw.x, qzw.y);
+        } else {
+          pf_q = ld_row(in.water + ew, lo16);
+        }
         const size_t el = (size_t)(rl < 0 ? 0 : (rl > Y - 1 ? Y - 1 : rl)) * X;
         pf_lx = ld_row(in.lsrc.x + el, lo4);
         pf_lzw = ld_row(in.lsrc.zw + el, lo8);
@@ -124,6 +138,7 @@
         WX_H_SET(h_near, __any(w_cur.y <= 1));
         if (h_near & 15u) pf_l0x = ld_row(in.l0.x + ew, lo4);
       }
+      if constexpr (PLANAR_Q) pf_zf = ld_row(qin.zero + (size_t)(yw_m1 + 1 == Y ? 0 : yw_m1 + 1) * n_strips_all, zf_in);
       if (HAS_FB) {
         fb_have = __any((pf_flag & 0xffu) == 0);
         dep_have = __any((pf_flag >> 8) == 0);
@@ -151,7 +166,16 @@
     if (st_valid && lane_out) {
       const size_t e = (size_t)(r - 5) * X;
       st_row(out.base + e, so16, st_p);
-      st_row(out.water + e, so16, st_q);
+      if constexpr (PLANAR_Q) {
+        st_row(qout.xy + e, so8, make_float2(st_q.x, st_q.y));
+        const bool z0 = __all(zw_bits_zero(st_q.z, st_q.w));
+        if (!(z0 && __all(pf_df == 1))) {
+          st_row(qout.zw + e, so8, make_float2(st_q.z, st_q.w));
+          if (lane == WLO) st_row(qout.zero + (size_t)(r - 5) * n_strips_all, zf_out, (unsigned char)(z0 ? 1 : 0));
+        }
+      } else {
+        st_row(out.water + e, so16, st_q);
+      }
       st_row(out.wall + e, so4, st_w);
       st_row(out.light.x + e, so4, st_l.x);
       st_row(out.light.y + e, so4, st_l.y);
@@ -162,6 +186,7 @@
 #endif
     }
     st_valid = false;
+    if constexpr (PLANAR_Q) pf_df = ld_row(qout.zero + (size_t)yw_m4 * n_strips_all, zf_out);
 #ifdef WX_STAGE_MARKS
     asm volatile("; @@velocity");
 #endif
@@ -381,7 +406,16 @@
   if (st_valid && lane_out) {
     const size_t e = (size_t)(y_hi - 1) * X;
     st_row(out.base + e, so16, st_p);
-    st_row(out.water + e, so16, st_q);
+    if constexpr (PLANAR_Q) {
+      st_row(qout.xy + e, so8, make_float2(st_q.x, st_q.y));
+      const bool z0 = __all(zw_bits_zero(st_q.z, st_q.w));
+      if (!(z0 && __all(pf_df == 1))) {
+        st_row(qout.zw + e, so8, make_float2(st_q.z, st_q.w));
+        if (lane == WLO) st_row(qout.zero + (size_t)(y_hi - 1) * n_strips_all, zf_out, (unsigned char)(z0 ? 1 : 0));
+      }
+    } else {
+      st_row(out.water + e, so16, st_q);
+    }
     st_row(out.wall + e, so4, st_w);
     st_row(out.light.x + e, so4, st_l.x);
     st_row(out.light.y + e, so4, st_l.y);
diff --git a/2d-weather-sandbox_amd/csrc/wxsim.hip b/2d-weather-sandbox_amd/csrc/wxsim.hip
--- a/2d-weather-sandbox_amd/csrc/wxsim.hip
+++ b/2d-weather-sandbox_amd/csrc/wxsim.hip
@@ -123,6 +123,7 @@
   int pool_exact = 0;
   bool exchange_in_order = false;
   bool lazy_water0 = true;
+  bool water_planes = false;
 };
 
 struct RunState {
@@ -134,6 +135,8 @@
   int64_t iter = 0;
   bool ran_fused = false;
   bool light_planar = false;
+  bool water_planar = false;
+  bool water_view_fresh[3] = {false, false, false};
   bool fb_dirty = false;
   bool water_trivial = false;
   bool local_water_free = false;
@@ -269,6 +272,7 @@
   float *initial_T = nullptr, *snd_T = nullptr, *snd_W = nullptr, *snd_Vel = nullptr;
   DevState *state = nullptr;
   LightPlanes lp[3] = {{nullptr, nullptr, nullptr}, {nullptr, nullptr, nullptr}, {nullptr, nullptr, nullptr}};
+  WaterPlanes wq[3] = {{nullptr, nullptr, nullptr}, {nullptr, nullptr, nullptr}, {nullptr, nullptr, nullptr}};
   float *tdisp = nullptr;
   float *pdisp = nullptr;
   FullCtx *full_ctx = nullptr;
@@ -657,6 +661,51 @@
   s->run.light_planar = false;
 }
 
+static bool water_planes_eligible(const wx_sim *s)
+{
+  return s->opt.water_planes && s->opt.fused && (s->p.pass_mask & 0x3Fu) == 0x3Fu && s->halo == 0 && !s->ens && s->n_drops == 0 && !s->run.fb_dirty;
+}
+static const float4 *water_rgba_view(wx_sim *s, int which)
+{
+  if (s->run.water_planar && (which == 1 || which == 2) && !s->run.water_view_fresh[which]) {
+    const WaterPlanesC src{s->wq[which].xy, s->wq[which].zw, s->wq[which].zero};
+    hipLaunchKernelGGL(k_water_from_planes, dim3(2048), dim3(256), 0, s->stream, ncell(s), src, s->water[which]);
+    s->run.water_view_fresh[which] = true;
+  }
+  return s->water[which];
+}
+static void water_rgba_mut(wx_sim *s)
+{
+  if (!s->run.water_planar) return;
+  water_rgba_view(s, 1);
+  water_rgba_view(s, 2);
+  s->run.water_planar = false;
+  s->run.water_view_fresh[1] = s->run.water_view_fresh[2] = false;
+}
+static int water_planes_enter(wx_sim *s)
+{
+  if (s->run.water_planar) return WX_OK;
+  const size_t n = ncell(s), nf = ((size_t)s->Y * ((s->X + WQ_STRIP - 1) / WQ_STRIP) + 255) & ~(size_t)255;
+  for (int i = 1; i <= 2; i++) {
+    if (!s->wq[i].xy)
+      if (int rc = dalloc(s, &s->wq[i].xy, n)) return rc;
+    if (!s->wq[i].zw)
+      if (int rc = dalloc(s, &s->wq[i].zw, n)) return rc;
+    if (!s->wq[i].zero)
+      if (int rc = dalloc(s, &s->wq[i].zero, nf)) return rc;
+  }
+  hipLaunchKernelGGL(k_water_to_planes, dim3(2048), dim3(256), 0, s->stream, s->X, s->Y, s->water[1], s->wq[1], s->wq[2].zero);
+  s->run.water_planar = true;
+  s->run.water_view_fresh[1] = s->run.water_view_fresh[2] = true;
+  return WX_OK;
+}
+static int water_planes_settle(wx_sim *s)
+{
+  if (water_planes_eligible(s)) return water_planes_enter(s);
+  water_rgba_mut(s);
+  return WX_OK;
+}
+
 static hipStream_t exchange_stream(const wx_sim *s)
 {
   const bool in_order = (s->pool.remote && s->opt.pool_exact) || s->opt.exchange_in_order || s->tx.xchg_inline;
@@ -736,6 +785,8 @@
   WetOut out;
   bool opt_out, quiet;
   float iter;
+  WaterPlanesC qin{nullptr, nullptr, nullptr};
+  WaterPlanes qout{nullptr, nullptr, nullptr};
 };
 int march_wet_prepare(wx_sim *s, bool opt_out, bool precip, WetIter &wi, int share_members = 1)
 {
@@ -746,6 +797,8 @@
   WetIn in{s->base[0], s->wall[0], s->water[1], LightPlanesC{s->lp[0].x, s->lp[0].y, s->lp[0].zw},
            LightPlanesC{s->lp[src].x, s->lp[src].y, s->lp[src].zw}, fb ? s->fb : nullptr, fb ? s->dep : nullptr, fb ? s->sg.fb_zero : nullptr,
            s->zero_row, s->sg.TXn};
+  const bool planar = s->run.water_planar;
+  if (planar && fb) return fail(s, WX_E_STATE, "wx_step: the water is held as planes while the feedback textures are live");
   const bool lazy_w0 = opt_out && !precip && !fb && s->opt.lazy_water0;
   WetOut out{s->base[1], s->wall[1], s->water[2], light_dst, s->pdisp, lazy_w0 ? nullptr : s->water[0], s->curl, (precip || opt_out) ? s->tdisp : nullptr};
   if (opt_out) s->run.disp_lazy = true;
@@ -791,6 +844,8 @@
   wi.opt_out = opt_out;
   wi.quiet = march_wet_quiet(s);
   wi.iter = (float)s->run.iter;
+  wi.qin = planar ? WaterPlanesC{s->wq[1].xy, s->wq[1].zw, s->wq[1].zero} : WaterPlanesC{nullptr, nullptr, nullptr};
+  wi.qout = planar ? s->wq[2] : WaterPlanes{nullptr, nullptr, nullptr};
   return WX_OK;
 }
 
@@ -814,8 +869,8 @@
         if (const char *e = wx_tune_env("WX_SPLIT_HALVE")) halved = atoi(e) != 0;
       }
       const WetFixList fl = edge_group ? s->split.edge_fix.wet(&s->state->fastest_bits) : fix;
-      launch_march_wet(halved ? wet_shape_halved(shape) : shape, iter, s->full_ctx, in, out, fl, opt_out, quiet, st, lo0, cnt0, lo1, cnt1, edge_prio, &vt);
-      launch_wet_fix(iter, s->full_ctx, in, out, fl, &s->state->fix_overflow, opt_out, st, halved ? 64 : 0);
+      launch_march_wet(halved ? wet_shape_halved(shape) : shape, iter, s->full_ctx, in, out, fl, opt_out, quiet, st, lo0, cnt0, lo1, cnt1, edge_prio, &vt, &wi.qin, &wi.qout);
+      launch_wet_fix(iter, s->full_ctx, in, out, fl, &s->state->fix_overflow, opt_out, st, halved ? 64 : 0, &wi.qin, &wi.qout);
     };
     const int nl = s->halo > 0 ? (2 * s->halo - 1) / WOUT + 1 : 0, nr0 = s->halo > 0 ? (s->X - 2 * s->halo) / WOUT : shape.n_strips;
     if (int rc = split_iteration(s, edge_mode, nl, nr0, shape.n_strips, true, launch)) return rc;
@@ -853,6 +908,10 @@
   std::swap(s->base[0], s->base[1]);
   std::swap(s->wall[0], s->wall[1]);
   std::swap(s->water[1], s->water[2]);
+  if (s->run.water_planar) {
+    std::swap(s->wq[1], s->wq[2]);
+    s->run.water_view_fresh[1] = s->run.water_view_fresh[2] = false;
+  }
   if (!s->run.even) std::swap(s->lp[0], s->lp[2]);
 }
 
@@ -1226,6 +1285,8 @@
   s->run.air_from_row = -1;
   s->run.ghost_check = false;
   s->run.light_planar = false;
+  s->run.water_planar = false;
+  s->run.water_view_fresh[1] = s->run.water_view_fresh[2] = false;
   s->run.period_j = 0;
   s->pool.exact_pending = 0;
   s->tx.since_exchange = 0;
@@ -1397,6 +1458,8 @@
   } tail_reset{s};
   s->prof.tail = nullptr;
   s->prof.chain = true;
+  if (n_iter > 0)
+    if (int rc = water_planes_settle(s)) return rc;
   if (!s->place.done && !s->place.busy && n_iter > 0) {
     s->place.done = true;
     if (s->opt.place_tries > 0 && s->halo == 0 && ncell(s) >= WX_PLACEMENT_AUTO_CELLS && !s->store.blocks.empty()) {
@@ -1590,6 +1653,9 @@
   case WX_OPT_CHECK_LAUNCHES:
     s->opt.check_launches = value != 0;
     return WX_OK;
+  case WX_OPT_WATER_PLANES:
+    s->opt.water_planes = value != 0;
+    return WX_OK;
   default:
     return fail(s, WX_E_INVALID, "wx_set_option: unknown option %d", option);
   }
@@ -1731,6 +1797,7 @@
   if (!s->uploaded || !s->have_params) return fail(s, WX_E_STATE, "wx_tune_placement before wx_upload / wx_set_params");
   if (s->pool.remote) return fail(s, WX_E_STATE, "wx_tune_placement: not on slab handles with particles (the exchange period would advance)");
   if (int rc = materialize_water0(s)) return rc;
+  if (int rc = water_planes_settle(s)) return rc;
   if (int rc = wx_sync(s)) return rc;
   struct Busy {
     wx_sim *s;
@@ -2029,7 +2096,7 @@
     }
   }
   const dim3 grid = grid2d(s), block(BX, BY);
-  const float4 *base_in = s->base[1], *water_in = s->water[2];
+  const float4 *base_in = s->base[1], *water_in = water_rgba_view(s, 2);
   const char4 *wall_in = s->wall[1];
   const LightPlanes &l0 = s->w0.even ? s->lp[0] : s->lp[2];
   const float4 *light0 = s->w0.light;
@@ -2063,7 +2130,7 @@
   case WX_FIELD_WATER_0:
     if (int rc = materialize_water0(s)) return rc < -1 ? rc : WX_E_DEVICE;
     *ptr = s->water[0]; *channels = 4; *elem = 4; return 0;
-  case WX_FIELD_WATER_CUR: *ptr = s->water[1]; *channels = 4; *elem = 4; return 0;
+  case WX_FIELD_WATER_CUR: *ptr = water_rgba_view(s, 1); *channels = 4; *elem = 4; return 0;
   case WX_FIELD_WALL_CUR: *ptr = s->wall[0]; *channels = 4; *elem = 1; return 0;
   case WX_FIELD_WALL_DISP: *ptr = s->run.ran_fused ? s->wall[0] : s->wall[1]; *channels = 4; *elem = 1; return 0;
   case WX_FIELD_LIGHT_0:
@@ -2104,9 +2171,9 @@
   }
   const int src = s->run.even ? 1 : 0;
   if (s->run.light_planar)
-    hipLaunchKernelGGL(k_emitted<true>, grid, block, 0, s->stream, s->geo, s->run.emit_uni, x, y, w, h, s->water[1], s->wall[0], nullptr, s->lp[src].x, s->emitted);
+    hipLaunchKernelGGL(k_emitted<true>, grid, block, 0, s->stream, s->geo, s->run.emit_uni, x, y, w, h, water_rgba_view(s, 1), s->wall[0], nullptr, s->lp[src].x, s->emitted);
   else
-    hipLaunchKernelGGL(k_emitted<false>, grid, block, 0, s->stream, s->geo, s->run.emit_uni, x, y, w, h, s->water[1], s->wall[0], s->light[src], nullptr, s->emitted);
+    hipLaunchKernelGGL(k_emitted<false>, grid, block, 0, s->stream, s->geo, s->run.emit_uni, x, y, w, h, water_rgba_view(s, 1), s->wall[0], s->light[src], nullptr, s->emitted);
   HIPCHK(s, hipGetLastError());
   return WX_OK;
 }
@@ -2205,7 +2272,7 @@
   HIPCHK(s, hipMemsetAsync(s->diag_table, 0, bytes, s->stream));
   const int Xo = s->X - 2 * s->halo;
   const unsigned chunks = (unsigned)((Xo + wxd::WG - 1) / wxd::WG) * (unsigned)s->Y;
-  hipLaunchKernelGGL(wxd::k_diag_cells, dim3(std::min<unsigned>(chunks, wxd::MAX_WGS)), dim3(wxd::WG), 0, s->stream, s->X, s->Y, s->halo, Xo, s->Xg, s->x0, s->base[0], s->water[1],
+  hipLaunchKernelGGL(wxd::k_diag_cells, dim3(std::min<unsigned>(chunks, wxd::MAX_WGS)), dim3(wxd::WG), 0, s->stream, s->X, s->Y, s->halo, Xo, s->Xg, s->x0, s->base[0], water_rgba_view(s, 1),
                      s->wall[0], s->diag_table);
   if (s->n_drops > 0) {
     const unsigned wgs = std::min<unsigned>((unsigned)((s->n_drops + wxd::WG - 1) / wxd::WG), wxd::MAX_WGS);
@@ -2350,9 +2417,21 @@
     if (field_info(s, WX_FIELD_BASE_DISP, &ptr, &ch, &el) || hipStreamSynchronize(s->stream) != hipSuccess) return nullptr;
     s->run.disp_lazy = false;
   }
+  if (field == WX_FIELD_WATER_CUR) water_rgba_mut(s);
   if (field_info(s, field, &ptr, &ch, &el)) return nullptr;
   if (field == WX_FIELD_BASE_CUR) s->vx.untracked = true;
   return const_cast<void *>(ptr);
+}
+
+int wx_debug_water_flags(wx_sim *s, int which, uint8_t *out)
+{
+  if (!s || !out) return WX_E_INVALID;
+  DeviceScope dev_scope(s);
+  if (which != 1 && which != 2) return fail(s, WX_E_INVALID, "wx_debug_water_flags: plane set %d (1: current water, 2: spare)", which);
+  if (!s->run.water_planar) return fail(s, WX_E_STATE, "wx_debug_water_flags: the handle's water is not in planar mode");
+  HIPCHK(s, hipMemcpyAsync(out, s->wq[which].zero, (size_t)s->Y * ((s->X + WQ_STRIP - 1) / WQ_STRIP), hipMemcpyDeviceToHost, s->stream));
+  HIPCHK(s, hipStreamSynchronize(s->stream));
+  return WX_OK;
 }
 
 int wx_local_width(const wx_sim *s) { return s ? s->X : 0; }
diff --git a/2d-weather-sandbox_amd/engine.py b/2d-weather-sandbox_amd/engine.py
--- a/2d-weather-sandbox_amd/engine.py
+++ b/2d-weather-sandbox_amd/engine.py
@@ -40,6 +40,7 @@
     "wx_ensemble_quantiles", "wx_ens_quant_cells", "wx_ens_quant_staged_members",
     "wx_ensemble_scores", "wx_ens_score_cells", "wx_ens_score_max_members",
     "wx_ensemble_assimilate", "wx_ens_assim_cells",
+    "wx_debug_water_flags",
 ]
 
 
@@ -516,6 +517,8 @@
     L.wx_init_droplets.argtypes = [vp, C.c_uint32]
     L.wx_fastest_velocity.argtypes = [vp, C.POINTER(C.c_float)]
     L.wx_placement_info.argtypes = [vp, C.POINTER(C.c_float), C.POINTER(C.c_float)]
+    if hasattr(L, "wx_debug_water_flags"):
+        L.wx_debug_water_flags.argtypes = [vp, i32, vp]
     L.wx_pair_stats.argtypes = [vp, C.POINTER(C.c_int64), C.POINTER(C.c_int64)]
     L.wx_slab_vx_take.argtypes = [vp, C.POINTER(C.c_float)]
     L.wx_slab_set_vx_bound.argtypes = [vp, C.c_float]
@@ -721,6 +724,7 @@
 
     OPT_SPLAT_ORDER, OPT_CHECK_LAUNCHES, OPT_KERNEL_SET, OPT_DRY_KERNEL, OPT_ROW_BANDS, OPT_FIX_CAP, OPT_POOL_EXACT, OPT_EXCHANGE_OVERLAP, OPT_DRY_PAIRS = 1, 2, 3, 4, 5, 6, 7, 8, 10
     OPT_PLACEMENT_SEARCH = 12
+    OPT_WATER_PLANES = 13
     OPT_WATER0_ON_DEMAND = 11
 
     def set_option(self, option: int, value: int):
@@ -863,6 +867,11 @@
         self._chk(lib().wx_fastest_velocity(self._h, C.byref(v)))
         return float(v.value)
 
+    def debug_water_flags(self, which: int = 1) -> np.ndarray:
+        out = np.zeros((self.Y, (self.X + 55) // 56), dtype=np.uint8)
+        self._chk(lib().wx_debug_water_flags(self._h, int(which), out.ctypes.data_as(C.c_void_p)))
+        return out
+
     def placement_info(self):
         a, b = C.c_float(0), C.c_float(0)
         return (float(a.value), float(b.value)) if lib().wx_placement_info(self._h, C.byref(a), C.byref(b)) == 1 else None
diff --git a/include/wxsim.h b/include/wxsim.h
--- a/include/wxsim.h
+++ b/include/wxsim.h
@@ -119,7 +119,9 @@
 #define WX_OPT_WATER0_ON_DEMAND 11
 #define WX_OPT_PLACEMENT_SEARCH 12
 #define WX_PLACEMENT_AUTO_CELLS (8u << 20)
+#define WX_OPT_WATER_PLANES 13
 int wx_set_option(wx_sim *s, int option, int value);
+int wx_debug_water_flags(wx_sim *s, int which, uint8_t *out);
 
 int64_t wx_get_iter(const wx_sim *s);
 int wx_set_iter(wx_sim *s, int64_t iter);
```

After: 48730. -1.2%, worse.
